# ARPA-SIMC/CRITERIA3D

Hardware: AMD Instinct MI355X
Metric: simulated-hours/sec on 512x512x20 grid (higher is better)
Workload: dtype f64

## Files before the change

### criteria3d_amd/csrc/sf3d_device.h

```cpp
#ifndef SF3D_DEVICE_H
#define SF3D_DEVICE_H

#include <stdint.h>

#define SF3D_SLOTS 10
#ifndef SF3D_LINKS_RING
#define SF3D_LINKS_RING 8
#endif
static_assert(SF3D_LINKS_RING >= 2 && SF3D_LINKS_RING <= 16, "the ring holds the matrix of the step in progress and at least one accepted step's");
#define SF3D_POOL 5
#define SF3D_BLOCK 256
#define SF3D_CHUNK 64
#define SF3D_MAX_BLOCKS 2048
#define CK_NONE 0
#define CK_MIXED 255

enum : uint8_t { LK_NONE = 0, LK_SOIL_VERT = 1, LK_SOIL_LAT = 2, LK_RUNOFF = 3, LK_INFILTRATION = 4 };

enum : uint32_t {
    ST_IDLE = 0,
    ST_ATTEMPT = 1,
    ST_APPROX = 2,
    ST_SWEEP = 3,
    ST_POST = 4,
// ... 100 lines not shown
    uint32_t probePad;
    uint64_t earlyCourant;
    uint64_t counters[8];
    uint64_t heatCounters[4];
};

#define SF3D_MAX_RANKS 16
struct DistMail { unsigned long long w[8]; };
struct DistWindow {
    DistMail mail[2][SF3D_MAX_RANKS];
    unsigned long long ping[SF3D_MAX_RANKS];
    unsigned long long rrec[2][SF3D_MAX_RANKS][4];
};
struct RecGet { uint32_t off0, cnt; };
struct RecPut { uint32_t off0, cnt, peer, nDest; };
struct DistView {
    int32_t world, rank;
    DistWindow* win[SF3D_MAX_RANKS];
    double* payload[SF3D_MAX_RANKS];
    const uint32_t* sendIdx[SF3D_MAX_RANKS]; uint32_t sendCount[SF3D_MAX_RANKS]; uint64_t sendOff[SF3D_MAX_RANKS];
    const uint32_t* recvIdx[SF3D_MAX_RANKS]; uint32_t recvCount[SF3D_MAX_RANKS]; uint64_t recvOff[SF3D_MAX_RANKS];
    const uint8_t* owner;
    const uint32_t* bndStart;
    const uint8_t* bndLane; const uint8_t* bndPeer; const uint32_t* bndSlot;
    const uint32_t* fsrc;
    const RecGet* recGet; const RecPut* recPut;
    int32_t rccl;
    double* mine;
    const double* gathered;
    double* sendBuf[SF3D_MAX_RANKS];
    const double* recvBuf[SF3D_MAX_RANKS];
    unsigned long long* stats;
    long long spinTicks;
};
#define SF3D_DIST_FIELDS 9
enum { DF_X = 0, DF_K = 1, DF_FLOW = 2, DF_RECLO = 3, DF_RECHI = 4, DF_KLO = 5, DF_KHI = 6, DF_FLO = 7, DF_FHI = 8 };
#define SF3D_FSRC_NONE 0xFFFFFFFFu

struct HeatDev {
    uint32_t on, water, vapor, advection, save;
    uint32_t gs;
    uint32_t redBlack;
    const uint8_t* lpar;
    const uint32_t* colourList[2]; uint32_t nColour[2];
    const uint32_t* gsOrder;
    double wf;
    double* TX[3];
    const double* heatSink;
    double *heatFlux, *invariant;
    double *hC, *hcapTerm, *hb, *hD;
    sf3d_d2* hA2;
    const double* hdist;
    const double* airP;
    double* thetaOld;
    double *thAvgC, *thNewC;
    double *kHeat, *kIsoVap, *hAvg;
    double *wThLiq, *wThVap, *wTm;
    const double *bHeightWind, *bHeightT, *bRoughH, *bT, *bRH, *bWind, *bNetIrr, *bFixT, *bFixDepth;
    double *bAero, *bSoilCond, *bSens, *bLat, *bRad, *bAdv;
    sf3d_f2* lwvFlux;
    double* lflux[SF3D_FLUX_TYPES];
};

#define SF3D_PAIR_NONE 15u
#define SF3D_PAIR_UP 9u
#define SF3D_PAIR_DOWN 10u
struct PairGrid {
    uint32_t NX, NY, NZ;
    uint32_t W;
    uint32_t patchCols, patchRows;
    uint32_t ownLo, ownHi;
    const uint32_t* nodeLat;
    const uint64_t* chunkCode;
    uint32_t masked;
    const int32_t* idxMap;
    const uint32_t* patchList;
    const uint8_t* patchDepth;
    uint32_t records;
    uint32_t recFast;
    int32_t sidePeer[2];
    uint32_t putBase[2], getBase[2];
    uint32_t recStride;
    const uint8_t* role;
};

struct ResGrid {
    uint32_t on;
    uint32_t NX, NY, NZ;
    uint32_t PR;
    uint32_t patchCols, rowGroups;
    uint32_t ownLo, ownHi;
    uint32_t K, NW;
    const uint32_t* nodeLat;
    const uint64_t* chunkCode;
    unsigned int* bar;
    unsigned long long* rec;
    unsigned long long* prec;
    unsigned long long* gpub;
    unsigned long long* prec2;
    uint32_t fusedPost;
    double* pub;
    const uint32_t* haloSrc;
    uint32_t forceTimeout;
    int32_t sidePeer[2];
    uint32_t recFast, putBase[2];
};

struct LinksBatch { uint32_t n, slot[SF3D_LINKS_RING]; double dt[SF3D_LINKS_RING]; };

struct DevView {
    uint32_t N, ns, nb;
    uint32_t Nnorm;
    uint32_t nChunks;
    uint32_t qSplit;
    uint32_t nbSurf, nbSoil;
    double probeMin;
    const uint32_t* chunkList; uint32_t nList, nListSurf;
    const uint32_t* asmList;
    uint32_t pLo, pHi;
    uint32_t aLo, aHi;
    const uint32_t* bndList; uint32_t nBnd;
    const uint16_t* lmask;
    uint32_t haloDirect;
    uint32_t ntStream;
    const DistView* dist;
    int32_t world, rank;
    const uint8_t* owner;
    const ChunkDesc* cdesc;
    const double *z, *size, *pond, *sink;
    const uint16_t* cls;
    const uint8_t* btype;
    const double *bslope, *bsize, *prescribed;
    const uint32_t* lto;
    const uint8_t* lkind;
    const uint8_t* probeMask;
    const double *larea, *ldist;
    double* lflowSum;
    sf3d_d2* A2x[SF3D_LINKS_RING];
    double* Hring[SF3D_LINKS_RING];
    double *b, *C;
    double* X[SF3D_POOL];
    double *Se, *SeHold, *K, *flow, *bflowRate, *bflowSum;
    double* compatCv; uint8_t* compatCn; double* compatDiag;
    double *cgDiag, *cgR, *cgP, *cgQ;
    double *part0, *part1;
    double *part2, *part3;
    unsigned int* arrive;
    unsigned int* gridBar;
    const SoilDev* soils;
    const double* roughness;
    PairGrid pair;
    ResGrid res;
    Ctrl* ctrl;
    HeatDev heat;
};

struct MapGeo {
    double cohesion;
    double tanFriction;
    double bulkDensity;
    double present;
};
struct MapView {
    const int32_t* col;
    const double* thick;
    const double* slope;
// ... 346 lines not shown
    const double* db[RAD_DOUBLE_MAPS];
    const int32_t* ok;
    double xll, yll, cellSize;
    float flag, demMax;
};

#define TR_MAX_WIDTH 63
#define TR_WINDOW_SLOTS 24
#define TR_MAX_POINTS 65536
#define TR_WAVE 64
enum { TR_MODE_POINTS = 0, TR_MODE_WINDOW = 1 };
struct TrPointDev {
    double x, y, z;
    RadCellDev cell;
    int32_t inGrid;
    int32_t pad;
};
struct TrView {
    RadGridDev grid;
    const RadHourDev* hours;
    const uint8_t* hourOk;
    const TrPointDev* points;
    const float* measured;
    uint8_t* written;
    float* elevationRefr;
    double* global;
    float* transmissivity;
    int32_t* windowSteps;
    uint32_t nPoints;
    int32_t nSlots, mode;
    float clearSky;
};
struct TrCall {
    const RadHourDev* hours;
    const uint8_t* hourOk;
    const TrPointDev* points;
    const float* measured;
    uint32_t nPoints;
    int32_t nSlots, mode;
    float clearSky;
};

struct HourRelhumView {
    const float* airT;
    const float* dewT;
    float* out;
    const uint8_t* mine;
    uint32_t nCells;
    float flag;
};
#define HOUR_TOTALS 3
struct HourTotalsView {
    const int32_t* col;
    const float* liquid;
    const double* actual;
    const float* dem;
    const uint8_t* mine;
    double* partials;
    double* totals;
    double area;
    uint32_t nCells, nBlocks, pass;
    float flag;
};
struct HourPondUnitDev { double maximumPond, laiMax; int32_t isCrop, pad; };
struct HourPondView {
    const int32_t* col;
    const double* tanSlope;
    const int32_t* unit;
    const float* lai;
    const HourPondUnitDev* units;
    float* out;
    const uint8_t* mine;
    uint32_t nCells;
    float laiFlag;
};
struct HourPondSetup {
    const double* tanSlope;
    const int32_t* unit;
    const HourPondUnitDev* units;
    uint32_t nCells, nUnits;
    uint64_t ver;
};

enum { KID_PROPS = 0, KID_ASSEMBLE, KID_SWEEP, KID_POST, KID_RESTORE, KID_ACCEPT, KID_SWEEP_PAIR, KID_SWEEP_RES, KID_MAPS, KID_COUNT };

#endif
```

### criteria3d_amd/csrc/sf3d_host_build.inc

```

namespace {

const char* kKernelNames[KID_COUNT] = {"k_props", "k_assemble", "k_sweep", "k_post", "k_restore", "k_accept", "k_sweep_pair", "k_sweep_resident", "k_output_map"};

}

struct ResShape { int K, NW; };
#define SF3D_RES_FOR_SHAPES(X) X(2, 5) X(2, 10) X(5, 8)
#define SF3D_RES_SHAPE(k, w) {k, w},
static const ResShape kResShapes[] = {SF3D_RES_FOR_SHAPES(SF3D_RES_SHAPE)};
#undef SF3D_RES_SHAPE

typedef void (*ViewKernel)(DevView);
static inline void launch_view(ViewKernel fn, dim3 grid, dim3 block, uint32_t lds, hipStream_t st, const DevView& v) { hipLaunchKernelGGL(fn, grid, block, lds, st, v); }
static ViewKernel res_kernel(int K, int NW, bool dist)
{
#define SF3D_RES_PTR(k, w) if (K == k && NW == w) return dist ? k_sweep_resident<k, w, true> : k_sweep_resident<k, w, false>;
    SF3D_RES_FOR_SHAPES(SF3D_RES_PTR)
#undef SF3D_RES_PTR
    return nullptr;
}
#define SF3D_PAIR_FOR_HEIGHTS(X) X(6) X(8) X(10) X(14)
static ViewKernel pair_kernel(uint32_t W, bool nt, bool dist, bool records, bool masked)
{
#define SF3D_PAIR_PTR(w)                                                                                                                      \
    if (W == w) {                                                                                                                             \
        if (masked) return dist ? (nt ? k_sweep_pair_masked<w, true, true> : k_sweep_pair_masked<w, false, true>)                             \
                                : (nt ? k_sweep_pair_masked<w, true, false> : k_sweep_pair_masked<w, false, false>);                          \
        if (dist && records) return nt ? k_sweep_pair<w, true, true, true> : k_sweep_pair<w, false, true, true>;                              \
        return dist ? (nt ? k_sweep_pair<w, true, true> : k_sweep_pair<w, false, true>) : (nt ? k_sweep_pair<w, true, false> : k_sweep_pair<w, false, false>); \
    }
    SF3D_PAIR_FOR_HEIGHTS(SF3D_PAIR_PTR)
#undef SF3D_PAIR_PTR
    return nullptr;
}
static ViewKernel sweep_kernel(int mode, bool nt)
{
#define SF3D_SWEEP_PTR(m) if (mode == m) return nt ? k_sweep<m, true> : k_sweep<m, false>;
    SF3D_SWEEP_PTR(0) SF3D_SWEEP_PTR(1) SF3D_SWEEP_PTR(2)
#undef SF3D_SWEEP_PTR
    return nullptr;
}

__global__ void k_dist_ping(DistView d, unsigned long long token, long long timeoutTicks, int* out);

struct MapsCache {
    int32_t* col = nullptr; double* thick = nullptr; double* slope = nullptr; MapGeo* geo = nullptr; float* out = nullptr; int* missing = nullptr;
    uint8_t* mine = nullptr;
    size_t colCap = 0, thickCap = 0, slopeCap = 0, geoCap = 0, outCap = 0, mineCap = 0;
    uint64_t colVer = 0, slopeVer = 0;
    std::vector<MapGeo> geoHost;
    void free_all()
    {
        for (void* q : {(void*)col, (void*)thick, (void*)slope, (void*)geo, (void*)out, (void*)missing, (void*)mine}) if (q) (void)hipFree(q);
        *this = MapsCache();
    }
};

struct SnowCache {
    float* base = nullptr; uint32_t nCells = 0; double lastMs = 0.; bool hourDone = false;
    const float* in[8] = {nullptr, nullptr, nullptr, nullptr, nullptr, nullptr, nullptr, nullptr};
    int feeds = 0;
    bool inputsHeld = false;
};
enum { FEED_METEO = 1, FEED_RAD = 2, FEED_SNOW = 4 };
struct CropCache { float* base = nullptr; CropUnitDev* units = nullptr; uint32_t nCells = 0, nUnits = 0; double lastMs[2] = {0., 0.}; };

struct RootCache {
    char* cells = nullptr;
    char* tables = nullptr;
    double* out = nullptr;
    size_t off[16] = {0};
    uint32_t nCells = 0, nUnits = 0, nSoils = 0, nRows = 0, nrLayers = 0, lunetteMax = 0;
    bool computed = false;
    double lastMs[3] = {0., 0., 0.};
};

struct MeteoCache {
    float* base = nullptr;
    char* stations = nullptr;
    bool hasMap[METEO_MAX_PROXIES] = {false};
    uint32_t nCells = 0, nRows = 0, nCols = 0, nProxies = 0;
    double xll = 0., yll = 0., cellSize = 0.;
    float flag = -9999.f;
    bool produced[METEO_VARIABLES] = {false};
    double lastMs = 0.;
    float* topoMaps = nullptr;
    char* topoTables = nullptr;
    float* topoMatrix = nullptr;
    uint32_t topoPoints = 0, topoMatrixCap = 0;
    double topoMs[3] = {0., 0., 0.};
    char* localFit = nullptr;
    char* localTables = nullptr;
    bool localDone = false;
    double localMs = 0.;
    char* proxiesFit = nullptr;
    char* proxiesTables = nullptr;
    bool proxiesDone = false;
    double proxiesMs = 0.;
};

struct RadCache {
    char* base = nullptr;
    uint32_t nCells = 0, nRows = 0, nCols = 0;
    double xll = 0., yll = 0., cellSize = 0.;
    float flag = -9999.f, demMax = -9999.f;
    double lastMs = 0.;
    bool hourDone = false;
    const float* trRead = nullptr;
    bool trFromMeteo = false;
    char* tr = nullptr;
    size_t trCap = 0, trOff[3] = {0, 0, 0};
    uint32_t trPoints = 0, trSlots = 0;
    double trMs = 0.;
};

struct SinkCache {
    char* cells = nullptr;
    char* tables = nullptr;
    double* nodes = nullptr;
    size_t off[8] = {0};
    uint32_t nCells = 0, nrLayers = 0, nUnits = 0, nSoils = 0, nodesN = 0;
    uint64_t nodesColVer = 0;
    int32_t lastEvapLayer = 0;
    double area = 0.;
    float flag = -9999.f;
    bool computed = false;
    double lastMs = 0.;
    SinkCrackDev crackDev{};
    char* crack = nullptr;
    uint64_t crackVer = 0;
    bool crackComputed = false;
    std::vector<double> layerDepth;
    const float* liquidRead = nullptr;
    int liquidFrom = 0;
};

struct HourCache {
    double* sums = nullptr; size_t sumsCap = 0;
    char* pond = nullptr;
    uint32_t pondCells = 0;
    uint64_t pondVer = 0;
    double lastMs[3] = {0., 0., 0.};
};

struct StepSwitches {
    bool residentGrids = true;
    bool graphs = true;
    bool asmNtOff = false;
    bool pairOddSingle = true;
    long residentFailAt = -1;
    int heatDebug = 0;
    int slabs = 0;
    uint32_t slabPropsBlocks = 512, slabAsmBlocks = 512; double slabFirst = 0.;
};

struct DeviceSolver::Impl {
    int device = -1;
    hipStream_t stream = nullptr;
    int overlapAccept = -1;
    uint32_t ring = 0;
    LinksBatch pend{};
    DevView v{};
    Ctrl* hostCtrl = nullptr;
    std::vector<void*> allocs;
    uint32_t N = 0, ns = 0;
    uint32_t ownedNodes = 0;
    uint32_t lastSweeps = 8;
    uint32_t lastBatches = 1;
    uint32_t predCount = 0, pred[16] = {0};
    uint32_t lastHeatSweeps = 8;
    std::vector<uint32_t> gsLevelStart;
    uint32_t lastHeatSteps = 1;
    double* heatOut[6] = {nullptr};
    double* heatAirP = nullptr;
    std::vector<std::pair<GraphKey, hipGraphExec_t>> graphs;
    template <class F> hipError_t replay(const GraphKey& key, hipStream_t st, F enqueue);
    int useFused = -1;
    StepSwitches sw;
    Partition part;
    DistWindow* window = nullptr;
    size_t windowBytes = 0;
    std::vector<void*> peerMaps;
    DistView hostDist{};
    DistView* devDist = nullptr;
    unsigned long long* distStats = nullptr;
    bool heatJacobiOnly = false;
    double hopUs[SF3D_MAX_RANKS] = {0};
    void* shmOwn = nullptr; int shmFd = -1; char shmName[48] = {0};
    std::vector<std::pair<void*, size_t>> shmPeers;
    std::vector<DistBlob> blobs;
    bool hostMode = false;
    void drop_shm()
    {
        for (auto& pr : shmPeers) { (void)hipHostUnregister(pr.first); munmap(pr.first, pr.second); }
        shmPeers.clear();
        if (shmOwn) { if (hostMode) (void)hipHostUnregister(shmOwn); munmap(shmOwn, windowBytes); shmOwn = nullptr; }
        if (shmFd >= 0) { close(shmFd); shmFd = -1; }
        if (shmName[0]) { shm_unlink(shmName); shmName[0] = 0; }
        hostMode = false;
    }
    uint32_t pushBlocks = 0;
    void* rcclLib = nullptr; ncclComm_t comm = nullptr; bool rcclMode = false;
    ncclResult_t (*pGetUniqueId)(ncclUniqueId*) = nullptr;
    ncclResult_t (*pCommInitRank)(ncclComm_t*, int, ncclUniqueId, int) = nullptr;
    ncclResult_t (*pCommDestroy)(ncclComm_t) = nullptr;
    ncclResult_t (*pSend)(const void*, size_t, ncclDataType_t, int, ncclComm_t, hipStream_t) = nullptr;
    ncclResult_t (*pRecv)(void*, size_t, ncclDataType_t, int, ncclComm_t, hipStream_t) = nullptr;
    ncclResult_t (*pAllGather)(const void*, void*, size_t, ncclDataType_t, ncclComm_t, hipStream_t) = nullptr;
    ncclResult_t (*pAllReduce)(const void*, void*, size_t, ncclDataType_t, ncclRedOp_t, ncclComm_t, hipStream_t) = nullptr;
    ncclResult_t (*pGroupStart)() = nullptr; ncclResult_t (*pGroupEnd)() = nullptr;
    double *rcclMine = nullptr, *rcclGathered = nullptr;
    bool rcclDistinct = false; unsigned char rcclId[128] = {0};
    bool load_rccl()
    {
        if (pAllGather) return true;
        if (const char* le = getenv("SF3D_RCCL_LIB")) if (!rcclLib && le[0]) rcclLib = dlopen(le, RTLD_NOW | RTLD_LOCAL);
        if (!rcclLib) rcclLib = dlopen("librccl.so.1", RTLD_NOW | RTLD_LOCAL);
        if (!rcclLib) rcclLib = dlopen("librccl.so", RTLD_NOW | RTLD_LOCAL);
        if (!rcclLib) return false;
        #define SF3D_SYM(ptr, name) ptr = reinterpret_cast<decltype(ptr)>(dlsym(rcclLib, name)); if (!ptr) return false
        SF3D_SYM(pGetUniqueId, "ncclGetUniqueId"); SF3D_SYM(pCommInitRank, "ncclCommInitRank"); SF3D_SYM(pCommDestroy, "ncclCommDestroy");
        SF3D_SYM(pSend, "ncclSend"); SF3D_SYM(pRecv, "ncclRecv"); SF3D_SYM(pAllReduce, "ncclAllReduce");
        SF3D_SYM(pGroupStart, "ncclGroupStart"); SF3D_SYM(pGroupEnd, "ncclGroupEnd"); SF3D_SYM(pAllGather, "ncclAllGather");
        #undef SF3D_SYM
        return true;
    }
    void rccl_halo(hipStream_t st, int fields)
    {
        pGroupStart();
        for (int p = 0; p < hostDist.world; ++p) {
            if (p == hostDist.rank) continue;
            if (hostDist.sendCount[p]) pSend(hostDist.sendBuf[p], (size_t)hostDist.sendCount[p] * fields, ncclDouble, p, comm, st);
            if (hostDist.recvCount[p]) pRecv(const_cast<double*>(hostDist.recvBuf[p]), (size_t)hostDist.recvCount[p] * fields, ncclDouble, p, comm, st);
        }
        pGroupEnd();
    }
    void rccl_gather(hipStream_t st) { pAllGather(rcclMine, rcclGathered, 4, ncclDouble, comm, st); }
    uint32_t resident_blocks(const void* fn)
    {
        for (auto& r : residentBlocks) if (r.first == fn) return r.second;
        int perCu = 0, dev = 0; hipDeviceProp_t prop;
        uint32_t nbk = SF3D_MAX_BLOCKS;
        if (hipOccupancyMaxActiveBlocksPerMultiprocessor(&perCu, fn, SF3D_BLOCK, 0) == hipSuccess && perCu > 0
            && hipGetDevice(&dev) == hipSuccess && hipGetDeviceProperties(&prop, dev) == hipSuccess && prop.multiProcessorCount > 0)
            nbk = (uint32_t)perCu * (uint32_t)prop.multiProcessorCount;
        if (!sw.residentGrids) nbk = SF3D_MAX_BLOCKS;
        residentBlocks.push_back({fn, nbk});
        return nbk;
    }
    hipError_t flush_links()
    {
        if (pend.n == 0) return hipSuccess;
        const void* fn = v.ntStream ? (const void*)k_links_flush<true> : (const void*)k_links_flush<false>;
        const uint32_t nbk = resident_blocks(fn);
        const dim3 fgrid(v.nb < nbk ? v.nb : nbk);
        if (v.ntStream) hipLaunchKernelGGL(k_links_flush<true>, fgrid, dim3(SF3D_BLOCK), 0, stream, v, pend);
        else hipLaunchKernelGGL(k_links_flush<false>, fgrid, dim3(SF3D_BLOCK), 0, stream, v, pend);
        pend.n = 0;
        return hipGetLastError();
    }
    bool links_pending(uint32_t slot) const { for (uint32_t k = 0; k < pend.n; ++k) if (pend.slot[k] == slot) return true; return false; }
    std::vector<uint8_t> dslot;
    std::vector<double> stage;
    uint32_t connectGen = 0;
    bool warnedShared = false;
    int timing = 0;
    std::vector<std::pair<const void*, uint32_t>> residentBlocks;
    std::vector<uint32_t> propsNeed;
    hipStream_t stream3 = nullptr;
    hipEvent_t evSlab[8] = {};
    uint32_t pairBlocks = 0;
    bool pairMasked = false;
    uint32_t resBlocks = 0, resLds = 0;
    uint32_t resCapacity = 0;
    uint32_t pairRecordsWish = 0;
    uint64_t stepSeq = 0;
    uint64_t stepSeqAll = 0;
    struct Pair { hipEvent_t a, b; int kid; };
    std::vector<Pair> pending;
    std::vector<hipEvent_t> freeEvents;
    uint64_t launches[KID_COUNT] = {0};
    double ms[KID_COUNT] = {0};
    MapsCache maps;
    SnowCache snow;
    CropCache crop;
    RootCache root;
    MeteoCache meteo;
    SinkCache sink;
    RadCache rad;
    HourCache hour;
};

#define HIP_TRY(expr)                                                                          \
    do { hipError_t e_ = (expr);                                                               \
         if (e_ != hipSuccess) {                                                               \
             snprintf(err_, sizeof(err_), "%s failed: %s (%s:%d)", #expr, hipGetErrorString(e_), __FILE__, __LINE__); \
             if (impl_ && impl_->stream) (void)hipStreamSynchronize(impl_->stream);           \
             fatal_ = true;                                                                    \
             return SF3D_SOLVER_ERROR; } } while (0)

#define RASTER_TRY(expr)                                                                       \
    do { hipError_t e_ = (expr);                                                               \
         if (e_ != hipSuccess) {                                                               \
             snprintf(err_, sizeof(err_), "%s failed: %s (%s:%d)", #expr, hipGetErrorString(e_), __FILE__, __LINE__); \
             if (impl_ && impl_->stream) (void)hipStreamSynchronize(impl_->stream);           \
             return SF3D_SOLVER_ERROR; } } while (0)

DeviceSolver& DeviceSolver::instance() { static DeviceSolver s; return s; }
const char* DeviceSolver::kernel_name(int kid) { return (kid >= 0 && kid < KID_COUNT) ? kKernelNames[kid] : nullptr; }

sf3d_error_t DeviceSolver::set_device(int dev)
{
    if (!impl_) impl_ = new Impl();
    int count = 0;
    HIP_TRY(hipGetDeviceCount(&count));
    if (dev < 0 || dev >= count) { snprintf(err_, sizeof(err_), "device %d out of range (%d visible)", dev, count); return SF3D_SOLVER_ERROR; }
    impl_->device = dev;
    HIP_TRY(hipSetDevice(dev));
    return SF3D_OK;
}

static uint64_t g_deviceBytes = 0;
sf3d_error_t DeviceSolver::release()
{
    if (!impl_) return SF3D_OK;
    Impl& I = *impl_;
    if (I.stream) hipStreamSynchronize(I.stream);
    if (I.stream3) hipStreamSynchronize(I.stream3);
#if SF3D_RES_PROFILE
    if (built_ && I.v.res.on && I.v.res.pub) {
        double pr[32];
        if (hipMemcpy(pr, I.v.res.pub, sizeof(pr), hipMemcpyDeviceToHost) == hipSuccess && pr[16] > 0.) {
            const char* names[7] = {"compute + record stores issued", "wave sum + block partial", "halo records", "partial records of all blocks", "barrier B", "norm + decision", "(prologue: per launch, not per iteration)"};
            fprintf(stderr, "[sf3d] resident sweep loop, block 0: %.0f launches, %.2f iterations per launch, %.2f us per launch\n", pr[16], pr[15] / pr[16], pr[17] / pr[16] / 100.);
            for (int p = 0; p < 7; ++p) fprintf(stderr, "[sf3d]   %-40s %7.2f us per iteration\n", names[p], pr[8 + p] / pr[15] / 100.);
        }
    }
#endif
    I.pend.n = 0; I.ring = 0;
    if (I.stream3) {
        (void)hipStreamDestroy(I.stream3); I.stream3 = nullptr;
        for (auto& ev : I.evSlab) if (ev) { (void)hipEventDestroy(ev); ev = nullptr; }
    }
    for (auto& p : I.pending) { I.freeEvents.push_back(p.a); I.freeEvents.push_back(p.b); }
    I.pending.clear();
    for (auto& g : I.graphs) hipGraphExecDestroy(g.second);
    I.graphs.clear();
    for (void* p : I.allocs) hipFree(p);
    I.allocs.clear();
    g_deviceBytes = 0;
    I.maps.free_all();
    if (I.sink.nodes) { (void)hipFree(I.sink.nodes); I.sink.nodes = nullptr; I.sink.nodesN = 0; I.sink.computed = false; }
    if (I.comm && I.pCommDestroy) { I.pCommDestroy(I.comm); I.comm = nullptr; }
    I.rcclMode = false; I.rcclMine = I.rcclGathered = nullptr;
    for (void* p : I.peerMaps) hipIpcCloseMemHandle(p);
    I.peerMaps.clear();
    I.drop_shm();
    if (I.window) { hipFree(I.window); I.window = nullptr; }
    I.devDist = nullptr; I.distStats = nullptr;
// ... 46 lines not shown
            for (const char* q = de; *q;) { char* end = nullptr; const long v = strtol(q, &end, 10); if (end == q) break; list.push_back((int)v); q = (*end == ',') ? end + 1 : end; }
            if (!list.empty()) {
                const int pick = list[(size_t)(dev < 0 ? 0 : dev) % list.size()];
                if (pick < 0 || pick >= count) { snprintf(err_, sizeof(err_), "SF3D_DEVICES names device %d, %d visible", pick, count); return SF3D_SOLVER_ERROR; }
                dev = pick;
            }
        }
        I.device = dev % count;
    }
    HIP_TRY(hipSetDevice(I.device));
    if (!I.stream) HIP_TRY(hipStreamCreateWithFlags(&I.stream, hipStreamNonBlocking));
    return SF3D_OK;
}

struct BuildSwitches {
    bool slotAlign;
    int pairSweep;
    bool residentSweep;
    bool forceMasked;
    uint32_t asmSoilBlocks;
    int overlapAccept;
    int ntStream;
    double probeMin;
    double autoCost;
    bool pairWSet; uint32_t pairW;
    double distTimeoutS;
    int fusedDecide;
    int haloDirect;
    uint32_t pairRecordsWish;
    uint32_t residentPR;
    uint32_t residentPost;
    uint32_t heatRedBlack;
    bool heatDebug, heatGS;
};
static BuildSwitches read_build_switches()
{
    BuildSwitches s;
    const char* re = getenv("SF3D_SLOT_ALIGN");
    s.slotAlign = !(re && re[0] == '0');
    const char* pe = getenv("SF3D_PAIR_SWEEP");
    s.pairSweep = pe ? (pe[0] == '0' ? 0 : 1) : -1;
    const char* rse = getenv("SF3D_RESIDENT_SWEEP");
    s.residentSweep = rse ? rse[0] != '0' : s.pairSweep != 1;
    s.forceMasked = false;
    if (const char* fm = getenv("SF3D_PAIR_FORCE_MASKED")) if (fm[0] == '1') s.forceMasked = true;
    s.asmSoilBlocks = 0;
    if (const char* be = getenv("SF3D_ASM_SOIL_BLOCKS")) s.asmSoilBlocks = (uint32_t)atoi(be);
    const char* oe = getenv("SF3D_OVERLAP_ACCEPT");
    s.overlapAccept = (oe && oe[0] == '0') ? 0 : 1;
    const char* e = getenv("SF3D_NT_STREAM");
    s.ntStream = e ? (e[0] != '0') : -1;
    s.probeMin = 0.8;
    if (const char* ce = getenv("SF3D_COURANT_PROBE")) { s.probeMin = atof(ce); if (ce[0] == '0' && ce[1] == 0) s.probeMin = -1.; if (ce[0] == 'a') s.probeMin = 0.; }
    s.autoCost = 1.9;
    if (const char* ae = getenv("SF3D_PAIR_AUTO_COST")) s.autoCost = atof(ae);
    const char* we = getenv("SF3D_PAIR_W");
    s.pairWSet = we != nullptr; s.pairW = we ? (uint32_t)atoi(we) : 0u;
    {   double ts = 10.; if (const char* te = getenv("SF3D_DIST_TIMEOUT_S")) { ts = atof(te); if (!(ts >= 0.5)) ts = 0.5; if (ts > 600.) ts = 600.; }
        s.distTimeoutS = ts; }
    { const char* fe = getenv("SF3D_FUSED_DECIDE"); s.fusedDecide = (fe && fe[0] == '0') ? 0 : 1; }
    s.haloDirect = -1;
    if (const char* hd = getenv("SF3D_HALO_DIRECT")) s.haloDirect = hd[0] == '1' ? 1 : 0;
    const char* pre = getenv("SF3D_PAIR_RECORDS");
    s.pairRecordsWish = (pre && pre[0] == '0') ? 0u : ((pre && pre[0] == '1') ? 2u : 1u);
    s.residentPR = 0; if (const char* pe = getenv("SF3D_RESIDENT_PR")) s.residentPR = (uint32_t)atoi(pe);
    {   const char* pe2 = getenv("SF3D_RESIDENT_POST"); s.residentPost = (pe2 && pe2[0] == '0') ? 0u : 1u; }
    const char* se = getenv("SF3D_HEAT_SWEEP");
    s.heatRedBlack = (se && se[0] == 'j') ? 0u : 1u;
    s.heatDebug = getenv("SF3D_HEAT_DEBUG") != nullptr;
    s.heatGS = false;
    if (const char* ge = getenv("SF3D_HEAT_GS")) if (ge[0] == '1') s.heatGS = true;
    return s;
}

static StepSwitches read_step_switches()
{
    StepSwitches s;
    auto off = [](const char* name) { const char* e = getenv(name); return e && e[0] == '0'; };
    s.residentGrids = !off("SF3D_RESIDENT_GRIDS");
    s.graphs = !off("SF3D_GRAPHS");
    s.asmNtOff = off("SF3D_ASM_NT");
    s.pairOddSingle = !off("SF3D_PAIR_ODD_SINGLE");
    if (const char* fe = getenv("SF3D_RESIDENT_FAIL_TEST")) s.residentFailAt = strtol(fe, nullptr, 10);
    if (const char* he = getenv("SF3D_HEAT_DEBUG")) s.heatDebug = he[0] == '2' ? 2 : 1;
    { const char* e = getenv("SF3D_SLAB_OVERLAP"); s.slabs = e ? atoi(e) : 0; if (s.slabs > 8) s.slabs = 8; if (s.slabs < 2) s.slabs = 0; }
    auto blocks_of = [](const char* e) -> uint32_t { const long n = e ? strtol(e, nullptr, 10) : 512L; return (uint32_t)(n < 1 ? 1 : (n > SF3D_MAX_BLOCKS ? SF3D_MAX_BLOCKS : n)); };
    s.slabPropsBlocks = blocks_of(getenv("SF3D_SLAB_PROPS_BLOCKS"));
    s.slabAsmBlocks = blocks_of(getenv("SF3D_SLAB_ASM_BLOCKS"));
    if (const char* fe = getenv("SF3D_SLAB_FIRST")) s.slabFirst = atof(fe);
    return s;
}

struct DeviceSolver::BuildState {
    BuildSwitches sw;
    LinkTables links;
    std::vector<ChunkDesc> cdesc;
    GridPlan grid;
    ChunkLists lists;
    EdgeRows edge;
};


sf3d_error_t DeviceSolver::build_dist_window(BuildState& st)
{
    Impl& I = *impl_; DevView& v = I.v; const BuildSwitches& sw = st.sw;
    const uint32_t N = I.N, ns = I.ns, nChunks = v.nChunks; const size_t NS = (size_t)N * SF3D_SLOTS;
    const std::vector<uint8_t>& kind = st.links.kind; const std::vector<uint32_t>& to = st.links.to;
    std::vector<ChunkDesc>& cdesc = st.cdesc; const std::vector<uint32_t>& listSurf = st.lists.listSurf;
    const uint32_t pairNX = st.grid.NX, pairNY = st.grid.NY, pairNZ = st.grid.NZ, pairOwnLo = st.grid.ownLo, pairOwnHi = st.grid.ownHi;
    const int32_t(&edgePeer)[2] = st.edge.edgePeer; const uint32_t(&edgePut)[2] = st.edge.edgePut, (&edgeGet)[2] = st.edge.edgeGet;
    auto edge_rows_direct = [&]() -> bool { return plan_edge_rows_direct(I.part, st.grid, ns, world_, rank_, st.edge); };
    uint8_t* downer; HIP_TRY(dev_alloc(I.allocs, downer, N));
    HIP_TRY(hipMemcpy(downer, I.part.owner.data(), N, hipMemcpyHostToDevice));
    v.owner = downer;
    DistView& d = I.hostDist;
    std::memset(&d, 0, sizeof(d));
    d.world = world_; d.rank = rank_; d.owner = downer;
    d.spinTicks = (long long)(sw.distTimeoutS * 1e8);
    uint64_t off = 0;
    uint32_t maxSend = 0;
    for (int pr = 0; pr < world_; ++pr) {
        d.recvCount[pr] = (uint32_t)I.part.recv[pr].size();
        d.recvOff[pr] = off;
        off += (uint64_t)d.recvCount[pr] * 2 * SF3D_DIST_FIELDS;
        d.sendCount[pr] = (uint32_t)I.part.send[pr].size();
        if (d.sendCount[pr] > maxSend) maxSend = d.sendCount[pr];
        uint32_t *si, *ri;
        HIP_TRY(dev_alloc(I.allocs, si, I.part.send[pr].size())); HIP_TRY(dev_alloc(I.allocs, ri, I.part.recv[pr].size()));
        if (d.sendCount[pr]) HIP_TRY(hipMemcpy(si, I.part.send[pr].data(), (size_t)d.sendCount[pr] * 4, hipMemcpyHostToDevice));
        if (d.recvCount[pr]) HIP_TRY(hipMemcpy(ri, I.part.recv[pr].data(), (size_t)d.recvCount[pr] * 4, hipMemcpyHostToDevice));
        d.sendIdx[pr] = si; d.recvIdx[pr] = ri;
    }
    {
        struct Ent { uint32_t node; uint8_t peer; uint32_t slot; };
        std::vector<Ent> ents;
        for (int pr = 0; pr < world_; ++pr)
            for (uint32_t k = 0; k < I.part.send[pr].size(); ++k) ents.push_back({I.part.send[pr][k], (uint8_t)pr, k});
        std::sort(ents.begin(), ents.end(), [](const Ent& a, const Ent& b) { return a.node != b.node ? a.node < b.node : a.peer < b.peer; });
        std::vector<uint32_t> bstart(nChunks + 1, 0), bslot(ents.size());
        std::vector<uint8_t> blane(ents.size()), bpeer(ents.size());
        for (size_t k = 0; k < ents.size(); ++k) {
            bstart[ents[k].node / SF3D_CHUNK + 1]++;
            blane[k] = (uint8_t)(ents[k].node % SF3D_CHUNK); bpeer[k] = ents[k].peer; bslot[k] = ents[k].slot;
        }
        for (uint32_t q = 0; q < nChunks; ++q) bstart[q + 1] += bstart[q];
        uint32_t *dbs, *dsl; uint8_t *dla, *dpe;
        HIP_TRY(dev_alloc(I.allocs, dbs, bstart.size())); HIP_TRY(dev_alloc(I.allocs, dsl, bslot.size()));
        HIP_TRY(dev_alloc(I.allocs, dla, blane.size())); HIP_TRY(dev_alloc(I.allocs, dpe, bpeer.size()));
        HIP_TRY(hipMemcpy(dbs, bstart.data(), bstart.size() * 4, hipMemcpyHostToDevice));
        if (!ents.empty()) {
            HIP_TRY(hipMemcpy(dsl, bslot.data(), bslot.size() * 4, hipMemcpyHostToDevice));
            HIP_TRY(hipMemcpy(dla, blane.data(), blane.size(), hipMemcpyHostToDevice));
            HIP_TRY(hipMemcpy(dpe, bpeer.data(), bpeer.size(), hipMemcpyHostToDevice));
        }
        d.bndStart = dbs; d.bndSlot = dsl; d.bndLane = dla; d.bndPeer = dpe;
    }
    v.haloDirect = I.useFused != 0 ? 1u : 0u;
    if (sw.haloDirect >= 0) v.haloDirect = (sw.haloDirect == 1 && I.useFused != 0) ? 1u : 0u;
    if (v.haloDirect) {
        std::vector<uint32_t> fsrc(NS, SF3D_FSRC_NONE);
        for (uint32_t i = 0; i < N; ++i) {
            if (I.part.owner[i] != rank_) continue;
            for (int sl = 0; sl < SF3D_SLOTS; ++sl) {
                const size_t e = (size_t)sl * N + i;
                if (kind[e] == LK_NONE) continue;
                const uint32_t j = to[e];
// ... 33 lines not shown
        if (ok && !bnd.empty()) {
            uint32_t* db; HIP_TRY(dev_alloc(I.allocs, db, bnd.size()));
            HIP_TRY(hipMemcpy(db, bnd.data(), bnd.size() * 4, hipMemcpyHostToDevice));
            v.bndList = db; v.nBnd = (uint32_t)bnd.size();
        } else if (!ok || I.pairMasked || (pairOwnLo > 0 || pairOwnHi < pairNY)) { I.pairBlocks = 0; v.pair.NX = v.pair.NY = v.pair.NZ = 0; }
    }
    v.pair.records = 0u; d.recGet = nullptr; d.recPut = nullptr; I.pairRecordsWish = 0u;
    if (I.pairBlocks != 0) {
        if (I.pairMasked) {
            std::vector<RecGet> rg(N, RecGet{SF3D_FSRC_NONE, 0u});
            std::vector<RecPut> rp(N, RecPut{0u, 0u, 0u, 0u});
            bool fits = true;
            for (int pr = 0; pr < world_; ++pr) {
                const uint64_t rc = d.recvCount[pr], sc = d.sendCount[pr];
                for (uint32_t k = 0; k < rc; ++k) {
                    const uint64_t o = d.recvOff[pr] + (uint64_t)DF_RECLO * rc + k;
                    if (o + (uint64_t)2 * SF3D_DIST_FIELDS * rc >= 0xFFFFFFFFull) fits = false;
                    rg[I.part.recv[pr][k]] = RecGet{(uint32_t)o, (uint32_t)rc};
                }
                for (uint32_t k = 0; k < sc; ++k) {
                    RecPut& e = rp[I.part.send[pr][k]];
                    if (e.nDest == 0u) {
                        e.off0 = (uint32_t)((uint64_t)DF_RECLO * sc + k); e.cnt = (uint32_t)sc; e.peer = (uint32_t)pr;
                    }
                    e.nDest++;
                }
            }
            if (fits) {
                RecGet* dg; RecPut* dp;
                HIP_TRY(dev_alloc(I.allocs, dg, N)); HIP_TRY(dev_alloc(I.allocs, dp, N));
                HIP_TRY(hipMemcpy(dg, rg.data(), (size_t)N * sizeof(RecGet), hipMemcpyHostToDevice));
                HIP_TRY(hipMemcpy(dp, rp.data(), (size_t)N * sizeof(RecPut), hipMemcpyHostToDevice));
                d.recGet = dg; d.recPut = dp;
            }
        }
        I.pairRecordsWish = sw.pairRecordsWish;
        if (I.pairRecordsWish != 0u) {
            bool all = true;
            for (uint32_t i = 0; i < N && all; ++i) {
                const int pr = I.part.owner[i];
                if (pr == rank_ || pr == SF3D_OWNER_NONE) continue;
                const auto& lst = I.part.recv[pr];
                const auto it = std::lower_bound(lst.begin(), lst.end(), i);
                if (it == lst.end() || *it != i) all = false;
            }
            v.pair.recFast = 0u; v.pair.sidePeer[0] = v.pair.sidePeer[1] = -1; v.pair.recStride = pairNX;
            if (all && !I.pairMasked && edge_rows_direct()) {
                v.pair.recFast = 1u;
                for (int side = 0; side < 2; ++side) { v.pair.sidePeer[side] = edgePeer[side]; v.pair.putBase[side] = edgePut[side]; v.pair.getBase[side] = edgeGet[side]; }
            }
            v.pair.records = (all && (I.pairMasked ? (d.recPut != nullptr && d.recGet != nullptr && pairNZ < 128u ) : v.pair.recFast != 0u)) ? 1u : 0u;
        }
    }
    I.windowBytes = sizeof(DistWindow) + off * sizeof(double);
    void* w = nullptr;
    HIP_TRY(hipExtMallocWithFlags(&w, I.windowBytes, hipDeviceMallocFinegrained));
    HIP_TRY(hipMemset(w, 0, I.windowBytes));
    I.window = static_cast<DistWindow*>(w);
    d.win[rank_] = I.window;
    d.payload[rank_] = reinterpret_cast<double*>(reinterpret_cast<char*>(w) + sizeof(DistWindow));
    HIP_TRY(dev_alloc(I.allocs, I.devDist, 1));
    HIP_TRY(dev_alloc(I.allocs, I.distStats, 1 + 2 * SF3D_MAX_RANKS));
    HIP_TRY(hipMemset(I.distStats, 0, sizeof(unsigned long long) * (1 + 2 * SF3D_MAX_RANKS)));
    d.stats = I.distStats;
    for (double& h : I.hopUs) h = 0.;
    I.pushBlocks = (maxSend + SF3D_BLOCK - 1) / SF3D_BLOCK;
    if (I.pushBlocks == 0) I.pushBlocks = 1;
    if (I.pushBlocks > 256) I.pushBlocks = 256;
    return SF3D_OK;
}

sf3d_error_t DeviceSolver::build_resident_plan(const HostModel& m, BuildState& st)
{
    Impl& I = *impl_; DevView& v = I.v; const BuildSwitches& sw = st.sw;
    const uint32_t N = I.N, ns = I.ns;
    const std::vector<uint64_t>&pairNode = st.grid.node, &pairChunk = st.grid.chunk; const std::vector<int32_t>& pairIdxMap = st.grid.idxMap;
    const uint32_t pairNX = st.grid.NX, pairNY = st.grid.NY, pairNZ = st.grid.NZ, pairOwnLo = st.grid.ownLo, pairOwnHi = st.grid.ownHi;
    const int32_t(&edgePeer)[2] = st.edge.edgePeer; const uint32_t(&edgePut)[2] = st.edge.edgePut;
    auto edge_rows_direct = [&]() -> bool { return plan_edge_rows_direct(I.part, st.grid, ns, world_, rank_, st.edge); };
    {
        v.res = ResGrid{};
        I.resBlocks = 0; I.resLds = 0;
        const bool asked = sw.residentSweep;
        const bool want = asked && I.useFused != 0 && !pairNode.empty() && pairIdxMap.empty() && (world_ == 1 || v.haloDirect);
        if (want) {
            const uint32_t ownRows = pairOwnHi - pairOwnLo, patchCols = pairNX / 64;
            int cus = 256; { hipDeviceProp_t prop; if (hipGetDeviceProperties(&prop, I.device) == hipSuccess && prop.multiProcessorCount > 0) cus = prop.multiProcessorCount; }
            const uint32_t onlyPR = sw.residentPR;
            for (uint32_t PR = 1; PR <= 8 && !v.res.on; ++PR) {
                if (ownRows % PR != 0 || (onlyPR != 0 && PR != onlyPR)) continue;
                const uint32_t blocks = patchCols * (ownRows / PR), T = PR * pairNZ;
                const uint32_t lds = 2u * pairNZ * (PR + 2) * SF3D_RES_RS * 8u;
                for (const ResShape& sh : kResShapes) {
                    if ((uint32_t)(sh.K * sh.NW) < T || (uint32_t)sh.NW % PR != 0) continue;
                    if (pairNZ * (2u * SF3D_RES_RS + 2u * PR) > (uint32_t)SF3D_RES_HM * sh.NW * 64u) continue;
                    const void* fn = (const void*)res_kernel(sh.K, sh.NW, world_ > 1);
                    if (!fn) continue;
                    if (lds > 48u * 1024u && hipFuncSetAttribute(fn, hipFuncAttributeMaxDynamicSharedMemorySize, (int)lds) != hipSuccess) { (void)hipGetLastError(); continue; }
                    int perCu = 0;
                    if (hipOccupancyMaxActiveBlocksPerMultiprocessor(&perCu, fn, sh.NW * 64, lds) != hipSuccess || perCu < 1) { (void)hipGetLastError(); continue; }
                    if (blocks > (uint32_t)perCu * (uint32_t)cus) continue;
                    v.res.on = 1; v.res.NX = pairNX; v.res.NY = pairNY; v.res.NZ = pairNZ; v.res.PR = PR;
                    v.res.patchCols = patchCols; v.res.rowGroups = ownRows / PR; v.res.ownLo = pairOwnLo; v.res.ownHi = pairOwnHi;
                    v.res.K = (uint32_t)sh.K; v.res.NW = (uint32_t)sh.NW;
                    I.resBlocks = blocks; I.resLds = lds; I.resCapacity = (uint32_t)perCu * (uint32_t)cus;
                    break;
                }
            }
        }
        if (v.res.on) {
            if (v.pair.nodeLat && v.pair.chunkCode && !v.pair.masked && v.pair.NX == pairNX) { v.res.nodeLat = v.pair.nodeLat; v.res.chunkCode = v.pair.chunkCode; }
            else {
                uint32_t* dn; uint64_t* dq;
                std::vector<uint32_t> lat(pairNode.size());
                for (size_t k = 0; k < pairNode.size(); ++k) lat[k] = (uint32_t)(pairNode[k] >> 8);
                HIP_TRY(dev_alloc(I.allocs, dn, lat.size()));
                HIP_TRY(hipMemcpy(dn, lat.data(), lat.size() * 4, hipMemcpyHostToDevice));
                HIP_TRY(dev_alloc(I.allocs, dq, pairChunk.size()));
                HIP_TRY(hipMemcpy(dq, pairChunk.data(), pairChunk.size() * 8, hipMemcpyHostToDevice));
                v.res.nodeLat = dn; v.res.chunkCode = dq;
            }
            HIP_TRY(dev_alloc(I.allocs, v.res.bar, (size_t)SF3D_RES_LINE * 18)); HIP_TRY(hipMemset(v.res.bar, 0, (size_t)SF3D_RES_LINE * 18 * sizeof(unsigned int)));
            HIP_TRY(dev_alloc(I.allocs, v.res.rec, (size_t)4 * N)); HIP_TRY(hipMemset(v.res.rec, 0, (size_t)4 * N * sizeof(unsigned long long)));
            HIP_TRY(dev_alloc(I.allocs, v.res.prec, (size_t)8 * I.resBlocks)); HIP_TRY(hipMemset(v.res.prec, 0, (size_t)8 * I.resBlocks * sizeof(unsigned long long)));
            HIP_TRY(dev_alloc(I.allocs, v.res.gpub, 8)); HIP_TRY(hipMemset(v.res.gpub, 0, 8 * sizeof(unsigned long long)));
            HIP_TRY(dev_alloc(I.allocs, v.res.prec2, (size_t)8 * I.resBlocks)); HIP_TRY(hipMemset(v.res.prec2, 0, (size_t)8 * I.resBlocks * sizeof(unsigned long long)));
            {   v.res.fusedPost = sw.residentPost;
                if (m.heat) v.res.fusedPost = 0u; }
            HIP_TRY(dev_alloc(I.allocs, v.res.pub, 32)); HIP_TRY(hipMemset(v.res.pub, 0, 32 * sizeof(double)));
            if (world_ > 1) {
                std::vector<uint32_t> hs((size_t)2 * pairNZ * pairNX, SF3D_FSRC_NONE);
                v.res.sidePeer[0] = v.res.sidePeer[1] = -1;
                bool oneRank = true;
                for (uint32_t side = 0; side < 2; ++side) {
                    if ((side == 0 && pairOwnLo == 0) || (side == 1 && pairOwnHi >= pairNY)) continue;
                    const uint32_t r = side == 0 ? pairOwnLo - 1 : pairOwnHi;
                    for (uint32_t l = 0; l < pairNZ; ++l)
                        for (uint32_t cc = 0; cc < pairNX; ++cc) {
                            const uint32_t j = l * ns + r * pairNX + cc;
                            const int pr = I.part.owner[j];
                            if (pr == rank_ || pr == SF3D_OWNER_NONE) continue;
                            const auto& lst = I.part.recv[pr];
                            const auto itp = std::lower_bound(lst.begin(), lst.end(), j);
                            if (itp != lst.end() && *itp == j) {
                                hs[((size_t)side * pairNZ + l) * pairNX + cc] = ((uint32_t)pr << 27) | (uint32_t)(itp - lst.begin());
                                if (v.res.sidePeer[side] < 0) v.res.sidePeer[side] = pr; else if (v.res.sidePeer[side] != pr) oneRank = false;
                            }
                        }
                }
                uint32_t* dh; HIP_TRY(dev_alloc(I.allocs, dh, hs.size()));
                HIP_TRY(hipMemcpy(dh, hs.data(), hs.size() * 4, hipMemcpyHostToDevice));
                v.res.haloSrc = dh;
                v.res.recFast = 0u; v.res.putBase[0] = v.res.putBase[1] = 0u;
                if (oneRank && edge_rows_direct() && edgePeer[0] == v.res.sidePeer[0] && edgePeer[1] == v.res.sidePeer[1]) {
                    v.res.recFast = 1u; v.res.putBase[0] = edgePut[0]; v.res.putBase[1] = edgePut[1];
                }
                if (!oneRank) { v.res.on = 0; I.resBlocks = 0; }
            }
        }
    }
    return SF3D_OK;
}

sf3d_error_t DeviceSolver::build_heat(HostModel& m, const ParamsHost& p, BuildState& st)
{
    Impl& I = *impl_; DevView& v = I.v; const BuildSwitches& sw = st.sw;
    const uint32_t N = I.N, ns = I.ns, nChunks = v.nChunks; const size_t NS = (size_t)N * SF3D_SLOTS;
// ... 174 lines not shown
        }
        v.pLo = 0; v.pHi = v.nList; v.aLo = v.nListSurf; v.aHi = v.nList;
        double *z, *size, *pond, *sink, *bslope, *bsize, *prescribed, *roughness, *larea, *ldist;
        uint16_t* cls; uint8_t *btype, *lkind; uint32_t* lto; SoilDev* soils; ChunkDesc* dcdesc;
        HIP_TRY(dev_alloc(I.allocs, z, N)); HIP_TRY(dev_alloc(I.allocs, size, N));
        HIP_TRY(dev_alloc(I.allocs, pond, N)); HIP_TRY(dev_alloc(I.allocs, sink, N));
        HIP_TRY(dev_alloc(I.allocs, cls, N)); HIP_TRY(dev_alloc(I.allocs, btype, N));
        HIP_TRY(dev_alloc(I.allocs, bslope, N)); HIP_TRY(dev_alloc(I.allocs, bsize, N));
        HIP_TRY(dev_alloc(I.allocs, prescribed, N));
        HIP_TRY(dev_alloc(I.allocs, lto, NS)); HIP_TRY(dev_alloc(I.allocs, lkind, NS));
        HIP_TRY(dev_alloc(I.allocs, larea, NS)); HIP_TRY(dev_alloc(I.allocs, ldist, NS));
        HIP_TRY(dev_alloc(I.allocs, v.lflowSum, NS)); HIP_TRY(dev_alloc(I.allocs, v.A2x[0], NS / 2)); HIP_TRY(dev_alloc(I.allocs, v.A2x[1], NS / 2));
        {
            I.overlapAccept = sw.overlapAccept;
            I.ring = 0; I.pend.n = 0;
            if (I.overlapAccept && world_ == 1 && !m.compat) {
                const size_t keep = I.allocs.size(); const uint64_t bytesBefore = g_deviceBytes;
                bool ok = true;
                for (int k = 2; k < SF3D_LINKS_RING && ok; ++k) ok = dev_alloc(I.allocs, v.A2x[k], NS / 2) == hipSuccess;
                for (int k = 0; k < SF3D_LINKS_RING && ok; ++k) ok = dev_alloc(I.allocs, v.Hring[k], N) == hipSuccess;
                if (ok) I.ring = SF3D_LINKS_RING;
                else {
                    (void)hipGetLastError();
                    while (I.allocs.size() > keep) { (void)hipFree(I.allocs.back()); I.allocs.pop_back(); }
                    g_deviceBytes = bytesBefore;
                    for (int k = 2; k < SF3D_LINKS_RING; ++k) v.A2x[k] = nullptr;
                    for (int k = 0; k < SF3D_LINKS_RING; ++k) v.Hring[k] = nullptr;
                }
            }
        }
        HIP_TRY(dev_alloc(I.allocs, v.b, N)); HIP_TRY(dev_alloc(I.allocs, v.C, N));
        for (int k = 0; k < SF3D_POOL; ++k) HIP_TRY(dev_alloc(I.allocs, v.X[k], N));
        HIP_TRY(dev_alloc(I.allocs, v.Se, N)); HIP_TRY(dev_alloc(I.allocs, v.K, N)); HIP_TRY(dev_alloc(I.allocs, v.SeHold, N));
        HIP_TRY(dev_alloc(I.allocs, dcdesc, (size_t)nChunks));
        uint32_t* dlist; HIP_TRY(dev_alloc(I.allocs, dlist, listSurf.size()));
        if (!listSurf.empty()) HIP_TRY(hipMemcpy(dlist, listSurf.data(), listSurf.size() * 4, hipMemcpyHostToDevice));
        v.chunkList = dlist;
        v.asmList = dlist;
        v.owner = nullptr; v.dist = nullptr;
        {
            const double sweepBytes = 152.0 * (double)v.nList * SF3D_CHUNK;
            v.ntStream = sw.ntStream >= 0 ? sw.ntStream : (sweepBytes > 256.0 * 1024 * 1024);
        }
        {
            v.probeMin = sw.probeMin;
        }
        I.pairBlocks = 0; I.pairMasked = false; v.pair.masked = 0;
        plan_strip_rows(I.part, N, ns, world_, rank_, st.grid);
        if (!pairNode.empty()) {
            bool on = sw.pairSweep >= 0 ? (sw.pairSweep != 0) : (v.ntStream != 0);
            const double autoCost = sw.autoCost;
            const bool tryAuto = sw.pairSweep < 0 && !on && autoCost > 0.;
            if (on || tryAuto) {
                int cus = 256; { hipDeviceProp_t prop; if (hipGetDeviceProperties(&prop, I.device) == hipSuccess && prop.multiProcessorCount > 0) cus = prop.multiProcessorCount; }
                const PairPlan pp = plan_pair_patches(st.grid, I.part, world_, rank_, cus, SF3D_PAIR_WAVES, tryAuto, autoCost, sw.pairWSet, sw.pairW);
                const uint32_t bestW = pp.bestW, ownRows = pairOwnHi - pairOwnLo;
                const std::vector<uint32_t>(&plist)[4] = pp.plist; const std::vector<uint8_t>(&pdepth)[4] = pp.pdepth;
                if (bestW) {
                    uint32_t* dn; uint64_t* dq;
                    {
                        std::vector<uint32_t> lat(pairNode.size());
                        for (size_t k = 0; k < pairNode.size(); ++k) lat[k] = (uint32_t)(pairNode[k] >> 8);
                        HIP_TRY(dev_alloc(I.allocs, dn, lat.size()));
                        HIP_TRY(hipMemcpy(dn, lat.data(), lat.size() * 4, hipMemcpyHostToDevice));
                    }
                    HIP_TRY(dev_alloc(I.allocs, dq, pairChunk.size()));
                    HIP_TRY(hipMemcpy(dq, pairChunk.data(), pairChunk.size() * 8, hipMemcpyHostToDevice));
                    v.pair.NX = pairNX; v.pair.NY = pairNY; v.pair.NZ = pairNZ; v.pair.W = bestW;
                    v.pair.ownLo = pairOwnLo; v.pair.ownHi = pairOwnHi;
                    v.pair.patchCols = pairNX / 64; v.pair.patchRows = (ownRows + bestW - 3) / (bestW - 2);
                    v.pair.nodeLat = dn; v.pair.chunkCode = dq;
                    I.pairBlocks = v.pair.patchCols * v.pair.patchRows;
                    v.pair.masked = 0; I.pairMasked = false;
                    if (!pairIdxMap.empty()) {
                        const int wi = pair_widx(bestW);
                        int32_t* dm; uint32_t* dl; uint8_t* dd;
                        HIP_TRY(dev_alloc(I.allocs, dm, pairIdxMap.size())); HIP_TRY(dev_alloc(I.allocs, dl, plist[wi].size())); HIP_TRY(dev_alloc(I.allocs, dd, pdepth[wi].size()));
                        HIP_TRY(hipMemcpy(dm, pairIdxMap.data(), pairIdxMap.size() * 4, hipMemcpyHostToDevice));
                        HIP_TRY(hipMemcpy(dl, plist[wi].data(), plist[wi].size() * 4, hipMemcpyHostToDevice));
                        HIP_TRY(hipMemcpy(dd, pdepth[wi].data(), pdepth[wi].size(), hipMemcpyHostToDevice));
                        v.pair.masked = 1; v.pair.idxMap = dm; v.pair.patchList = dl; v.pair.patchDepth = dd;
                        I.pairBlocks = (uint32_t)plist[wi].size(); I.pairMasked = true;
                    }
                }
            }
        }
        if (world_ > 1) { const sf3d_error_t e = build_dist_window(st); if (e != SF3D_OK) return e; }
        { const sf3d_error_t e = build_resident_plan(m, st); if (e != SF3D_OK) return e; }
        if (m.compat) {
            HIP_TRY(dev_alloc(I.allocs, v.compatCv, (size_t)N * (SF3D_SLOTS + 2))); HIP_TRY(hipMemset(v.compatCv, 0, (size_t)N * (SF3D_SLOTS + 2) * 8));
            HIP_TRY(dev_alloc(I.allocs, v.compatCn, N)); HIP_TRY(hipMemset(v.compatCn, 0, N));
            HIP_TRY(dev_alloc(I.allocs, v.compatDiag, N)); HIP_TRY(hipMemset(v.compatDiag, 0, (size_t)N * 8));
        }
        if (m.cgArrays && world_ == 1) {
            HIP_TRY(dev_alloc(I.allocs, v.cgDiag, N)); HIP_TRY(dev_alloc(I.allocs, v.cgR, N)); HIP_TRY(dev_alloc(I.allocs, v.cgP, N)); HIP_TRY(dev_alloc(I.allocs, v.cgQ, N));
            HIP_TRY(hipMemset(v.cgDiag, 0, (size_t)N * 8)); HIP_TRY(hipMemset(v.cgR, 0, (size_t)N * 8)); HIP_TRY(hipMemset(v.cgP, 0, (size_t)N * 8)); HIP_TRY(hipMemset(v.cgQ, 0, (size_t)N * 8));
        }
        HIP_TRY(dev_alloc(I.allocs, v.flow, N)); HIP_TRY(dev_alloc(I.allocs, v.bflowRate, N));
        HIP_TRY(dev_alloc(I.allocs, v.bflowSum, N));
        {   const size_t np = std::max<size_t>(v.nb + v.nbSurf, I.pairBlocks) + 8;
            HIP_TRY(dev_alloc(I.allocs, v.part0, np)); HIP_TRY(dev_alloc(I.allocs, v.part1, np));
            HIP_TRY(dev_alloc(I.allocs, v.part2, np)); HIP_TRY(dev_alloc(I.allocs, v.part3, np)); }
        HIP_TRY(dev_alloc(I.allocs, v.arrive, 16 * 17)); HIP_TRY(hipMemset(v.arrive, 0, 16 * 17 * sizeof(unsigned int)));
        HIP_TRY(dev_alloc(I.allocs, v.gridBar, 16)); HIP_TRY(hipMemset(v.gridBar, 0, 16 * sizeof(unsigned int)));
        HIP_TRY(dev_alloc(I.allocs, soils, m.soils.size())); HIP_TRY(dev_alloc(I.allocs, roughness, m.roughness.size()));
        HIP_TRY(dev_alloc(I.allocs, v.ctrl, 1));
        v.z = z; v.size = size; v.pond = pond; v.sink = sink; v.cls = cls; v.btype = btype;
        v.bslope = bslope; v.bsize = bsize; v.prescribed = prescribed;
        v.lto = lto; v.lkind = lkind; v.larea = larea; v.ldist = ldist; v.soils = soils; v.roughness = roughness;
        v.cdesc = dcdesc;

        I.heatAirP = nullptr;
        if (m.heat) { const sf3d_error_t e = build_heat(m, p, st); if (e != SF3D_OK) return e; }

        std::vector<SoilDev> sd(m.soils.size());
        for (size_t k = 0; k < sd.size(); ++k) {
            const SoilHost& s = m.soils[k];
            sd[k] = SoilDev{s.alpha, s.n, s.m, s.he, s.Sc, 1.0 / s.Sc, s.thetaS, s.thetaR, s.Ksat, s.L, 1.0 / s.m, s.mualemDen, s.clay, s.organicMatter};
        }
        HIP_TRY(hipMemcpy(z, m.z.data(), N * 8, hipMemcpyHostToDevice));
        HIP_TRY(hipMemcpy(size, m.size.data(), N * 8, hipMemcpyHostToDevice));
        HIP_TRY(hipMemcpy(cls, m.cls.data(), N * 2, hipMemcpyHostToDevice));
        HIP_TRY(hipMemcpy(lto, to.data(), NS * 4, hipMemcpyHostToDevice));
        HIP_TRY(hipMemcpy(lkind, kind.data(), NS, hipMemcpyHostToDevice));
        {
            const std::vector<uint8_t> pm = plan_probe_mask(st.links, N, ns);
            for (int sl = 0; sl < 2 && v.probeMin >= 0.; ++sl)
                for (uint32_t i = 0; i < ns; ++i) if (kind[(size_t)sl * N + i] == LK_RUNOFF) { v.probeMin = -1.; break; }
            uint8_t* dpm; HIP_TRY(dev_alloc(I.allocs, dpm, (size_t)(ns ? ns : 1)));
            if (ns) HIP_TRY(hipMemcpy(dpm, pm.data(), ns, hipMemcpyHostToDevice));
            v.probeMask = dpm;
        }
        {   std::vector<uint16_t> mask(N, 0);
            for (int sl = 0; sl < SF3D_SLOTS; ++sl) { const uint8_t* kk = kind.data() + (size_t)sl * N; for (uint32_t i = 0; i < N; ++i) if (kk[i] != LK_NONE) mask[i] |= (uint16_t)(1u << sl); }
            uint16_t* dm; HIP_TRY(dev_alloc(I.allocs, dm, N));
            HIP_TRY(hipMemcpy(dm, mask.data(), (size_t)N * 2, hipMemcpyHostToDevice));
            v.lmask = dm; }
        HIP_TRY(hipMemcpy(larea, area.data(), NS * 8, hipMemcpyHostToDevice));
        HIP_TRY(hipMemcpy(ldist, dist.data(), NS * 8, hipMemcpyHostToDevice));
        HIP_TRY(hipMemcpy(dcdesc, cdesc.data(), cdesc.size() * sizeof(ChunkDesc), hipMemcpyHostToDevice));
        if (!sd.empty()) HIP_TRY(hipMemcpy(soils, sd.data(), sd.size() * sizeof(SoilDev), hipMemcpyHostToDevice));
        if (!m.roughness.empty()) HIP_TRY(hipMemcpy(roughness, m.roughness.data(), m.roughness.size() * 8, hipMemcpyHostToDevice));
        for (uint32_t k = 0; k < (I.ring ? I.ring : 2u); ++k) HIP_TRY(hipMemset(v.A2x[k], 0, NS * 8));
        for (uint32_t k = 0; k < I.ring; ++k) HIP_TRY(hipMemset(v.Hring[k], 0, N * 8));
        HIP_TRY(hipMemset(v.b, 0, N * 8)); HIP_TRY(hipMemset(v.C, 0, N * 8));
        HIP_TRY(hipMemset(v.flow, 0, N * 8)); HIP_TRY(hipMemset(v.bflowRate, 0, N * 8)); HIP_TRY(hipMemset(v.SeHold, 0, N * 8));
        for (int k = 0; k < SF3D_POOL; ++k) HIP_TRY(hipMemset(v.X[k], 0, N * 8));
        if (m.heat && I.heatAirP) hipLaunchKernelGGL(k_heat_static, dim3(v.nb), dim3(SF3D_BLOCK), 0, 0, v, I.heatAirP);
        HIP_TRY(hipDeviceSynchronize());

        std::memset(&mirror_, 0, sizeof(mirror_));
        mirror_.cur = 0; mirror_.hold = 0; mirror_.best = -1; mirror_.stage = ST_IDLE;
        mirror_.bestMBR = NODATA_D;
        mirror_.tCur = 0; mirror_.tOld = 0; mirror_.hStage = HS_IDLE;
        mirror_.aRing = I.ring ? I.ring : 2u;
        built_ = true;
        m.graphDirty = false;
        m.stateDirty = m.sinkDirty = m.pondDirty = m.boundaryDirty = m.flowSumsDirty = m.ctrlDirty = true;
        m.sinkLo = 0; m.sinkHi = UINT32_MAX;
        m.hostStaleState = m.hostStaleFlows = false;
    }

    DevView& v = I.v;
    if (m.stateDirty) {
        HIP_TRY(hipMemcpyAsync(v.X[mirror_.cur], m.H.data(), N * 8, hipMemcpyHostToDevice, I.stream));
        HIP_TRY(hipMemcpyAsync(v.Se, m.Se.data(), N * 8, hipMemcpyHostToDevice, I.stream));
// ... 59 lines not shown
```

### criteria3d_amd/csrc/sf3d_host_plan.inc

```
#include <algorithm>
#include <atomic>
#include <cmath>
#include <cstdio>
#include <cstdlib>
#include <cstring>
#include <thread>
#include <vector>

namespace {

template <class F> void parallel_for(uint32_t n, F f)
{
    unsigned nt = std::thread::hardware_concurrency();
    if (nt == 0) nt = 1;
    if (nt > 16) nt = 16;
    if (n < 65536 || nt == 1) { f(0u, n); return; }
    std::vector<std::thread> th;
    const uint32_t chunk = (n + nt - 1) / nt;
    for (unsigned t = 0; t < nt; ++t) {
        const uint32_t a = t * chunk, b = (a + chunk < n) ? a + chunk : n;
        if (a >= b) break;
        th.emplace_back([=] { f(a, b); });
    }
    for (auto& t : th) t.join();
// ... 184 lines not shown
                    kind[e] = LK_INFILTRATION;
                    const uint32_t su = sj ? i : j, so = sj ? j : i;
                    dist[e] = m.z[su] - m.z[so];
                }
            }
            if (m.btype[i] == SF3D_BND_FREE_DRAINAGE && m.ltype[0][i] == SF3D_LINK_NONE
                && (m.presetPartition == nullptr || m.presetPartition->owner[i] == rank)) bad = true;
        }
    });
    if (bad) { snprintf(err, errLen, "FreeDrainage node without an Up link"); return SF3D_BOUNDARY_ERROR; }
    t.kind.swap(kind); t.dist.swap(dist); t.area.swap(area); t.to.swap(to);
    return SF3D_OK;
}

inline std::vector<ChunkDesc> plan_chunk_descriptors(const LinkTables& t, uint32_t N, uint32_t ns)
{
    const std::vector<uint8_t>& kind = t.kind; const std::vector<double>&dist = t.dist, &area = t.area; const std::vector<uint32_t>& to = t.to;
    const uint32_t nChunks = (N + SF3D_CHUNK - 1) / SF3D_CHUNK;
    std::vector<ChunkDesc> cdesc(nChunks);
    parallel_for(nChunks, [&](uint32_t qa, uint32_t qb) {
        for (uint32_t q = qa; q < qb; ++q) {
            const uint32_t i0 = q * SF3D_CHUNK, i1 = (i0 + SF3D_CHUNK < N) ? i0 + SF3D_CHUNK : N;
            ChunkDesc d;
            std::memset(&d, 0, sizeof(d));
            d.rowType = (i1 <= ns) ? 0 : (i0 >= ns ? 1 : 2);
            for (int s = 0; s < SF3D_SLOTS; ++s) {
                bool any = false, all = true, same = true, sameDelta = true;
                uint8_t k0 = LK_NONE; int64_t d0 = 0;
                for (uint32_t i = i0; i < i1; ++i) {
                    const size_t e = (size_t)s * N + i;
                    if (kind[e] == LK_NONE) { all = false; continue; }
                    const int64_t dd = (int64_t)to[e] - (int64_t)i;
                    if (!any) { any = true; k0 = kind[e]; d0 = dd; }
                    else { if (kind[e] != k0 || dd != d0) same = false; if (dd != d0) sameDelta = false; }
                }
                const bool fits = d0 >= INT32_MIN && d0 <= INT32_MAX;
                uint8_t ck = CK_NONE;
                if (any) ck = (all && same && fits) ? k0 : (uint8_t)CK_MIXED;
                d.kind[s] = ck;
                d.ukind[s] = any ? ((same && fits) ? k0 : (uint8_t)CK_MIXED) : (uint8_t)CK_NONE;
                d.delta[s] = (ck != CK_NONE && ck != CK_MIXED) ? (int32_t)d0 : 0;
                if (ck == CK_MIXED && sameDelta && fits) { d.delta[s] = (int32_t)d0; d.sweepUniform |= (uint16_t)(1u << s); }
                if (any) {
                    bool first = true, uni = true; double a0 = 0.;
                    for (uint32_t i = i0; i < i1 && uni; ++i) {
                        const size_t e = (size_t)s * N + i;
                        if (kind[e] == LK_NONE) continue;
                        if (first) { a0 = area[e]; first = false; }
                        else if (area[e] != a0) uni = false;
                    }
                    if (uni) { d.areaUniform |= (uint16_t)(1u << s); d.area[s] = a0; }
                    first = true; uni = true; double d0v = 0.;
                    for (uint32_t i = i0; i < i1 && uni; ++i) {
                        const size_t e = (size_t)s * N + i;
                        if (kind[e] == LK_NONE) continue;
                        if (first) { d0v = dist[e]; first = false; }
                        else if (dist[e] != d0v) uni = false;
                    }
                    if (uni) { d.distUniform |= (uint16_t)(1u << s); d.dist[s] = d0v; }
                }
            }
            {
                bool su = d.rowType == 1 && i1 - i0 == SF3D_CHUNK, partial = false;
                for (int s = 0; s < SF3D_SLOTS && su; ++s) {
                    if (d.kind[s] == CK_NONE) continue;
                    if (d.kind[s] == CK_MIXED) partial = true;
                    su = (d.ukind[s] == LK_SOIL_VERT || d.ukind[s] == LK_SOIL_LAT) && (d.kind[s] != CK_MIXED || ((d.sweepUniform >> s) & 1u))
                         && ((d.areaUniform >> s) & 1u) && ((d.distUniform >> s) & 1u);
                }
                d.soilUniform = su ? (partial ? 2 : 1) : 0;
            }
            cdesc[q] = d;
        }
    });
    return cdesc;
}

inline bool plan_regular_box(const LinkTables& t, const HostModel& m, GridPlan& g)
{
    const std::vector<uint8_t>& kind = t.kind; const std::vector<uint32_t>& to = t.to;
    std::vector<uint64_t>&pairNode = g.node, &pairChunk = g.chunk;
    uint32_t &pairNX = g.NX, &pairNY = g.NY, &pairNZ = g.NZ;
    const uint32_t N = m.N, ns = m.ns, nChunks = (N + SF3D_CHUNK - 1) / SF3D_CHUNK;
    bool regular = ns >= 64 && N % ns == 0 && N / ns >= 2 && N < (1u << 28);
    int64_t maxOff = 0;
    if (regular) {
        for (int sl = 2; sl < SF3D_SLOTS && regular; ++sl)
            for (uint32_t i = 0; i < N; ++i) {
                const size_t e = (size_t)sl * N + i;
                if (kind[e] == LK_NONE) continue;
                const int64_t o = std::llabs((int64_t)to[e] - (int64_t)i);
                if (o > maxOff) maxOff = o;
            }
        const int64_t NX = maxOff - 1;
        regular = NX >= 64 && NX % 64 == 0 && ns % (uint64_t)NX == 0 && ns / (uint64_t)NX >= 6;
        if (regular) { pairNX = (uint32_t)NX; pairNY = (uint32_t)(ns / (uint64_t)NX); pairNZ = N / ns; }
    }
    if (regular) {
        pairNode.assign(N, 0);
        std::atomic<bool> irregular{false};
        const int64_t NX = pairNX, NY = pairNY;
        parallel_for(N, [&](uint32_t a, uint32_t b) {
            for (uint32_t i = a; i < b && !irregular.load(std::memory_order_relaxed); ++i) {
                const int64_t l = i / ns, r = (i % ns) / NX, cidx = i % NX;
                uint64_t code = 0; unsigned seen = 0;
                for (int sl = 0; sl < SF3D_SLOTS; ++sl) {
                    const size_t e = (size_t)sl * N + i;
                    uint64_t nib = SF3D_PAIR_NONE;
                    if (kind[e] != LK_NONE) {
                        const int64_t off = (int64_t)to[e] - (int64_t)i;
                        if (sl == 0) { if (off != -(int64_t)ns) irregular = true; nib = SF3D_PAIR_UP; }
                        else if (sl == 1) { if (off != (int64_t)ns) irregular = true; nib = SF3D_PAIR_DOWN; }
                        else {
                            const int64_t rr = (off >= 0) ? (off + NX / 2) / NX : -((-off + NX / 2) / NX), cc = off - rr * NX;
                            if (rr < -1 || rr > 1 || cc < -1 || cc > 1 || (rr == 0 && cc == 0) || r + rr < 0 || r + rr >= NY || cidx + cc < 0 || cidx + cc >= NX
                                || (int64_t)(to[e] / ns) != l) { irregular = true; break; }
                            nib = (uint64_t)((rr + 1) * 3 + (cc + 1));
                            if (seen & (1u << nib)) irregular = true;
                            seen |= 1u << nib;
                        }
                    }
                    code |= nib << (4 * sl);
                }
                pairNode[i] = code;
            }
        });
        regular = !irregular;
    }
    if (regular) {
        pairChunk.assign(nChunks, 0);
        for (uint32_t q = 0; q < nChunks; ++q) {
            bool same = (size_t)(q + 1) * SF3D_CHUNK <= N;
            for (uint32_t k = 1; k < SF3D_CHUNK && same; ++k) same = pairNode[(size_t)q * SF3D_CHUNK + k] == pairNode[(size_t)q * SF3D_CHUNK];
            if (same) pairChunk[q] = pairNode[(size_t)q * SF3D_CHUNK] | (1ull << 63);
        }
    } else { pairNode.clear(); pairNX = pairNY = pairNZ = 0; }
    return regular;
}

inline bool plan_masked_grid(const LinkTables& t, const HostModel& m, int world, int rank, GridPlan& g)
{
    const std::vector<uint8_t>& kind = t.kind; const std::vector<uint32_t>& to = t.to;
    std::vector<uint64_t>&pairNode = g.node, &pairChunk = g.chunk; std::vector<int32_t>& pairIdxMap = g.idxMap;
    uint32_t &pairNX = g.NX, &pairNY = g.NY, &pairNZ = g.NZ;
    const uint32_t N = m.N, ns = m.ns, nChunks = (N + SF3D_CHUNK - 1) / SF3D_CHUNK;
    if (ns >= 64 && N < (1u << 28) && m.x.size() == N && m.y.size() == N) {
        bool ok = true;
        std::vector<int32_t> lay(N, -1), row(N, -1), colv(N, -1);
        double cell = 0.;
        for (int sl = 2; sl < SF3D_SLOTS; ++sl)
            for (uint32_t i = 0; i < ns; ++i) {
                const size_t e = (size_t)sl * N + i;
                if (kind[e] == LK_NONE) continue;
                const double dx = std::fabs(m.x[to[e]] - m.x[i]), dy = std::fabs(m.y[to[e]] - m.y[i]);
                const double d = dx > 0 ? (dy > 0 ? std::min(dx, dy) : dx) : dy;
                if (d > 0 && (cell == 0. || d < cell)) cell = d;
            }
        ok = cell > 0.;
        double xmin = 0, ymin = 0, ymax = 0;
        bool northFirst = false;
        auto place_rc = [&](uint32_t i) -> bool {
            const double fc = (m.x[i] - xmin) / cell, fr = (northFirst ? (ymax - m.y[i]) : (m.y[i] - ymin)) / cell;
            const long long c = std::llround(fc), r = std::llround(fr);
            if (std::fabs(fc - (double)c) > 1e-6 || std::fabs(fr - (double)r) > 1e-6 || c < 0 || r < 0 || c > 60000 || r > 60000) return false;
            row[i] = (int32_t)r; colv[i] = (int32_t)c;
            return true;
        };
// ... 140 lines not shown
        if (ok && pairIdxMap.empty()) {
            while (lo < pairNY && rowMine[lo] != 1) ++lo;
            hi = lo;
            while (hi < pairNY && rowMine[hi] == 1) ++hi;
            for (uint32_t r = hi; r < pairNY && ok; ++r) if (rowMine[r] == 1) ok = false;
            if (hi <= lo) ok = false;
        }
        if (ok) { pairOwnLo = lo; pairOwnHi = hi; }
        else { pairNode.clear(); pairChunk.clear(); pairNX = pairNY = pairNZ = 0; }
    }
    return !pairNode.empty();
}

inline PairPlan plan_pair_patches(const GridPlan& g, const Partition& part, int world, int rank, int cus, int pairWaves, bool tryAuto, double autoCost,
                                  bool wSet, uint32_t onlyW)
{
    const std::vector<int32_t>& pairIdxMap = g.idxMap;
    const uint32_t pairNX = g.NX, pairNY = g.NY, pairNZ = g.NZ, pairOwnLo = g.ownLo, pairOwnHi = g.ownHi;
    PairPlan pp;
    uint32_t& bestW = pp.bestW; double bestCost = 1e30;
    std::vector<uint32_t>(&plist)[4] = pp.plist; std::vector<uint8_t>(&pdepth)[4] = pp.pdepth;
    if (!pairIdxMap.empty()) {
        std::vector<uint8_t> colDepth((size_t)pairNX * pairNY, 0);
        for (uint32_t l = 0; l < pairNZ; ++l)
            for (size_t k = 0; k < colDepth.size(); ++k)
                if (pairIdxMap[(size_t)l * colDepth.size() + k] >= 0) colDepth[k] = (uint8_t)(l + 1);
        std::vector<uint8_t> colMine(colDepth.size(), 1);
        if (world > 1) for (size_t k = 0; k < colMine.size(); ++k) colMine[k] = pairIdxMap[k] >= 0 && part.owner[(uint32_t)pairIdxMap[k]] == rank;
        int wi = 0;
        for (uint32_t W : {6u, 8u, 10u, 14u}) {
            const uint32_t prs = (pairNY + W - 3) / (W - 2);
            std::vector<uint8_t> band(pairNX);
            for (uint32_t pr = 0; pr < prs; ++pr) {
                const int64_t r0 = (int64_t)pr * (W - 2) - 1;
                std::fill(band.begin(), band.end(), 0);
                for (int64_t r = r0 + 1; r < r0 + (int64_t)W - 1 && r < (int64_t)pairNY; ++r)
                    for (uint32_t cc = 0; cc < pairNX; ++cc) if (colDepth[(size_t)r * pairNX + cc] && colMine[(size_t)r * pairNX + cc]) band[cc] = 1;
                uint32_t cc = 0;
                while (cc < pairNX) {
                    if (!band[cc]) { ++cc; continue; }
                    const uint32_t c0 = pairNX <= 4096 ? cc : cc / 64 * 64;
                    uint8_t depth = 0;
                    for (int64_t r = r0; r < r0 + (int64_t)W; ++r) {
                        if (r < 0 || r >= (int64_t)pairNY) continue;
                        for (int64_t x = (int64_t)c0 - 1; x < (int64_t)c0 + 65; ++x) {
                            if (x < 0 || x >= (int64_t)pairNX) continue;
                            const uint8_t d = colDepth[(size_t)r * pairNX + (size_t)x];
                            if (d > depth) depth = d;
                        }
                    }
                    if (world > 1 && pairNZ < 128u)
                        for (int64_t r = r0 - 1; r < r0 + (int64_t)W + 1 && !(depth & 0x80u); ++r) {
                            if (r < 0 || r >= (int64_t)pairNY) continue;
                            for (int64_t x = (int64_t)c0 - 2; x < (int64_t)c0 + 66; ++x) {
                                if (x < 0 || x >= (int64_t)pairNX) continue;
                                const size_t k = (size_t)r * pairNX + (size_t)x;
                                if (colDepth[k] && !colMine[k]) { depth |= 0x80u; break; }
                            }
                        }
                    plist[wi].push_back(pairNX <= 4096 ? ((pr << 12) | c0) : ((pr << 12) | (c0 / 64)));
                    pdepth[wi].push_back(depth);
                    cc = c0 + 64;
                }
            }
            {
                const uint32_t nbk = (uint32_t)plist[wi].size(), per = nbk >> 3, rem = nbk & 7u;
                uint32_t at = 0;
                for (uint32_t x = 0; x < 8 && nbk >= 8; ++x) {
                    const uint32_t len = per + (x < rem ? 1u : 0u);
                    std::vector<uint32_t> ord(len);
                    for (uint32_t k = 0; k < len; ++k) ord[k] = at + k;
                    std::stable_sort(ord.begin(), ord.end(), [&](uint32_t a, uint32_t b) { return pdepth[wi][a] > pdepth[wi][b]; });
                    std::vector<uint32_t> pl(len); std::vector<uint8_t> pd(len);
                    for (uint32_t k = 0; k < len; ++k) { pl[k] = plist[wi][ord[k]]; pd[k] = pdepth[wi][ord[k]]; }
                    std::copy(pl.begin(), pl.end(), plist[wi].begin() + at); std::copy(pd.begin(), pd.end(), pdepth[wi].begin() + at);
                    at += len;
                }
            }
            ++wi;
        }
    }
    const uint32_t ownRows = pairOwnHi - pairOwnLo;
    for (uint32_t W : {6u, 8u, 10u, 14u}) {
        if (pairNY < W || (wSet && onlyW != W)) continue;
        if (W == 8 && !wSet) continue;
        const uint64_t blocks = pairIdxMap.empty() ? (uint64_t)((ownRows + W - 3) / (W - 2)) * (pairNX / 64) : (uint64_t)plist[pair_widx(W)].size();
        if (blocks == 0) continue;
        const uint64_t perCU = (uint64_t)(4 * pairWaves / (W + 1)), resident = perCU * cus;
        double quant = 1., busyShare = 1., wavesPerCU = (double)(perCU * (W + 1));
        if (blocks >= resident) { const uint64_t rounds = (blocks + resident - 1) / resident; quant = (double)(rounds * resident) / (double)blocks; }
        else { const uint64_t busy = std::min<uint64_t>(blocks, (uint64_t)cus); busyShare = (double)busy / cus; wavesPerCU = (double)blocks / (double)busy * (W + 1); }
        const double cost = (1. + 0.6 / (double)(W - 2)) * quant * (1. + 3.26 / (busyShare * wavesPerCU)) / std::sqrt(busyShare);
        if (cost < bestCost) { bestCost = cost; bestW = W; }
    }
    if (tryAuto && !(bestCost < autoCost)) bestW = 0;
    return pp;
}

inline bool plan_edge_rows_direct(const Partition& part, const GridPlan& g, uint32_t ns, int world, int rank, EdgeRows& er)
{
    const uint32_t pairNX = g.NX, pairNY = g.NY, pairNZ = g.NZ, pairOwnLo = g.ownLo, pairOwnHi = g.ownHi;
    int32_t(&edgePeer)[2] = er.edgePeer; uint32_t(&edgePut)[2] = er.edgePut, (&edgeGet)[2] = er.edgeGet;
    if (pairNX == 0 || pairOwnHi - pairOwnLo < 2) return false;
    for (uint32_t side = 0; side < 2; ++side) {
        if ((side == 0 && pairOwnLo == 0) || (side == 1 && pairOwnHi >= pairNY)) continue;
        const uint32_t rEdge = side == 0 ? pairOwnLo : pairOwnHi - 1, rHalo = side == 0 ? pairOwnLo - 1 : pairOwnHi;
        const int pr = part.owner[rHalo * pairNX];
        if (pr == rank || pr == SF3D_OWNER_NONE || pr >= world) return false;
        const auto& sl = part.send[pr]; const auto& rl = part.recv[pr];
        const auto si = std::lower_bound(sl.begin(), sl.end(), rEdge * pairNX), ri = std::lower_bound(rl.begin(), rl.end(), rHalo * pairNX);
        if (si == sl.end() || ri == rl.end()) return false;
        const size_t sb = (size_t)(si - sl.begin()), rb = (size_t)(ri - rl.begin());
        for (uint32_t l = 0; l < pairNZ; ++l)
            for (uint32_t cc = 0; cc < pairNX; ++cc) {
                const size_t ks = sb + (size_t)l * pairNX + cc, kr = rb + (size_t)l * pairNX + cc;
                if (ks >= sl.size() || kr >= rl.size() || sl[ks] != l * ns + rEdge * pairNX + cc || rl[kr] != l * ns + rHalo * pairNX + cc
                    || part.owner[l * ns + rHalo * pairNX + cc] != pr) return false;
            }
        edgePeer[side] = pr; edgePut[side] = (uint32_t)sb; edgeGet[side] = (uint32_t)rb;
    }
    return true;
}

inline std::vector<uint8_t> plan_probe_mask(const LinkTables& t, uint32_t N, uint32_t ns)
{
    const std::vector<uint8_t>& kind = t.kind; const std::vector<uint32_t>& to = t.to;
    std::vector<uint8_t> pm(ns, 0);
    parallel_for(ns, [&](uint32_t a, uint32_t b) {
        for (uint32_t i = a; i < b; ++i)
            for (int sl = 2; sl < SF3D_SLOTS; ++sl) {
                const size_t e = (size_t)sl * N + i;
                if (kind[e] != LK_RUNOFF) continue;
                const uint32_t j = to[e];
                bool mineToDo = j > i;
                if (!mineToDo) {
                    bool back = false;
                    for (int s2 = 2; s2 < SF3D_SLOTS && !back; ++s2) back = kind[(size_t)s2 * N + j] == LK_RUNOFF && to[(size_t)s2 * N + j] == i;
                    mineToDo = !back || j == i;
                }
                if (mineToDo) pm[i] |= (uint8_t)(1u << (sl - 2));
            }
    });
    return pm;
}

struct StepFacts {
    bool multi = false;
    bool heatOn = false;
    bool useFused = true;
    bool lineal = false, haveCg = false;
    bool resAvail = false, resFusedPost = false;
    bool haloDirect = false, rccl = false;
    uint32_t nBnd = 0;
    bool pairAvail = false;
    int timing = 0; bool sampled = false;
    bool overlapAccept = false, ring = false;
    bool compat = false;
    bool ntStream = false, asmNtOff = false;
    double probeMin = -1., courant = 0.; uint32_t probeBudget = 0;
    int slabs = 0; bool havePropsNeed = false; uint32_t nList = 0, nListSurf = 0;
    bool useGraphs = true, heatGs = false;
    long residentFailAt = -1; uint64_t residentSteps = 0;
};
struct StepPlan {
    bool useFused;
    bool fused, fusedMulti;
    bool linealOn;
    bool resOn;
    bool resFusedPost;
    bool countsResidentStep, forceTimeout;
    bool pairOn;
    bool timedStep;
    bool overlap;
    bool compat, asmNT;
    bool probeNow;
    bool slabOn;
    bool replayWater, replayHeat;
};
inline StepPlan plan_step(const StepFacts& f)
{
    StepPlan P;
    P.useFused = f.useFused || (f.heatOn && f.multi);
    P.fused = !f.multi && P.useFused;
    P.fusedMulti = f.multi && P.useFused;
    P.linealOn = f.lineal && f.haveCg && !f.multi && P.useFused;
    P.resOn = f.resAvail && (P.fused || (P.fusedMulti && f.haloDirect && !f.rccl)) && !P.linealOn;
    P.resFusedPost = P.resOn && f.resFusedPost;
    P.countsResidentStep = P.resOn && !f.multi;
    P.forceTimeout = P.countsResidentStep && f.residentFailAt >= 0 && (long)f.residentSteps == f.residentFailAt;
    P.pairOn = !P.resOn && (P.fused || (P.fusedMulti && f.haloDirect && f.nBnd != 0)) && f.pairAvail && !P.linealOn;
    P.timedStep = f.timing == 1 || (f.timing == 2 && f.sampled);
    P.overlap = f.overlapAccept && !f.multi && f.ring && !P.timedStep && f.timing != 1 && !f.compat;
    P.compat = f.compat;
    P.asmNT = f.ntStream && !f.asmNtOff;
    P.probeNow = f.probeMin >= 0. && !f.heatOn && !f.multi && !f.compat && f.courant >= 0.75 * f.probeMin && (f.probeBudget > 0 || f.probeMin == 0.);
    P.slabOn = f.slabs >= 2 && !f.multi && !f.heatOn && P.useFused && !f.compat && !P.timedStep && f.timing != 1 && f.havePropsNeed
               && f.nList > f.nListSurf + 64u * (uint32_t)f.slabs;
    P.replayWater = f.useGraphs && !P.timedStep && !f.rccl;
    P.replayHeat = f.useGraphs && !f.heatGs;
    return P;
}

inline uint32_t predicted_sweeps(uint32_t index, bool withHead, uint32_t predCount, const uint32_t* pred, uint32_t lastSweeps)
{
    uint32_t chunk;
    if (withHead && index < predCount && index < 16u) { chunk = pred[index] + 1; if (chunk < 2) chunk = 2; }
    else { chunk = lastSweeps + 2; if (chunk < 4) chunk = 4; }
    if (chunk > 40) chunk = 40;
    return chunk;
}
struct PairSchedule { uint32_t nPairs, singleAfter; };
inline PairSchedule pair_schedule(uint32_t chunk, bool oddSingle)
{
    const uint32_t expected = chunk > 1 ? chunk - 1 : 1;
    return {oddSingle ? expected / 2 + 1 : (chunk + 1) / 2, (oddSingle && (expected & 1u)) ? expected / 2 : UINT32_MAX};
}
inline uint32_t heat_chunk(uint32_t lastHeatSweeps)
{
    const uint32_t chunk = ((lastHeatSweeps + 1 + 1) / 2) * 2;
    return chunk < 4 ? 4 : (chunk > 64 ? 64 : chunk);
}
inline uint32_t water_look_ahead(uint32_t lastBatches) { return lastBatches < 1 ? 1 : (lastBatches > 6 ? 6 : lastBatches); }
inline uint32_t heat_look_ahead(uint32_t lastHeatSteps, bool gs) { return gs ? 1 : (lastHeatSteps < 1 ? 1 : (lastHeatSteps > 8 ? 8 : lastHeatSteps)); }

enum : uint32_t { GK_HEAT = 1u, GK_HEAD = 2u, GK_TAIL = 4u, GK_RES = 8u, GK_RES_POST = 16u, GK_RES_FAIL = 32u, GK_OVERLAP = 64u, GK_PAIR = 128u,
                  GK_LINEAL = 256u, GK_PROBE = 512u, GK_SLAB = 1024u, GK_SAVE = 2048u };
struct GraphKey {
    uint32_t flags, sweeps, steps;
    bool operator==(const GraphKey& o) const { return flags == o.flags && sweeps == o.sweeps && steps == o.steps; }
};
inline GraphKey water_graph_key(const StepPlan& P, bool withHead, bool withTail, uint32_t chunk)
{
    const uint32_t flags = (withHead ? GK_HEAD : 0u) | (withTail ? GK_TAIL : 0u) | (P.resOn ? GK_RES : 0u) | (P.resFusedPost ? GK_RES_POST : 0u) | (P.forceTimeout ? GK_RES_FAIL : 0u)
                           | (P.overlap ? GK_OVERLAP : 0u) | (P.pairOn ? GK_PAIR : 0u) | (P.linealOn ? GK_LINEAL : 0u) | (P.probeNow ? GK_PROBE : 0u) | (P.slabOn ? GK_SLAB : 0u);
    return {flags, P.resOn ? 0u : chunk, 0u};
}
inline GraphKey heat_graph_key(uint32_t steps, uint32_t chunk, bool save) { return {GK_HEAT | (save ? GK_SAVE : 0u), chunk, steps}; }
```

### criteria3d_amd/csrc/sf3d_host_step.inc

```
sf3d_error_t DeviceSolver::fetch_state(HostModel& m)
{
    Impl& I = *impl_;
    HIP_TRY(hipMemcpyAsync(m.H.data(), I.v.X[mirror_.cur], (size_t)m.N * 8, hipMemcpyDeviceToHost, I.stream));
    HIP_TRY(hipMemcpyAsync(m.Se.data(), I.v.Se, (size_t)m.N * 8, hipMemcpyDeviceToHost, I.stream));
    HIP_TRY(hipMemcpyAsync(m.K.data(), I.v.K, (size_t)m.N * 8, hipMemcpyDeviceToHost, I.stream));
    HIP_TRY(hipStreamSynchronize(I.stream));
    m.hostStaleState = false;
    return SF3D_OK;
}

sf3d_error_t DeviceSolver::fetch_flows(HostModel& m)
{
    Impl& I = *impl_;
    const size_t N = m.N;
    HIP_TRY(I.flush_links());
    HIP_TRY(hipMemcpyAsync(m.bflowSum.data(), I.v.bflowSum, N * 8, hipMemcpyDeviceToHost, I.stream));
    HIP_TRY(hipMemcpyAsync(m.bflowRate.data(), I.v.bflowRate, N * 8, hipMemcpyDeviceToHost, I.stream));
    if (I.dslot.empty()) {
        for (int s = 0; s < SF3D_SLOTS; ++s)
            HIP_TRY(hipMemcpyAsync(m.lflowSum[s].data(), I.v.lflowSum + (size_t)s * N, N * 8, hipMemcpyDeviceToHost, I.stream));
        HIP_TRY(hipStreamSynchronize(I.stream));
    } else {
        I.stage.resize(N * SF3D_SLOTS);
        HIP_TRY(hipMemcpyAsync(I.stage.data(), I.v.lflowSum, N * SF3D_SLOTS * 8, hipMemcpyDeviceToHost, I.stream));
// ... 621 lines not shown
                if (!h) h = dlopen("libroctx64.so", RTLD_NOW | RTLD_GLOBAL);
                if (h) { push() = reinterpret_cast<push_t>(dlsym(h, "roctxRangePushA")); pop() = reinterpret_cast<pop_t>(dlsym(h, "roctxRangePop")); }
                if (push() && pop()) state = 1;
                else fprintf(stderr, "sf3d: SF3D_ROCTX=1 but no roctx library could be loaded: no ranges\n");
            }
        }
        return state == 1;
    }
};
struct RoctxRange {
    bool active;
    explicit RoctxRange(const char* name) : active(Roctx::on()) { if (active) Roctx::push()(name); }
    ~RoctxRange() { if (active) Roctx::pop()(); }
    RoctxRange(const RoctxRange&) = delete; RoctxRange& operator=(const RoctxRange&) = delete;
};
}


template <class F> hipError_t DeviceSolver::Impl::replay(const GraphKey& key, hipStream_t st, F enqueue)
{
    for (auto& g : graphs) if (g.first == key) return hipGraphLaunch(g.second, st);
    hipGraph_t graph = nullptr; hipGraphExec_t exec = nullptr;
    hipError_t e = hipStreamBeginCapture(st, hipStreamCaptureModeThreadLocal);
    if (e != hipSuccess) return e;
    enqueue();
    e = hipStreamEndCapture(st, &graph);
    if (e != hipSuccess) return e;
    e = hipGraphInstantiate(&exec, graph, nullptr, nullptr, 0);
    (void)hipGraphDestroy(graph);
    if (e != hipSuccess) return e;
    graphs.push_back({key, exec});
    return hipGraphLaunch(exec, st);
}

static ViewKernel assemble_kernel(bool fused, bool nt, bool heat)
{
    if (heat) return fused ? (nt ? k_assemble<true, true, true> : k_assemble<true, false, true>) : k_assemble<false, false, true>;
    return fused ? (nt ? k_assemble<true, true, false> : k_assemble<true, false, false>) : (nt ? k_assemble<false, true, false> : k_assemble<false, false, false>);
}

struct StepCounts {
    uint64_t counters[8], pairLaunches, singleLaunches, earlyCourant, residentLaunches;
    explicit StepCounts(const Ctrl& c) : pairLaunches(c.pairLaunches), singleLaunches(c.singleLaunches), earlyCourant(c.earlyCourant), residentLaunches(c.residentLaunches)
    { std::memcpy(counters, c.counters, sizeof(counters)); }
};

struct DeviceSolver::StepCtx {
    Impl& I;
    const DevView& v;
    const StepPlan P;
    const hipStream_t st;
    const bool multi, heatOn;
    const dim3 grid, block, one, pgrid;
    dim3 propsGrid, propsHeatGrid, acceptGrid;
    ViewKernel sweepFn = nullptr;
    dim3 gSaveWater, gBoundary, gHProps, gHAsm, gHPost, gHSave;
    bool slabFailed = false;

    StepCtx(Impl& impl, const StepPlan& plan, bool multiRank)
        : I(impl), v(impl.v), P(plan), st(impl.stream), multi(multiRank), heatOn(impl.v.heat.on != 0), grid(impl.v.nb), block(SF3D_BLOCK), one(1), pgrid(impl.pushBlocks ? impl.pushBlocks : 1) {}

    dim3 resident(ViewKernel fn) const
    {
        const uint32_t nbk = I.resident_blocks((const void*)fn);
        return dim3(v.nb < nbk ? v.nb : nbk);
    }
    void launch(ViewKernel fn, dim3 g) const { launch_view(fn, g, block, 0, st, v); }
    template <class F> void timed(int kid, F queue)
    {
        if (!P.timedStep || (I.timing == 2 && kid != KID_SWEEP && kid != KID_SWEEP_PAIR && kid != KID_SWEEP_RES)) { queue(); return; }
        hipEvent_t a, b;
        if (I.freeEvents.size() >= 2) { a = I.freeEvents.back(); I.freeEvents.pop_back(); b = I.freeEvents.back(); I.freeEvents.pop_back(); }
        else { (void)hipEventCreate(&a); (void)hipEventCreate(&b); }
        (void)hipEventRecord(a, st); queue(); (void)hipEventRecord(b, st);
        I.pending.push_back({a, b, kid});
    }
    void timed_launch(int kid, ViewKernel fn, dim3 g) { timed(kid, [&] { launch(fn, g); }); }

    bool water_grids()
    {
        propsGrid = resident(k_props<0, false>); propsHeatGrid = resident(k_props<0, true>);
        acceptGrid = resident(v.ntStream ? k_accept<true> : k_accept<false>);
        if (P.resOn) sweepFn = res_kernel((int)v.res.K, (int)v.res.NW, multi);
        else if (P.pairOn) sweepFn = pair_kernel(v.pair.W, v.ntStream != 0, multi, v.pair.records != 0, I.pairMasked);
        return sweepFn != nullptr || !(P.resOn || P.pairOn);
    }
    void heat_grids()
    {
        gSaveWater = resident(v.ntStream ? k_heat_save_water<true> : k_heat_save_water<false>); gBoundary = resident(k_heat_boundary);
        gHProps = resident(k_heat_props); gHAsm = resident(v.ntStream ? k_heat_assemble<true> : k_heat_assemble<false>);
        gHPost = resident(k_heat_post); gHSave = resident(k_heat_save);
    }

    void enqueue_props()
    {
        if (heatOn && multi) {
            timed_launch(KID_PROPS, k_props<2, true>, grid);
            launch(k_halo_copy<0>, pgrid);
            launch(k_heat_halo_water, pgrid);
        }
        else if (heatOn) timed_launch(KID_PROPS, k_props<0, true>, propsHeatGrid);
        else if (multi && P.fusedMulti) { timed_launch(KID_PROPS, k_props<2, false>, grid); launch(k_halo_copy<0>, pgrid); }
        else timed_launch(KID_PROPS, k_props<0, false>, propsGrid);
        if (multi && !P.fusedMulti) {
            launch(k_push_kf, pgrid);
            if (I.rcclMode) I.rccl_halo(st, 2);
            launch(k_sync_kf, one);
        }
    }
    void enqueue_slabs()
    {
        auto chk = [&](hipError_t e) { if (e != hipSuccess) slabFailed = true; };
        const int S = I.sw.slabs;
        const uint32_t soil = v.nList - v.nListSurf;
        uint32_t aEnd[8], pEnd[8];
        for (int k = 0; k < S; ++k) {
            double share = (double)(k + 1) / S;
            if (I.sw.slabFirst > 0. && I.sw.slabFirst < 1.) share = (k + 1 == S) ? 1. : I.sw.slabFirst + (1. - I.sw.slabFirst) * (double)k / (double)(S - 1);
            aEnd[k] = (k + 1 == S) ? v.nList : v.nListSurf + (uint32_t)(share * soil);
            pEnd[k] = (k + 1 == S) ? v.nList : I.propsNeed[aEnd[k] - 1];
            if (k > 0 && pEnd[k] < pEnd[k - 1]) pEnd[k] = pEnd[k - 1];
        }
        DevView w = v;
        w.pLo = 0; w.pHi = pEnd[0];
        launch_view(k_props<0, false>, propsGrid, block, 0, st, w); chk(hipGetLastError());
        chk(hipEventRecord(I.evSlab[0], st));
        chk(hipStreamWaitEvent(I.stream3, I.evSlab[0], 0));
        for (int k = 1; k < S; ++k) {
            w.pLo = pEnd[k - 1]; w.pHi = pEnd[k];
            if (w.pHi > w.pLo) { launch_view(k_props<0, false>, dim3(I.sw.slabPropsBlocks), block, 0, I.stream3, w); chk(hipGetLastError()); }
            chk(hipEventRecord(I.evSlab[k], I.stream3));
        }
        w = v;
        for (int k = 0; k < S; ++k) {
            const bool last = k + 1 == S;
            if (k > 0) chk(hipStreamWaitEvent(st, I.evSlab[k], 0));
            w.aLo = k == 0 ? v.nListSurf : aEnd[k - 1]; w.aHi = aEnd[k];
            if (!last) { w.nbSurf = 0; w.nbSoil = I.sw.slabAsmBlocks; }
            else { w.nbSurf = v.nbSurf; w.nbSoil = v.nbSoil; }
            launch_view(assemble_kernel(last, P.asmNT, false), dim3(w.nbSurf + w.nbSoil), block, 0, st, w);
        }
    }
    void enqueue_batch(bool withHead, bool withTail, uint32_t chunk)
    {
        if (withHead) {
            if (P.probeNow) {
                launch(k_props_surface, dim3(v.nbSurf));
                launch(P.asmNT ? k_courant_probe<true> : k_courant_probe<false>, dim3(v.nbSurf));
            }
            if (P.slabOn) enqueue_slabs();
            else {
                enqueue_props();
                timed_launch(KID_ASSEMBLE, assemble_kernel(P.useFused, P.asmNT, heatOn), dim3(v.nbSurf + v.nbSoil));
                if (!P.useFused) {
                    if (!heatOn && I.rcclMode) { hipLaunchKernelGGL(k_local_reduce, one, block, 0, st, v, 1); I.rccl_gather(st); }
                    launch(k_decide_courant, one);
                }
            }
            if (P.compat) launch(k_compat_rows, grid);
        }
        if (P.linealOn) {
            launch(k_cg_init, grid);
            for (uint32_t k = 0; k < chunk; ++k) timed(KID_SWEEP, [&] { launch(k_cg_matvec, grid); launch(k_cg_update, grid); launch(k_cg_dir, grid); });
            launch(k_cg_finish, grid);
        }
        else if (P.resOn) timed(KID_SWEEP_RES, [&] { launch_view(sweepFn, dim3(I.resBlocks), dim3(v.res.NW * 64), I.resLds, st, v); });
        else if (P.pairOn) {
// ... 6 lines not shown
                    if (multi && !v.pair.records) launch(v.ntStream ? k_sweep_bnd<true> : k_sweep_bnd<false>, bgr);
                });
            }
        }
        else for (uint32_t k = 0; k < chunk; ++k) {
            timed_launch(KID_SWEEP, sweep_kernel(P.fused ? 1 : (P.fusedMulti ? 2 : 0), v.ntStream != 0), grid);
            if (P.useFused) continue;
            if (multi) launch(k_push_x, pgrid);
            if (I.rcclMode) { I.rccl_halo(st, 1); hipLaunchKernelGGL(k_local_reduce, one, block, 0, st, v, 3); I.rccl_gather(st); }
            launch(k_decide_sweep, one);
        }
        if (P.useFused) {
            if (!P.resFusedPost) timed_launch(KID_POST, k_post<true>, grid);
            if (multi && v.haloDirect && !P.resFusedPost) launch(k_halo_copy<1>, pgrid);
        }
        else {
            timed_launch(KID_POST, k_post<false>, grid);
            if (I.rcclMode) { hipLaunchKernelGGL(k_local_reduce, one, block, 0, st, v, 2); I.rccl_gather(st); }
            launch(k_decide_balance, one);
        }
        if (withTail) {
            timed_launch(KID_RESTORE, P.useFused ? (heatOn ? k_restore<true, true> : k_restore<true, false>) : (heatOn ? k_restore<false, true> : k_restore<false, false>), grid);
            if (!P.useFused) {
                if (I.rcclMode) { hipLaunchKernelGGL(k_local_reduce, one, block, 0, st, v, 2); I.rccl_gather(st); }
                launch(k_decide_restore, one);
            }
            if (P.overlap) launch(k_accept_boundary, grid);
            else timed_launch(KID_ACCEPT, v.ntStream ? k_accept<true> : k_accept<false>, acceptGrid);
        }
    }
    hipError_t launch_batch(bool withHead, bool withTail, uint32_t chunk)
    {
        if (!P.replayWater) { enqueue_batch(withHead, withTail, chunk); return hipSuccess; }
        return I.replay(water_graph_key(P, withHead, withTail, chunk), st, [&] { enqueue_batch(withHead, withTail, chunk); });
    }
    void enqueue_heat(uint32_t steps, uint32_t chunk)
    {
        for (uint32_t bq = 0; bq < steps; ++bq) {
            launch(k_heat_boundary, gBoundary);
            launch(k_heat_props, gHProps);
            launch(v.ntStream ? k_heat_assemble<true> : k_heat_assemble<false>, gHAsm);
            if (v.heat.gs) {
                for (uint32_t k = 0; k < chunk; ++k) {
                    launch(k_heat_gs_begin, grid);
                    for (size_t l = 0; l + 1 < I.gsLevelStart.size(); ++l) {
                        const uint32_t first = I.gsLevelStart[l], cnt = I.gsLevelStart[l + 1] - first;
                        if (cnt) hipLaunchKernelGGL(k_heat_gs_level, dim3((cnt + SF3D_BLOCK - 1) / SF3D_BLOCK), block, 0, st, v, first, cnt);
                    }
                    hipLaunchKernelGGL(k_heat_gs_decide, one, one, 0, st, v.ctrl);
                }
            } else
            for (uint32_t k = 0; k < chunk; ++k) {
                if (v.heat.redBlack) { launch(v.ntStream ? k_heat_sweep<0, true> : k_heat_sweep<0, false>, grid); launch(v.ntStream ? k_heat_sweep<1, true> : k_heat_sweep<1, false>, grid); }
                else launch(k_heat_sweep<-1, false>, grid);
            }
            launch(k_heat_post, gHPost);
            if (v.heat.save != 0) launch(k_heat_save, gHSave);
        }
    }
    hipError_t launch_heat(uint32_t steps, uint32_t chunk)
    {
        if (!P.replayHeat) { enqueue_heat(steps, chunk); return hipSuccess; }
        return I.replay(heat_graph_key(steps, chunk, v.heat.save != 0), st, [&] { enqueue_heat(steps, chunk); });
    }
    void attribute_events(const Ctrl& c, const StepCounts& before)
    {
        uint64_t ran[KID_COUNT];
        ran[KID_PROPS] = ran[KID_ASSEMBLE] = (c.counters[2] - before.counters[2]) - (c.earlyCourant - before.earlyCourant);
        ran[KID_SWEEP] = P.pairOn ? c.singleLaunches - before.singleLaunches : (P.resOn ? 0 : c.counters[3] - before.counters[3]);
        ran[KID_SWEEP_RES] = c.residentLaunches - before.residentLaunches;
        ran[KID_SWEEP_PAIR] = c.pairLaunches - before.pairLaunches;
        ran[KID_POST] = c.counters[7] - before.counters[7];
        ran[KID_RESTORE] = c.counters[6] - before.counters[6];
        ran[KID_ACCEPT] = c.counters[1] - before.counters[1];
        std::vector<float> el[KID_COUNT];
        for (auto& pr : I.pending) {
            float t = 0.f;
            if (hipEventElapsedTime(&t, pr.a, pr.b) == hipSuccess) el[pr.kid].push_back(t);
            I.freeEvents.push_back(pr.a); I.freeEvents.push_back(pr.b);
        }
        I.pending.clear();
        for (int k = 0; k < KID_COUNT; ++k) {
            std::sort(el[k].begin(), el[k].end(), [](float x, float y) { return x > y; });
            for (size_t q = 0; q < el[k].size() && q < ran[k]; ++q) { I.ms[k] += el[k][q]; I.launches[k]++; }
        }
    }
};

sf3d_error_t DeviceSolver::step_water(StepCtx& c, double maxTimeStep, uint32_t& stage)
{
    Impl& I = c.I; const DevView& v = c.v; const StepPlan& P = c.P; hipStream_t st = c.st;
    if (!c.water_grids()) { snprintf(err_, sizeof(err_), "no kernel was compiled for the sweep form of this model (%s)", P.resOn ? "resident loop" : "paired pass"); fatal_ = true; return SF3D_SOLVER_ERROR; }
    {
        const uint32_t ringSlots = mirror_.aRing < 2u ? 2u : mirror_.aRing;
        if (I.pend.n && (!P.overlap || I.links_pending((mirror_.aBuf + 1u) % ringSlots))) HIP_TRY(I.flush_links());
    }
    hipLaunchKernelGGL(k_step_begin, c.one, c.one, 0, st, v.ctrl, maxTimeStep);
    stage = ST_APPROX;
    StepCounts before(mirror_);
    const uint64_t approxAtStart = mirror_.counters[2];
    int guard = 0;
    if (P.slabOn && !I.stream3) {
        HIP_TRY(hipStreamCreateWithFlags(&I.stream3, hipStreamNonBlocking));
        for (auto& ev : I.evSlab) HIP_TRY(hipEventCreateWithFlags(&ev, hipEventDisableTiming));
    }
    uint32_t look = water_look_ahead(I.lastBatches);
    uint32_t batchIndex = 0;
    while (true) {
        RoctxRange pollRange(look > 1 ? "sf3d water: look-ahead batches of approximations + poll" : "sf3d water: one approximation batch + poll");
        for (uint32_t bq = 0; bq < look; ++bq) {
            const bool head = bq > 0 || stage == ST_APPROX;
            HIP_TRY(c.launch_batch(head, bq + 1 == look, predicted_sweeps(batchIndex, head, I.predCount, I.pred, I.lastSweeps)));
            if (head) ++batchIndex;
        }
        look = 1;
        HIP_TRY(hipGetLastError());
        if (c.slabFailed) { I.sw.slabs = 0; snprintf(err_, sizeof(err_), "SF3D_SLAB_OVERLAP: a launch or an event call of the slab experiment failed - its rows may have read stale node properties"); (void)hipStreamSynchronize(st); fatal_ = true; return SF3D_SOLVER_ERROR; }
        HIP_TRY(hipMemcpyAsync(I.hostCtrl, v.ctrl, sizeof(Ctrl), hipMemcpyDeviceToHost, st));
        HIP_TRY(hipStreamSynchronize(st));
        const Ctrl& hc = *I.hostCtrl;
        if (P.timedStep) c.attribute_events(hc, before);
        before = StepCounts(hc);

        stage = hc.stage;
        if (stage != ST_SWEEP && hc.iter > 0) I.lastSweeps = hc.iter;
        if (stage == ST_ACCEPT || stage == ST_FAIL) break;
        if (++guard > 1000000) { snprintf(err_, sizeof(err_), "step state machine did not terminate (stage %u)", stage); return SF3D_SOLVER_ERROR; }
    }
    {
        const uint64_t used = I.hostCtrl->counters[2] - approxAtStart;
        I.lastBatches = used < 1 ? 1u : (uint32_t)used;
        I.predCount = I.hostCtrl->seqCount < 16u ? I.hostCtrl->seqCount : 16u;
        for (uint32_t k = 0; k < I.predCount; ++k) I.pred[k] = I.hostCtrl->seqSweeps[k];
    }
    if (P.overlap && stage == ST_ACCEPT) {
        const Ctrl& hc = *I.hostCtrl;
        if (I.pend.n >= (uint32_t)SF3D_LINKS_RING) HIP_TRY(I.flush_links());
        I.pend.slot[I.pend.n] = hc.acceptABuf < (uint32_t)SF3D_LINKS_RING ? hc.acceptABuf : 0u; I.pend.dt[I.pend.n] = hc.acceptDt; ++I.pend.n;
    }
    return SF3D_OK;
}

sf3d_error_t DeviceSolver::step_heat(StepCtx& c, HostModel& m, double maxTimeStep, uint32_t& stage)
{
    Impl& I = c.I; const DevView& v = c.v; hipStream_t st = c.st;
    hipLaunchKernelGGL(k_heat_begin, c.one, c.one, 0, st, v.ctrl, maxTimeStep, m.water ? 1 : 0);
    c.heat_grids();
    c.launch(k_heat_save_water_props, c.resident(k_heat_save_water_props));
    c.launch(v.ntStream ? k_heat_save_water<true> : k_heat_save_water<false>, c.gSaveWater);
    int hguard = 0;
    const uint32_t lookH = heat_look_ahead(I.lastHeatSteps, v.heat.gs != 0);
    RoctxRange heatRange("sf3d heat part of computeStep");
    while (true) {
        RoctxRange heatPoll("sf3d heat: sub-steps + poll");
        HIP_TRY(c.launch_heat(lookH, heat_chunk(I.lastHeatSweeps)));
        HIP_TRY(hipGetLastError());
        HIP_TRY(hipMemcpyAsync(I.hostCtrl, v.ctrl, sizeof(Ctrl), hipMemcpyDeviceToHost, st));
        HIP_TRY(hipStreamSynchronize(st));
        const Ctrl& hc = *I.hostCtrl;
        if (hc.hSweepsLast > 0) I.lastHeatSweeps = hc.hSweepsLast;
        if (I.sw.heatDebug == 2) fprintf(stderr, "gpu heatLoop stage %u next dt %g outer %g/%g sweeps %u MBR %.6e storage %.12e sink %.6e courant %.6e\n", hc.hStage, hc.hDt, hc.hOuterDt, hc.hOuterSum, hc.hSweepsLast, hc.heatCur.MBR, hc.heatCur.storage, hc.heatCur.sinkSource, hc.hCourant);
        if (hc.hStage == HS_FINISHED) { I.lastHeatSteps = hc.hRows + hc.hPad; break; }
        if (hc.hStage == HS_IDLE) { snprintf(err_, sizeof(err_), "heat step did not start (water stage %u)", hc.stage); stage = ST_FAIL; fatal_ = true; break; }
        if (++hguard > 1000000) { snprintf(err_, sizeof(err_), "heat state machine did not terminate (stage %u)", hc.hStage); return SF3D_SOLVER_ERROR; }
    }
    if (I.sw.heatDebug) fprintf(stderr, "heat: water dt %g: %u heat steps accepted, %u halved, last dt %g, last sweeps %u, courant %g, MBR %g\n", I.hostCtrl->dtWater, I.hostCtrl->hRows, I.hostCtrl->hPad, I.hostCtrl->hDt, I.hostCtrl->hSweepsLast, I.hostCtrl->hCourant, I.hostCtrl->heatCur.MBR);
    m.hostStaleHeat = true;
    return SF3D_OK;
}

sf3d_error_t DeviceSolver::step_finish(HostModel& m, ParamsHost& p, double maxTimeStep, double* dtOut, uint32_t stage)
{
    Impl& I = *impl_; const DevView& v = I.v; hipStream_t st = I.stream;
    if (world_ == 1 && stage == ST_FAIL && I.hostCtrl->barTimeout && !I.hostCtrl->distError && I.resBlocks != 0) {
        fprintf(stderr, "sf3d: warning: resident sweep loop: a wait for another block's records expired (%u blocks not on the device together: is the GPU shared?) - "
                        "the step is taken again with the sweeps as separate launches, and so are the following ones\n", I.resBlocks);
        I.resBlocks = 0; I.v.res.on = 0; I.v.res.forceTimeout = 0;
        Ctrl c0 = mirror_;
        c0.seSource = 0; c0.barTimeout = 0;
        mirror_ = c0;
        HIP_TRY(hipMemcpyAsync(v.ctrl, &mirror_, sizeof(Ctrl), hipMemcpyHostToDevice, st));
        HIP_TRY(hipStreamSynchronize(st));
        return step(m, p, maxTimeStep, dtOut);
    }
    mirror_ = *I.hostCtrl;
    if (mirror_.distError) {
        char who[96] = ""; size_t at = 0;
        for (int p = 0; p < world_ && at + 6 < sizeof(who); ++p) if ((mirror_.distSilent >> p) & 1u) at += (size_t)snprintf(who + at, sizeof(who) - at, "%s%d", at ? ", " : "", p);
        snprintf(err_, sizeof(err_), "rank %d: no mail from rank(s) %s within the bounded wait of an exchange epoch%s (multi-GPU exchange: the peer died, hangs or runs far behind)", rank_, who[0] ? who : "?", mirror_.pairRecTimeout ? " (the records of a paired pass: SF3D_PAIR_RECORDS=0 exchanges plain values between two launches)" : "");
        fatal_ = true;
    }
    else if (mirror_.barTimeout) { snprintf(err_, sizeof(err_), "resident sweep loop: a wait for another block's records expired (%u blocks not resident at once?%s); SF3D_RESIDENT_SWEEP=0 runs the sweeps as separate launches", I.resBlocks, world_ > 1 ? " or a neighbouring rank's records did not arrive within SF3D_DIST_TIMEOUT_S" : ""); fatal_ = true; }
    else if (stage != ST_ACCEPT && !fatal_) snprintf(err_, sizeof(err_), "the mass balance is not a number at the minimum time step (stepNan, cpusolver.cpp:176-180): state left as the reference leaves it");
    p.dtCurr = mirror_.dtCurr;
    *dtOut = mirror_.dt;
    m.hostStaleState = true;
    m.hostStaleFlows = true;
    return (stage == ST_ACCEPT) ? SF3D_OK : SF3D_SOLVER_ERROR;
}

sf3d_error_t DeviceSolver::step(HostModel& m, ParamsHost& p, double maxTimeStep, double* dtOut)
{
    RoctxRange stepRange("sf3d computeStep");
    sf3d_error_t e = sync_to_device(m, p);
    if (e != SF3D_OK) return e;
    if (world_ > 1 && !connected_) { snprintf(err_, sizeof(err_), "multi-GPU model used before sf3d_dist_connect / sf3d_dist_finalize%s%.150s", distWhy_[0] ? ": " : "", distWhy_); return SF3D_SOLVER_ERROR; }
    Impl& I = *impl_;
    StepFacts f;
    {
        const DevView& v = I.v; const StepSwitches& sw = I.sw;
        f.multi = world_ > 1; f.heatOn = v.heat.on != 0; f.useFused = I.useFused != 0;
        f.lineal = p.lineal; f.haveCg = v.cgDiag != nullptr;
        f.resAvail = v.res.on && I.resBlocks != 0; f.resFusedPost = v.res.fusedPost != 0;
        f.haloDirect = v.haloDirect != 0; f.rccl = I.rcclMode; f.nBnd = v.nBnd; f.pairAvail = I.pairBlocks != 0;
        f.timing = I.timing; f.sampled = I.timing == 2 && (I.stepSeq++ % 8 == 0);
        f.overlapAccept = I.overlapAccept != 0; f.ring = I.ring != 0; f.compat = v.compatCv != nullptr;
        f.ntStream = v.ntStream != 0; f.asmNtOff = sw.asmNtOff;
        f.probeMin = v.probeMin; f.courant = mirror_.courant; f.probeBudget = mirror_.probeBudget;
        f.slabs = sw.slabs; f.havePropsNeed = !I.propsNeed.empty(); f.nList = v.nList; f.nListSurf = v.nListSurf;
        f.useGraphs = sw.graphs; f.heatGs = v.heat.gs != 0;
        f.residentFailAt = sw.residentFailAt; f.residentSteps = I.stepSeqAll;
    }
    StepCtx c(I, plan_step(f), f.multi);
    I.useFused = c.P.useFused ? 1 : 0;
    if (c.P.countsResidentStep) { I.v.res.forceTimeout = c.P.forceTimeout ? 1u : 0u; ++I.stepSeqAll; }

    if (c.heatOn) {
        if (c.v.heat.save == 2) c.launch(k_heat_reset_water_fluxes, c.grid);
        c.launch(k_heat_conductance, c.grid);
        for (int t = 0; t < SF3D_FLUX_TYPES; ++t) m.lfluxValid[t] = false;
    }
    uint32_t stage = ST_ACCEPT;
    if (m.water) { e = step_water(c, maxTimeStep, stage); if (e != SF3D_OK) return e; }
    if (c.heatOn && stage == ST_ACCEPT) { e = step_heat(c, m, maxTimeStep, stage); if (e != SF3D_OK) return e; }
    else if (!m.water) {
        HIP_TRY(hipMemcpyAsync(I.hostCtrl, c.v.ctrl, sizeof(Ctrl), hipMemcpyDeviceToHost, c.st));
        HIP_TRY(hipStreamSynchronize(c.st));
    }
    return step_finish(m, p, maxTimeStep, dtOut, stage);
}
```

### criteria3d_amd/csrc/sf3d_pair.inc

```
template <class T> __device__ __forceinline__ const T* at32(const T* base, uint32_t idx)
{
    return reinterpret_cast<const T*>(reinterpret_cast<const char*>(base) + (idx * (uint32_t)sizeof(T)));
}
template <class T> __device__ __forceinline__ T* at32(T* base, uint32_t idx)
{
    return reinterpret_cast<T*>(reinterpret_cast<char*>(base) + (idx * (uint32_t)sizeof(T)));
}

#ifndef SF3D_PAIR_XCD_ROWS
#define SF3D_PAIR_XCD_ROWS 1
#endif
#ifndef SF3D_PAIR_WAVES
#define SF3D_PAIR_WAVES 6
#endif
#define SF3D_PAIR_WAVES_OF(W) ((W) == 14 ? 4 : ((W) == 8 ? 5 : SF3D_PAIR_WAVES))
__device__ __forceinline__ double pair_wait_record_at(const DevView& v, Ctrl* c, const double* lo, const double* hi, uint32_t tag, uint32_t peer)
{
    long long t0 = 0;
    unsigned long long a = (unsigned long long)__double_as_longlong(SYS_LOAD(lo)), b = (unsigned long long)__double_as_longlong(SYS_LOAD(hi));
    for (uint32_t polls = 0;; ++polls) {
        if (rec_ok(a, b, tag)) return rec_value(a, b);
        if (polls == 0) { t0 = wall_clock64(); if (__hip_atomic_load(&c->pairRecTimeout, __ATOMIC_RELAXED, __HIP_MEMORY_SCOPE_AGENT)) return 0.; }
        else __builtin_amdgcn_s_sleep(1);
        if ((polls & 63u) == 63u && (wall_clock64() - t0 > v.dist->spinTicks || __hip_atomic_load(&c->pairRecTimeout, __ATOMIC_RELAXED, __HIP_MEMORY_SCOPE_AGENT))) {
            atomicOr(&c->pairRecTimeout, 1u); if (peer < SF3D_MAX_RANKS) atomicOr(&c->distSilent, 1u << peer);
            return 0.;
        }
        a = (unsigned long long)__double_as_longlong(SYS_LOAD(lo));
        b = (unsigned long long)__double_as_longlong(SYS_LOAD(hi));
    }
}

__device__ __forceinline__ bool pair_records_failed(Ctrl* c, bool rec)
{
    if (!rec || !__hip_atomic_load(&c->pairRecTimeout, __ATOMIC_RELAXED, __HIP_MEMORY_SCOPE_AGENT)) return false;
    if (threadIdx.x == 0) { c->distError = 1; c->stage = ST_FAIL; }
    return true;
}

template <int W, bool NT, bool DIST, bool RECORDS = false>
__global__ void __launch_bounds__((W + 1) * 64, SF3D_PAIR_WAVES_OF(W)) k_sweep_pair(DevView v)
{
    Ctrl* c = v.ctrl;
    if (c->stage != ST_SWEEP) return;
    if (DIST && c->pairPending) return;
    __shared__ double ring[4][W][66];
    __shared__ double xs[2][W + 2][68];
    __shared__ sf3d_d2 parked[SF3D_SLOTS / 2][W - 2][64];
    __shared__ double parkedB[W - 2][64];
    __shared__ int32_t tabRing[16], tabXs[16];
    __shared__ double sm[4][W + 1];
    int nxt1, nxt2;
    free_buffers2(c, nxt1, nxt2);
    const double* __restrict__ xin = v.X[c->cur];
    const sf3d_d2* __restrict__ A2 = cur_A2(v);
    double* __restrict__ xo1 = v.X[nxt1];
    double* __restrict__ xo2 = v.X[nxt2];
    const int32_t NX = (int32_t)v.pair.NX, NY = (int32_t)v.pair.NY, NZ = (int32_t)v.pair.NZ;
    const int32_t layer = NX * NY;
    if (threadIdx.x < 16) {
        const int32_t n = (int32_t)threadIdx.x, tq = (int32_t)((threadIdx.x * 11u) >> 5);
        tabRing[n] = n < 9 ? (tq - 1) * 66 + (n - 3 * tq - 1) : 0;
        tabXs[n] = n < 9 ? (tq - 1) * 68 + (n - 3 * tq - 1) : 0;
    }
    const int wave = __builtin_amdgcn_readfirstlane(threadIdx.x >> 6), lane = threadIdx.x & 63;
#if SF3D_PAIR_XCD_ROWS
    uint32_t lb;
    {   const uint32_t nb = gridDim.x, x = blockIdx.x & 7u, k = blockIdx.x >> 3, per = nb >> 3, rem = nb & 7u;
        lb = (x < rem ? x * (per + 1u) : rem * (per + 1u) + (x - rem) * per) + k; }
#else
    const uint32_t lb = blockIdx.x;
#endif
    const int pr = (int)(lb / v.pair.patchCols), pc = (int)(lb % v.pair.patchCols);
    const int ownLo = DIST ? (int)v.pair.ownLo : 0, ownHi = DIST ? (int)v.pair.ownHi : NY;
    static_assert(DIST || !RECORDS, "record hand-over is a strip's");
    constexpr bool REC = RECORDS;
    if (DIST && ((v.pair.records != 0u) != REC || (REC && !v.pair.recFast))) return;
    const int bLo = (DIST && !REC && ownLo > 0) ? ownLo + 1 : ownLo, bHi = (DIST && !REC && ownHi < NY) ? ownHi - 1 : ownHi;
    const uint32_t par = DIST ? (c->epoch & 1u) : 0u;
    const uint32_t rtag = DIST ? c->epoch + 1u : 0u;
    const bool later = DIST && c->iter > 0;
    int r0 = ownLo + pr * (W - 2) - 1;
    if (r0 + W > NY + 1) r0 = NY + 1 - W;
    const int c0 = pc * 64;
    const bool halo = wave == W;
    const int prow = halo ? (lane >> 1) : wave;
    const int r = r0 + prow;
    const int col = halo ? ((lane & 1) ? c0 + 64 : c0 - 1) : c0 + lane;
    const int slot = halo ? ((lane & 1) ? 65 : 0) : lane + 1;
    const bool inGrid = prow < W && r >= 0 && r < NY && col >= 0 && col < NX;
    const bool ok = inGrid && (!DIST || (r >= ownLo && r < ownHi));
    const bool foreign = REC && inGrid && !ok;
    constexpr bool FAST = REC;
    const int rowS = __builtin_amdgcn_readfirstlane(r0 + (halo ? 0 : wave));
    const bool edgeRow = DIST && !halo && ((ownLo > 0 && rowS == ownLo) || (ownHi < NY && rowS == ownHi - 1));
    double* putBase = nullptr; uint32_t putLoOff = 0u, putCnt = 0u;
    __shared__ uint32_t getTab[6];
    const double* getBase = nullptr;
    if (DIST && FAST) {
        const DistView* d = v.dist;
        if (edgeRow) {
            const int side = (ownLo > 0 && rowS == ownLo) ? 0 : 1, p = v.pair.sidePeer[side];
            putCnt = d->sendCount[p];
            putBase = d->payload[p] + d->sendOff[p];
            const uint32_t o = par * SF3D_DIST_FIELDS * putCnt + v.pair.putBase[side] - (uint32_t)rowS * (uint32_t)NX;
            putLoOff = o + DF_RECLO * putCnt;
        }
        getBase = d->payload[v.rank];
        if (threadIdx.x < 2) {
            const int side = (int)threadIdx.x, p = v.pair.sidePeer[side];
            const uint32_t cnt = p >= 0 ? d->recvCount[p] : 0u;
            getTab[2 + side] = cnt;
            getTab[4 + side] = p >= 0 ? (uint32_t)d->recvOff[p] + ((par ^ 1u) * SF3D_DIST_FIELDS + DF_X) * cnt + v.pair.getBase[side] - (uint32_t)(side == 0 ? ownLo - 1 : ownHi) * (uint32_t)NX : 0u;
            getTab[side] = p >= 0 ? (uint32_t)d->recvOff[p] + (par * SF3D_DIST_FIELDS + DF_RECLO) * cnt + v.pair.getBase[side] - (uint32_t)(side == 0 ? ownLo - 1 : ownHi) * (uint32_t)NX : 0u;
        }
    }
    const uint32_t recStride = (uint32_t)NX;
    const bool rowsOwned = wave >= 1 && wave <= W - 2;
    const bool owned = rowsOwned && ok && r >= ownLo + pr * (W - 2) && r < ownLo + (pr + 1) * (W - 2) && r < ownHi;
    const bool second = owned && r >= bLo && r < bHi;
    const bool edge = DIST && ok && ((ownLo > 0 && r == ownLo) || (ownHi < NY && r == ownHi - 1));
    const uint32_t i0 = inGrid ? (uint32_t)(r * NX + col) : 0u;
    const bool rowWave = !halo && r >= 0 && r < NY;
    int er = 0, ec = 0;
    bool hasOuter = !rowsOwned;
    if (wave == 0) { er = 0; ec = lane + 2; }
    else if (wave == W - 1) { er = W + 1; ec = lane + 2; }
    else if (halo) {
        if (lane < 2 * W) { er = (lane >> 1) + 1; ec = (lane & 1) ? 67 : 0; }
        else if (lane < 2 * W + 8) { const int k = lane - 2 * W; er = (k & 4) ? W + 1 : 0; ec = (k & 2) ? 66 + (k & 1) : (k & 1); }
        else hasOuter = false;
    }
    const int xr = r0 - 1 + er, xc = c0 - 2 + ec;
    const bool outer = hasOuter && xr >= 0 && xr < NY && xc >= 0 && xc < NX;
    const uint32_t e0 = outer ? (uint32_t)(xr * NX + xc) : 0u;
    const int32_t ePos = er * 68 + ec;
    double n1 = 0., n1l = 0., n2 = 0., n2l = 0.;
    const int32_t ownPos = (prow < W ? prow : 0) * 66 + slot;
    const int32_t xsPos = ((prow < W ? prow : 0) + 1) * 68 + slot + 1;
    sf3d_d2* park = &parked[0][rowsOwned ? wave - 1 : 0][lane];
    double* parkB = &parkedB[rowsOwned ? wave - 1 : 0][lane];
    constexpr uint32_t order[SF3D_SLOTS] = {0, 2, 3, 4, 5, 6, 7, 8, 9, 1};
    constexpr size_t PSTRIDE = (size_t)(W - 2) * 64;
    auto fetch_lat = [&](int t) -> uint32_t {
        const uint32_t i = (uint32_t)t * (uint32_t)layer + i0;
        uint64_t code = 0;
        if (rowWave) code = v.pair.chunkCode[__builtin_amdgcn_readfirstlane(i >> 6)];
        return (code >> 63) ? (uint32_t)(code >> 8) : *at32(v.pair.nodeLat, i);
    };
    uint32_t latP = 0, latC = 0;
    const bool fromWindow = REC && foreign && later;
    if (REC) __syncthreads();
    const uint32_t oldAt = fromWindow ? getTab[4 + (i0 >= (uint32_t)ownHi * (uint32_t)NX ? 1 : 0)] + i0 : 0u;
    const bool outerWin = REC && later && outer && (xr < ownLo || xr >= ownHi);
    const uint32_t outerAt = outerWin ? getTab[4 + (xr >= ownHi ? 1 : 0)] + e0 : 0u;
    if (NZ > 0) {
        if (inGrid) xs[0][0][xsPos] = fromWindow ? SYS_LOAD(getBase + oldAt) : *at32(xin, i0);
        if (outer) xs[0][0][ePos] = outerWin ? SYS_LOAD(getBase + outerAt) : *at32(xin, e0);
    }
    double zP = 0., zc = 0., bc = 0., ac[SF3D_SLOTS];
    auto stage_a = [&](int t, auto haloWave) {
        constexpr bool HALO = decltype(haloWave)::value;
        #pragma unroll
        for (int s = 0; s < SF3D_SLOTS; ++s) ac[s] = 0.;
        bc = 0.;
        double xouter = 0.;
        if (HALO && outer && t + 1 < NZ) xouter = (REC && outerWin) ? SYS_LOAD(getBase + (outerAt + (uint32_t)(t + 1) * recStride)) : *at32(xin, (uint32_t)(t + 1) * (uint32_t)layer + e0);
        if (t < NZ && prow < W) {
            double x1 = 0., xnext = 0., xj[SF3D_SLOTS];
            const uint32_t i = (uint32_t)t * (uint32_t)layer + i0;
            const double* xo = &xs[t & 1][0][0] + xsPos;
            double* xw = &xs[(t + 1) & 1][0][0];
            if (inGrid && t + 1 < NZ) xnext = (REC && fromWindow) ? SYS_LOAD(getBase + (oldAt + (uint32_t)(t + 1) * recStride)) : *at32(xin, i + (uint32_t)layer);
            if (ok) {
                #pragma unroll
                for (int p = 0; p < SF3D_SLOTS / 2; ++p) { const sf3d_d2 w = load_coeff<NT>(at32(A2 + (size_t)p * v.N, i)); ac[2 * p] = w.x; ac[2 * p + 1] = w.y; }
                bc = *at32(v.b, i);
                if (owned || t == 0) zc = *at32(v.z, i);
                latC = fetch_lat(t);
                xj[0] = xw[xsPos];
                xj[1] = xnext;
                #pragma unroll
                for (int k = 0; k < SF3D_SLOTS - 2; ++k) xj[2 + k] = xo[tabXs[(latC >> (4 * k)) & 15u]];
                if (DIST && !REC && edge && later) {
                    const DistView* d = v.dist;
                    #pragma unroll
                    for (int s = 0; s < SF3D_SLOTS; ++s) {
                        const uint32_t f = d->fsrc[(size_t)s * v.N + i];
                        if (f != SF3D_FSRC_NONE) {
                            const uint32_t p = f >> 27, k = f & 0x07FFFFFFu;
                            xj[s] = SYS_LOAD(d->payload[v.rank] + d->recvOff[p] + (size_t)((par ^ 1u) * SF3D_DIST_FIELDS + DF_X) * d->recvCount[p] + k);
                        }
                    }
                }
                x1 = bc;
                #pragma unroll
                for (int o = 0; o < SF3D_SLOTS; ++o) { const uint32_t s = order[o]; if (ac[s] != 0.) x1 -= ac[s] * xj[s]; }
                if (t == 0) x1 = dmax(x1, zc);
            }
            xw[xsPos] = xnext;
            ring[t & 3][0][ownPos] = x1;
            if (!HALO && owned) {
                double d = fabs(x1 - xo[0]);
                const double psi = fabs(x1 - zc);
                if (psi > 1.) d *= (1. / psi);
                dd_add(n1, n1l, d);
                *at32(xo1, i) = x1;
            }
            if (DIST && !HALO && owned && edge) {
                if (REC) {
                    double* dst = putBase + (putLoOff + i0 + (uint32_t)t * recStride);
                    SYS_STORE(dst, __longlong_as_double((long long)rec_lo(x1, rtag)));
                    SYS_STORE(dst + putCnt, __longlong_as_double((long long)rec_hi(x1, rtag)));
                } else dist_put_chunk(v, __builtin_amdgcn_readfirstlane(((uint32_t)t * (uint32_t)layer + i0) >> 6), (uint32_t)lane, par, DF_X, x1);
            }
        }
        if (DIST && HALO && foreign && t >= 1) {
            const uint32_t i = (uint32_t)(t - 1) * (uint32_t)layer + i0;
            const int below = i0 >= (uint32_t)ownHi * (uint32_t)NX ? 1 : 0;
            uint32_t ii = i0;
            asm volatile("" : "+v"(ii));
            const double* q = getBase + (getTab[below] + ii + (uint32_t)(t - 1) * recStride);
            const uint32_t hiAt = getTab[2 + below];
            const double xv = pair_wait_record_at(v, c, q, q + hiAt, rtag, (uint32_t)v.pair.sidePeer[below]);
            ring[(t - 1) & 3][0][ownPos] = xv;
            *at32(xo1, i) = xv;
        }
        if (HALO && hasOuter) xs[(t + 1) & 1][0][ePos] = xouter;
    };
    __syncthreads();
    const bool foreignRow = REC && !halo && (rowS < ownLo || rowS >= ownHi);
    if (!rowsOwned || foreignRow) {
        for (int t = 0; t <= NZ; ++t) { stage_a(t, std::true_type{}); __syncthreads(); }
    } else for (int t = 0; t <= NZ; ++t) {
        latP = latC;
        zP = zc;
        stage_a(t, std::false_type{});
        __syncthreads();
        if (owned) {
            double ap[SF3D_SLOTS];
            #pragma unroll
            for (int p = 0; p < SF3D_SLOTS / 2; ++p) {
                const sf3d_d2 w = park[(size_t)p * PSTRIDE];
                sf3d_d2 n; n.x = ac[2 * p]; n.y = ac[2 * p + 1];
                park[(size_t)p * PSTRIDE] = n;
                ap[2 * p] = w.x; ap[2 * p + 1] = w.y;
            }
            const double bP = *parkB;
            *parkB = bc;
            if (t >= 1 && second) {
                const int l = t - 1;
                const uint32_t i = (uint32_t)l * (uint32_t)layer + i0;
                const double* own = &ring[l & 3][0][0] + ownPos;
                double xj[SF3D_SLOTS];
                #pragma unroll
                for (int k = 0; k < SF3D_SLOTS - 2; ++k) xj[2 + k] = own[tabRing[(latP >> (4 * k)) & 15u]];
                xj[0] = ring[(l + 3) & 3][0][ownPos];
                xj[1] = ring[(l + 1) & 3][0][ownPos];
                const double x1 = own[0];
                double x2 = bP;
                #pragma unroll
                for (int o = 0; o < SF3D_SLOTS; ++o) { const uint32_t s = order[o]; if (ap[s] != 0.) x2 -= ap[s] * xj[s]; }
                if (l == 0) x2 = dmax(x2, zP);
                double d = fabs(x2 - x1);
                const double psi = fabs(x2 - zP);
                if (psi > 1.) d *= (1. / psi);
                dd_add(n2, n2l, d);
                *at32(xo2, i) = x2;
                if (DIST && REC && edge) SYS_STORE(putBase + (putLoOff - DF_RECLO * putCnt + i0 + (uint32_t)l * recStride), x2);
            }
        }
    }
    if (DIST) asm volatile("s_waitcnt vmcnt(0)" ::: "memory");
    wave_sum_dd(n1, n1l); wave_sum_dd(n2, n2l);
    if (lane == 0) { sm[0][wave] = n1; sm[1][wave] = n1l; sm[2][wave] = n2; sm[3][wave] = n2l; }
    __syncthreads();
    double s1 = 0., s1l = 0., s2 = 0., s2l = 0.;
    if (threadIdx.x == 0) for (int w = 0; w <= W; ++w) { dd_merge(s1, s1l, sm[0][w], sm[1][w]); dd_merge(s2, s2l, sm[2][w], sm[3][w]); }
    if (!arrive_last4(v, s1, s1l, s2, s2l)) return;
    double t1, t1l, t2, t2l;
    sum_published_dd(v.part0, v.part1, gridDim.x, t1, t1l);
    sum_published_dd(v.part2, v.part3, gridDim.x, t2, t2l);
    wave_sum_dd(t1, t1l); wave_sum_dd(t2, t2l);
    __syncthreads();
    if (lane == 0) { sm[0][wave] = t1; sm[1][wave] = t1l; sm[2][wave] = t2; sm[3][wave] = t2l; }
    __syncthreads();
    double a = sm[0][0], al = sm[1][0], b = sm[2][0], bl = sm[3][0];
    for (int w = 1; w < SF3D_BLOCK / 64; ++w) { dd_merge(a, al, sm[0][w], sm[1][w]); dd_merge(b, bl, sm[2][w], sm[3][w]); }
    if (DIST) {
        double vals[4] = {a, al, b, bl};
        __syncthreads();
        if (pair_records_failed(c, REC)) return;
        if (!dist_allgather(v, c, vals, 3)) return;
        if (threadIdx.x == 0) {
            c->pairLaunches++;
            sweep_decision(c, nxt1, (vals[0] + vals[1]) / v.Nnorm);
            if (REC) {
                if (c->stage == ST_SWEEP) sweep_decision(c, nxt2, (vals[2] + vals[3]) / v.Nnorm);
                else c->haloLocalTag = c->epoch + 1u;
            } else if (c->stage == ST_SWEEP) { c->pairNorm2 = vals[2]; c->pairNorm2Lo = vals[3]; c->pairX2 = nxt2; c->pairPending = 1; }
        }
        return;
    }
    if (threadIdx.x == 0) {
        c->pairLaunches++;
        sweep_decision(c, nxt1, (a + al) / v.Nnorm);
        if (c->stage == ST_SWEEP) sweep_decision(c, nxt2, (b + bl) / v.Nnorm);
    }
}
```

Before: 46.68.

## Exchange pair-sweep halo rows between blocks via tagged records on a single GPU

Adds a local-records variant of the paired sweep kernel for single-device runs. Blocks publish their edge-row first-sweep values to a tagged record buffer and neighbouring blocks spin-wait on those records, instead of recomputing the halo rows redundantly. The aim is to cut the duplicated halo computation and let blocks carry fewer extra rows. It depends on all blocks being co-resident, so it adds an occupancy check and a timeout that falls back to the old path and retakes the step. It also relaxes grid planning to allow NZ=1 and to accept heights close to NY.

Measured after the change: 46.35. About the same (-0.7%).

```diff
diff --git a/criteria3d_amd/csrc/sf3d_device.h b/criteria3d_amd/csrc/sf3d_device.h
--- a/criteria3d_amd/csrc/sf3d_device.h
+++ b/criteria3d_amd/csrc/sf3d_device.h
@@ -206,6 +206,10 @@
     uint32_t putBase[2], getBase[2];
     uint32_t recStride;
     const uint8_t* role;
+    uint32_t local;
+    uint32_t lrFail;
+    double* lrec;
+    uint32_t* lrTag;
 };
 
 struct ResGrid {
@@ -718,6 +722,6 @@
     uint64_t ver;
 };
 
-enum { KID_PROPS = 0, KID_ASSEMBLE, KID_SWEEP, KID_POST, KID_RESTORE, KID_ACCEPT, KID_SWEEP_PAIR, KID_SWEEP_RES, KID_MAPS, KID_COUNT };
+enum { KID_PROPS = 0, KID_ASSEMBLE, KID_SWEEP, KID_POST, KID_RESTORE, KID_ACCEPT, KID_SWEEP_PAIR, KID_SWEEP_RES, KID_MAPS, KID_SWEEP_PAIR_LOCAL, KID_COUNT };
 
 #endif
diff --git a/criteria3d_amd/csrc/sf3d_host_build.inc b/criteria3d_amd/csrc/sf3d_host_build.inc
--- a/criteria3d_amd/csrc/sf3d_host_build.inc
+++ b/criteria3d_amd/csrc/sf3d_host_build.inc
@@ -1,7 +1,7 @@
 
 namespace {
 
-const char* kKernelNames[KID_COUNT] = {"k_props", "k_assemble", "k_sweep", "k_post", "k_restore", "k_accept", "k_sweep_pair", "k_sweep_resident", "k_output_map"};
+const char* kKernelNames[KID_COUNT] = {"k_props", "k_assemble", "k_sweep", "k_post", "k_restore", "k_accept", "k_sweep_pair", "k_sweep_resident", "k_output_map", "k_sweep_pair_local"};
 
 }
 
@@ -21,8 +21,13 @@
     return nullptr;
 }
 #define SF3D_PAIR_FOR_HEIGHTS(X) X(6) X(8) X(10) X(14)
-static ViewKernel pair_kernel(uint32_t W, bool nt, bool dist, bool records, bool masked)
-{
+static ViewKernel pair_kernel(uint32_t W, bool nt, bool dist, bool records, bool masked, bool local = false)
+{
+    if (local && !dist && !masked) {
+        if (W == 6) return nt ? k_sweep_pair_local<6, true> : k_sweep_pair_local<6, false>;
+        if (W == 10) return nt ? k_sweep_pair_local<10, true> : k_sweep_pair_local<10, false>;
+        return nullptr;
+    }
 #define SF3D_PAIR_PTR(w)                                                                                                                      \
     if (W == w) {                                                                                                                             \
         if (masked) return dist ? (nt ? k_sweep_pair_masked<w, true, true> : k_sweep_pair_masked<w, false, true>)                             \
@@ -150,6 +155,8 @@
     bool asmNtOff = false;
     bool pairOddSingle = true;
     long residentFailAt = -1;
+    bool pairLocal = true;
+    long pairLocalFailAt = -1;
     int heatDebug = 0;
     int slabs = 0;
     uint32_t slabPropsBlocks = 512, slabAsmBlocks = 512; double slabFirst = 0.;
@@ -276,6 +283,7 @@
     uint32_t resCapacity = 0;
     uint32_t pairRecordsWish = 0;
     uint64_t stepSeq = 0;
+    uint64_t stepSeqPairLocal = 0;
     uint64_t stepSeqAll = 0;
     struct Pair { hipEvent_t a, b; int kid; };
     std::vector<Pair> pending;
@@ -488,6 +496,8 @@
     s.asmNtOff = off("SF3D_ASM_NT");
     s.pairOddSingle = !off("SF3D_PAIR_ODD_SINGLE");
     if (const char* fe = getenv("SF3D_RESIDENT_FAIL_TEST")) s.residentFailAt = strtol(fe, nullptr, 10);
+    s.pairLocal = !off("SF3D_PAIR_LOCAL_RECORDS");
+    if (const char* fe = getenv("SF3D_PAIR_LOCAL_FAIL_TEST")) s.pairLocalFailAt = strtol(fe, nullptr, 10);
     if (const char* he = getenv("SF3D_HEAT_DEBUG")) s.heatDebug = he[0] == '2' ? 2 : 1;
     { const char* e = getenv("SF3D_SLAB_OVERLAP"); s.slabs = e ? atoi(e) : 0; if (s.slabs > 8) s.slabs = 8; if (s.slabs < 2) s.slabs = 0; }
     auto blocks_of = [](const char* e) -> uint32_t { const long n = e ? strtol(e, nullptr, 10) : 512L; return (uint32_t)(n < 1 ? 1 : (n > SF3D_MAX_BLOCKS ? SF3D_MAX_BLOCKS : n)); };
@@ -687,7 +697,7 @@
         v.res = ResGrid{};
         I.resBlocks = 0; I.resLds = 0;
         const bool asked = sw.residentSweep;
-        const bool want = asked && I.useFused != 0 && !pairNode.empty() && pairIdxMap.empty() && (world_ == 1 || v.haloDirect);
+        const bool want = asked && I.useFused != 0 && !pairNode.empty() && pairIdxMap.empty() && pairNZ >= 2 && (world_ == 1 || v.haloDirect);
         if (want) {
             const uint32_t ownRows = pairOwnHi - pairOwnLo, patchCols = pairNX / 64;
             int cus = 256; { hipDeviceProp_t prop; if (hipGetDeviceProperties(&prop, I.device) == hipSuccess && prop.multiProcessorCount > 0) cus = prop.multiProcessorCount; }
@@ -1028,6 +1038,21 @@
                         v.pair.masked = 1; v.pair.idxMap = dm; v.pair.patchList = dl; v.pair.patchDepth = dd;
                         I.pairBlocks = (uint32_t)plist[wi].size(); I.pairMasked = true;
                     }
+                    v.pair.local = 0u; v.pair.lrFail = 0u; v.pair.lrec = nullptr; v.pair.lrTag = nullptr;
+                    if (I.sw.pairLocal && world_ == 1 && !I.pairMasked) {
+                        PairLocalFacts lf;
+                        lf.world = world_; lf.masked = I.pairMasked; lf.NX = pairNX; lf.NY = pairNY; lf.W = bestW;
+                        lf.fused = I.useFused != 0; lf.sideLaunches = I.sw.slabs >= 2;
+                        const ViewKernel lfn = pair_kernel(bestW, v.ntStream != 0, false, false, false, true);
+                        int perCu = 0;
+                        if (lfn && hipOccupancyMaxActiveBlocksPerMultiprocessor(&perCu, lfn, (int)(bestW + 1) * 64, 0) == hipSuccess && perCu > 0) lf.slots = (uint64_t)perCu * (uint64_t)cus;
+                        else (void)hipGetLastError();
+                        if (plan_pair_local(lf)) {
+                            HIP_TRY(dev_alloc(I.allocs, v.pair.lrec, (size_t)2 * N)); HIP_TRY(hipMemset(v.pair.lrec, 0, (size_t)2 * N * 8));
+                            HIP_TRY(dev_alloc(I.allocs, v.pair.lrTag, 1)); HIP_TRY(hipMemset(v.pair.lrTag, 0, sizeof(uint32_t)));
+                            v.pair.local = 1u;
+                        }
+                    }
                 }
             }
         }
diff --git a/criteria3d_amd/csrc/sf3d_host_plan.inc b/criteria3d_amd/csrc/sf3d_host_plan.inc
--- a/criteria3d_amd/csrc/sf3d_host_plan.inc
+++ b/criteria3d_amd/csrc/sf3d_host_plan.inc
@@ -290,7 +290,7 @@
     std::vector<uint64_t>&pairNode = g.node, &pairChunk = g.chunk;
     uint32_t &pairNX = g.NX, &pairNY = g.NY, &pairNZ = g.NZ;
     const uint32_t N = m.N, ns = m.ns, nChunks = (N + SF3D_CHUNK - 1) / SF3D_CHUNK;
-    bool regular = ns >= 64 && N % ns == 0 && N / ns >= 2 && N < (1u << 28);
+    bool regular = ns >= 64 && N % ns == 0 && N / ns >= 1 && N < (1u << 28);
     int64_t maxOff = 0;
     if (regular) {
         for (int sl = 2; sl < SF3D_SLOTS && regular; ++sl)
@@ -597,7 +597,8 @@
     }
     const uint32_t ownRows = pairOwnHi - pairOwnLo;
     for (uint32_t W : {6u, 8u, 10u, 14u}) {
-        if (pairNY < W || (wSet && onlyW != W)) continue;
+        const bool askedFits = wSet && onlyW == W && world == 1 && pairIdxMap.empty() && pairNY + 2 >= W;
+        if ((pairNY < W && !askedFits) || (wSet && onlyW != W)) continue;
         if (W == 8 && !wSet) continue;
         const uint64_t blocks = pairIdxMap.empty() ? (uint64_t)((ownRows + W - 3) / (W - 2)) * (pairNX / 64) : (uint64_t)plist[pair_widx(W)].size();
         if (blocks == 0) continue;
@@ -610,6 +611,21 @@
     }
     if (tryAuto && !(bestCost < autoCost)) bestW = 0;
     return pp;
+}
+
+struct PairLocalFacts {
+    int world = 1; bool masked = false;
+    uint32_t NX = 0, NY = 0, W = 0;
+    uint64_t slots = 0;
+    bool fused = true, sideLaunches = false;
+};
+inline bool plan_pair_local(const PairLocalFacts& f)
+{
+    if (f.world != 1 || f.masked) return false;
+    if (f.W < 6 || f.NX == 0 || f.NX % 64 != 0 || f.NY < f.W - 2 || f.NY % (f.W - 2) != 0) return false;
+    const uint64_t blocks = (uint64_t)(f.NY / (f.W - 2)) * (f.NX / 64);
+    if (blocks == 0 || blocks > f.slots) return false;
+    return f.fused && !f.sideLaunches;
 }
 
 inline bool plan_edge_rows_direct(const Partition& part, const GridPlan& g, uint32_t ns, int world, int rank, EdgeRows& er)
@@ -676,6 +692,8 @@
     int slabs = 0; bool havePropsNeed = false; uint32_t nList = 0, nListSurf = 0;
     bool useGraphs = true, heatGs = false;
     long residentFailAt = -1; uint64_t residentSteps = 0;
+    bool pairLocalAvail = false;
+    long pairLocalFailAt = -1; uint64_t pairLocalSteps = 0;
 };
 struct StepPlan {
     bool useFused;
@@ -685,6 +703,8 @@
     bool resFusedPost;
     bool countsResidentStep, forceTimeout;
     bool pairOn;
+    bool pairLocal;
+    bool pairLocalFail;
     bool timedStep;
     bool overlap;
     bool compat, asmNT;
@@ -704,6 +724,8 @@
     P.countsResidentStep = P.resOn && !f.multi;
     P.forceTimeout = P.countsResidentStep && f.residentFailAt >= 0 && (long)f.residentSteps == f.residentFailAt;
     P.pairOn = !P.resOn && (P.fused || (P.fusedMulti && f.haloDirect && f.nBnd != 0)) && f.pairAvail && !P.linealOn;
+    P.pairLocal = P.pairOn && P.fused && f.pairLocalAvail;
+    P.pairLocalFail = P.pairLocal && f.pairLocalFailAt >= 0 && (long)f.pairLocalSteps == f.pairLocalFailAt;
     P.timedStep = f.timing == 1 || (f.timing == 2 && f.sampled);
     P.overlap = f.overlapAccept && !f.multi && f.ring && !P.timedStep && f.timing != 1 && !f.compat;
     P.compat = f.compat;
@@ -739,7 +761,7 @@
 inline uint32_t heat_look_ahead(uint32_t lastHeatSteps, bool gs) { return gs ? 1 : (lastHeatSteps < 1 ? 1 : (lastHeatSteps > 8 ? 8 : lastHeatSteps)); }
 
 enum : uint32_t { GK_HEAT = 1u, GK_HEAD = 2u, GK_TAIL = 4u, GK_RES = 8u, GK_RES_POST = 16u, GK_RES_FAIL = 32u, GK_OVERLAP = 64u, GK_PAIR = 128u,
-                  GK_LINEAL = 256u, GK_PROBE = 512u, GK_SLAB = 1024u, GK_SAVE = 2048u };
+                  GK_LINEAL = 256u, GK_PROBE = 512u, GK_SLAB = 1024u, GK_SAVE = 2048u, GK_PAIR_LOCAL = 4096u, GK_PAIR_LOCAL_FAIL = 8192u };
 struct GraphKey {
     uint32_t flags, sweeps, steps;
     bool operator==(const GraphKey& o) const { return flags == o.flags && sweeps == o.sweeps && steps == o.steps; }
@@ -747,7 +769,8 @@
 inline GraphKey water_graph_key(const StepPlan& P, bool withHead, bool withTail, uint32_t chunk)
 {
     const uint32_t flags = (withHead ? GK_HEAD : 0u) | (withTail ? GK_TAIL : 0u) | (P.resOn ? GK_RES : 0u) | (P.resFusedPost ? GK_RES_POST : 0u) | (P.forceTimeout ? GK_RES_FAIL : 0u)
-                           | (P.overlap ? GK_OVERLAP : 0u) | (P.pairOn ? GK_PAIR : 0u) | (P.linealOn ? GK_LINEAL : 0u) | (P.probeNow ? GK_PROBE : 0u) | (P.slabOn ? GK_SLAB : 0u);
+                           | (P.overlap ? GK_OVERLAP : 0u) | (P.pairOn ? GK_PAIR : 0u) | (P.linealOn ? GK_LINEAL : 0u) | (P.probeNow ? GK_PROBE : 0u) | (P.slabOn ? GK_SLAB : 0u)
+                           | (P.pairLocal ? GK_PAIR_LOCAL : 0u) | (P.pairLocalFail ? GK_PAIR_LOCAL_FAIL : 0u);
     return {flags, P.resOn ? 0u : chunk, 0u};
 }
 inline GraphKey heat_graph_key(uint32_t steps, uint32_t chunk, bool save) { return {GK_HEAT | (save ? GK_SAVE : 0u), chunk, steps}; }
diff --git a/criteria3d_amd/csrc/sf3d_host_step.inc b/criteria3d_amd/csrc/sf3d_host_step.inc
--- a/criteria3d_amd/csrc/sf3d_host_step.inc
+++ b/criteria3d_amd/csrc/sf3d_host_step.inc
@@ -727,7 +727,7 @@
         propsGrid = resident(k_props<0, false>); propsHeatGrid = resident(k_props<0, true>);
         acceptGrid = resident(v.ntStream ? k_accept<true> : k_accept<false>);
         if (P.resOn) sweepFn = res_kernel((int)v.res.K, (int)v.res.NW, multi);
-        else if (P.pairOn) sweepFn = pair_kernel(v.pair.W, v.ntStream != 0, multi, v.pair.records != 0, I.pairMasked);
+        else if (P.pairOn) sweepFn = pair_kernel(v.pair.W, v.ntStream != 0, multi, v.pair.records != 0, I.pairMasked, P.pairLocal);
         return sweepFn != nullptr || !(P.resOn || P.pairOn);
     }
     void heat_grids()
@@ -900,7 +900,10 @@
         I.pending.clear();
         for (int k = 0; k < KID_COUNT; ++k) {
             std::sort(el[k].begin(), el[k].end(), [](float x, float y) { return x > y; });
-            for (size_t q = 0; q < el[k].size() && q < ran[k]; ++q) { I.ms[k] += el[k][q]; I.launches[k]++; }
+            for (size_t q = 0; q < el[k].size() && q < ran[k]; ++q) {
+                I.ms[k] += el[k][q]; I.launches[k]++;
+                if (k == KID_SWEEP_PAIR && P.pairLocal) I.launches[KID_SWEEP_PAIR_LOCAL]++;
+            }
         }
     }
 };
@@ -990,6 +993,17 @@
 sf3d_error_t DeviceSolver::step_finish(HostModel& m, ParamsHost& p, double maxTimeStep, double* dtOut, uint32_t stage)
 {
     Impl& I = *impl_; const DevView& v = I.v; hipStream_t st = I.stream;
+    if (world_ == 1 && stage == ST_FAIL && I.hostCtrl->pairRecTimeout && !I.hostCtrl->distError && I.v.pair.local) {
+        fprintf(stderr, "sf3d: warning: paired pass: a wait for another block's records expired (%u blocks not on the device together: is the GPU shared?) - "
+                        "the step is taken again with the halo rows recomputed, and so are the following ones\n", I.pairBlocks);
+        I.v.pair.local = 0; I.v.pair.lrFail = 0;
+        Ctrl c0 = mirror_;
+        c0.seSource = 0; c0.pairRecTimeout = 0;
+        mirror_ = c0;
+        HIP_TRY(hipMemcpyAsync(v.ctrl, &mirror_, sizeof(Ctrl), hipMemcpyHostToDevice, st));
+        HIP_TRY(hipStreamSynchronize(st));
+        return step(m, p, maxTimeStep, dtOut);
+    }
     if (world_ == 1 && stage == ST_FAIL && I.hostCtrl->barTimeout && !I.hostCtrl->distError && I.resBlocks != 0) {
         fprintf(stderr, "sf3d: warning: resident sweep loop: a wait for another block's records expired (%u blocks not on the device together: is the GPU shared?) - "
                         "the step is taken again with the sweeps as separate launches, and so are the following ones\n", I.resBlocks);
@@ -1038,10 +1052,12 @@
         f.slabs = sw.slabs; f.havePropsNeed = !I.propsNeed.empty(); f.nList = v.nList; f.nListSurf = v.nListSurf;
         f.useGraphs = sw.graphs; f.heatGs = v.heat.gs != 0;
         f.residentFailAt = sw.residentFailAt; f.residentSteps = I.stepSeqAll;
+        f.pairLocalAvail = v.pair.local != 0; f.pairLocalFailAt = sw.pairLocalFailAt; f.pairLocalSteps = I.stepSeqPairLocal;
     }
     StepCtx c(I, plan_step(f), f.multi);
     I.useFused = c.P.useFused ? 1 : 0;
     if (c.P.countsResidentStep) { I.v.res.forceTimeout = c.P.forceTimeout ? 1u : 0u; ++I.stepSeqAll; }
+    if (c.P.pairLocal) { I.v.pair.lrFail = c.P.pairLocalFail ? 1u : 0u; ++I.stepSeqPairLocal; }
 
     if (c.heatOn) {
         if (c.v.heat.save == 2) c.launch(k_heat_reset_water_fluxes, c.grid);
diff --git a/criteria3d_amd/csrc/sf3d_pair.inc b/criteria3d_amd/csrc/sf3d_pair.inc
--- a/criteria3d_amd/csrc/sf3d_pair.inc
+++ b/criteria3d_amd/csrc/sf3d_pair.inc
@@ -1,3 +1,6 @@
+#ifndef SF3D_PAIR_LOCAL_SPIN_TICKS
+#define SF3D_PAIR_LOCAL_SPIN_TICKS 300000000LL
+#endif
 template <class T> __device__ __forceinline__ const T* at32(const T* base, uint32_t idx)
 {
     return reinterpret_cast<const T*>(reinterpret_cast<const char*>(base) + (idx * (uint32_t)sizeof(T)));
@@ -14,6 +17,7 @@
 #define SF3D_PAIR_WAVES 6
 #endif
 #define SF3D_PAIR_WAVES_OF(W) ((W) == 14 ? 4 : ((W) == 8 ? 5 : SF3D_PAIR_WAVES))
+template <bool LOCAL = false>
 __device__ __forceinline__ double pair_wait_record_at(const DevView& v, Ctrl* c, const double* lo, const double* hi, uint32_t tag, uint32_t peer)
 {
     long long t0 = 0;
@@ -22,7 +26,7 @@
         if (rec_ok(a, b, tag)) return rec_value(a, b);
         if (polls == 0) { t0 = wall_clock64(); if (__hip_atomic_load(&c->pairRecTimeout, __ATOMIC_RELAXED, __HIP_MEMORY_SCOPE_AGENT)) return 0.; }
         else __builtin_amdgcn_s_sleep(1);
-        if ((polls & 63u) == 63u && (wall_clock64() - t0 > v.dist->spinTicks || __hip_atomic_load(&c->pairRecTimeout, __ATOMIC_RELAXED, __HIP_MEMORY_SCOPE_AGENT))) {
+        if ((polls & 63u) == 63u && (wall_clock64() - t0 > (LOCAL ? SF3D_PAIR_LOCAL_SPIN_TICKS : v.dist->spinTicks)  || __hip_atomic_load(&c->pairRecTimeout, __ATOMIC_RELAXED, __HIP_MEMORY_SCOPE_AGENT))) {
             atomicOr(&c->pairRecTimeout, 1u); if (peer < SF3D_MAX_RANKS) atomicOr(&c->distSilent, 1u << peer);
             return 0.;
         }
@@ -41,270 +45,12 @@
 template <int W, bool NT, bool DIST, bool RECORDS = false>
 __global__ void __launch_bounds__((W + 1) * 64, SF3D_PAIR_WAVES_OF(W)) k_sweep_pair(DevView v)
 {
-    Ctrl* c = v.ctrl;
-    if (c->stage != ST_SWEEP) return;
-    if (DIST && c->pairPending) return;
-    __shared__ double ring[4][W][66];
-    __shared__ double xs[2][W + 2][68];
-    __shared__ sf3d_d2 parked[SF3D_SLOTS / 2][W - 2][64];
-    __shared__ double parkedB[W - 2][64];
-    __shared__ int32_t tabRing[16], tabXs[16];
-    __shared__ double sm[4][W + 1];
-    int nxt1, nxt2;
-    free_buffers2(c, nxt1, nxt2);
-    const double* __restrict__ xin = v.X[c->cur];
-    const sf3d_d2* __restrict__ A2 = cur_A2(v);
-    double* __restrict__ xo1 = v.X[nxt1];
-    double* __restrict__ xo2 = v.X[nxt2];
-    const int32_t NX = (int32_t)v.pair.NX, NY = (int32_t)v.pair.NY, NZ = (int32_t)v.pair.NZ;
-    const int32_t layer = NX * NY;
-    if (threadIdx.x < 16) {
-        const int32_t n = (int32_t)threadIdx.x, tq = (int32_t)((threadIdx.x * 11u) >> 5);
-        tabRing[n] = n < 9 ? (tq - 1) * 66 + (n - 3 * tq - 1) : 0;
-        tabXs[n] = n < 9 ? (tq - 1) * 68 + (n - 3 * tq - 1) : 0;
-    }
-    const int wave = __builtin_amdgcn_readfirstlane(threadIdx.x >> 6), lane = threadIdx.x & 63;
-#if SF3D_PAIR_XCD_ROWS
-    uint32_t lb;
-    {   const uint32_t nb = gridDim.x, x = blockIdx.x & 7u, k = blockIdx.x >> 3, per = nb >> 3, rem = nb & 7u;
-        lb = (x < rem ? x * (per + 1u) : rem * (per + 1u) + (x - rem) * per) + k; }
-#else
-    const uint32_t lb = blockIdx.x;
-#endif
-    const int pr = (int)(lb / v.pair.patchCols), pc = (int)(lb % v.pair.patchCols);
-    const int ownLo = DIST ? (int)v.pair.ownLo : 0, ownHi = DIST ? (int)v.pair.ownHi : NY;
-    static_assert(DIST || !RECORDS, "record hand-over is a strip's");
-    constexpr bool REC = RECORDS;
-    if (DIST && ((v.pair.records != 0u) != REC || (REC && !v.pair.recFast))) return;
-    const int bLo = (DIST && !REC && ownLo > 0) ? ownLo + 1 : ownLo, bHi = (DIST && !REC && ownHi < NY) ? ownHi - 1 : ownHi;
-    const uint32_t par = DIST ? (c->epoch & 1u) : 0u;
-    const uint32_t rtag = DIST ? c->epoch + 1u : 0u;
-    const bool later = DIST && c->iter > 0;
-    int r0 = ownLo + pr * (W - 2) - 1;
-    if (r0 + W > NY + 1) r0 = NY + 1 - W;
-    const int c0 = pc * 64;
-    const bool halo = wave == W;
-    const int prow = halo ? (lane >> 1) : wave;
-    const int r = r0 + prow;
-    const int col = halo ? ((lane & 1) ? c0 + 64 : c0 - 1) : c0 + lane;
-    const int slot = halo ? ((lane & 1) ? 65 : 0) : lane + 1;
-    const bool inGrid = prow < W && r >= 0 && r < NY && col >= 0 && col < NX;
-    const bool ok = inGrid && (!DIST || (r >= ownLo && r < ownHi));
-    const bool foreign = REC && inGrid && !ok;
-    constexpr bool FAST = REC;
-    const int rowS = __builtin_amdgcn_readfirstlane(r0 + (halo ? 0 : wave));
-    const bool edgeRow = DIST && !halo && ((ownLo > 0 && rowS == ownLo) || (ownHi < NY && rowS == ownHi - 1));
-    double* putBase = nullptr; uint32_t putLoOff = 0u, putCnt = 0u;
-    __shared__ uint32_t getTab[6];
-    const double* getBase = nullptr;
-    if (DIST && FAST) {
-        const DistView* d = v.dist;
-        if (edgeRow) {
-            const int side = (ownLo > 0 && rowS == ownLo) ? 0 : 1, p = v.pair.sidePeer[side];
-            putCnt = d->sendCount[p];
-            putBase = d->payload[p] + d->sendOff[p];
-            const uint32_t o = par * SF3D_DIST_FIELDS * putCnt + v.pair.putBase[side] - (uint32_t)rowS * (uint32_t)NX;
-            putLoOff = o + DF_RECLO * putCnt;
-        }
-        getBase = d->payload[v.rank];
-        if (threadIdx.x < 2) {
-            const int side = (int)threadIdx.x, p = v.pair.sidePeer[side];
-            const uint32_t cnt = p >= 0 ? d->recvCount[p] : 0u;
-            getTab[2 + side] = cnt;
-            getTab[4 + side] = p >= 0 ? (uint32_t)d->recvOff[p] + ((par ^ 1u) * SF3D_DIST_FIELDS + DF_X) * cnt + v.pair.getBase[side] - (uint32_t)(side == 0 ? ownLo - 1 : ownHi) * (uint32_t)NX : 0u;
-            getTab[side] = p >= 0 ? (uint32_t)d->recvOff[p] + (par * SF3D_DIST_FIELDS + DF_RECLO) * cnt + v.pair.getBase[side] - (uint32_t)(side == 0 ? ownLo - 1 : ownHi) * (uint32_t)NX : 0u;
-        }
-    }
-    const uint32_t recStride = (uint32_t)NX;
-    const bool rowsOwned = wave >= 1 && wave <= W - 2;
-    const bool owned = rowsOwned && ok && r >= ownLo + pr * (W - 2) && r < ownLo + (pr + 1) * (W - 2) && r < ownHi;
-    const bool second = owned && r >= bLo && r < bHi;
-    const bool edge = DIST && ok && ((ownLo > 0 && r == ownLo) || (ownHi < NY && r == ownHi - 1));
-    const uint32_t i0 = inGrid ? (uint32_t)(r * NX + col) : 0u;
-    const bool rowWave = !halo && r >= 0 && r < NY;
-    int er = 0, ec = 0;
-    bool hasOuter = !rowsOwned;
-    if (wave == 0) { er = 0; ec = lane + 2; }
-    else if (wave == W - 1) { er = W + 1; ec = lane + 2; }
-    else if (halo) {
-        if (lane < 2 * W) { er = (lane >> 1) + 1; ec = (lane & 1) ? 67 : 0; }
-        else if (lane < 2 * W + 8) { const int k = lane - 2 * W; er = (k & 4) ? W + 1 : 0; ec = (k & 2) ? 66 + (k & 1) : (k & 1); }
-        else hasOuter = false;
-    }
-    const int xr = r0 - 1 + er, xc = c0 - 2 + ec;
-    const bool outer = hasOuter && xr >= 0 && xr < NY && xc >= 0 && xc < NX;
-    const uint32_t e0 = outer ? (uint32_t)(xr * NX + xc) : 0u;
-    const int32_t ePos = er * 68 + ec;
-    double n1 = 0., n1l = 0., n2 = 0., n2l = 0.;
-    const int32_t ownPos = (prow < W ? prow : 0) * 66 + slot;
-    const int32_t xsPos = ((prow < W ? prow : 0) + 1) * 68 + slot + 1;
-    sf3d_d2* park = &parked[0][rowsOwned ? wave - 1 : 0][lane];
-    double* parkB = &parkedB[rowsOwned ? wave - 1 : 0][lane];
-    constexpr uint32_t order[SF3D_SLOTS] = {0, 2, 3, 4, 5, 6, 7, 8, 9, 1};
-    constexpr size_t PSTRIDE = (size_t)(W - 2) * 64;
-    auto fetch_lat = [&](int t) -> uint32_t {
-        const uint32_t i = (uint32_t)t * (uint32_t)layer + i0;
-        uint64_t code = 0;
-        if (rowWave) code = v.pair.chunkCode[__builtin_amdgcn_readfirstlane(i >> 6)];
-        return (code >> 63) ? (uint32_t)(code >> 8) : *at32(v.pair.nodeLat, i);
-    };
-    uint32_t latP = 0, latC = 0;
-    const bool fromWindow = REC && foreign && later;
-    if (REC) __syncthreads();
-    const uint32_t oldAt = fromWindow ? getTab[4 + (i0 >= (uint32_t)ownHi * (uint32_t)NX ? 1 : 0)] + i0 : 0u;
-    const bool outerWin = REC && later && outer && (xr < ownLo || xr >= ownHi);
-    const uint32_t outerAt = outerWin ? getTab[4 + (xr >= ownHi ? 1 : 0)] + e0 : 0u;
-    if (NZ > 0) {
-        if (inGrid) xs[0][0][xsPos] = fromWindow ? SYS_LOAD(getBase + oldAt) : *at32(xin, i0);
-        if (outer) xs[0][0][ePos] = outerWin ? SYS_LOAD(getBase + outerAt) : *at32(xin, e0);
-    }
-    double zP = 0., zc = 0., bc = 0., ac[SF3D_SLOTS];
-    auto stage_a = [&](int t, auto haloWave) {
-        constexpr bool HALO = decltype(haloWave)::value;
-        #pragma unroll
-        for (int s = 0; s < SF3D_SLOTS; ++s) ac[s] = 0.;
-        bc = 0.;
-        double xouter = 0.;
-        if (HALO && outer && t + 1 < NZ) xouter = (REC && outerWin) ? SYS_LOAD(getBase + (outerAt + (uint32_t)(t + 1) * recStride)) : *at32(xin, (uint32_t)(t + 1) * (uint32_t)layer + e0);
-        if (t < NZ && prow < W) {
-            double x1 = 0., xnext = 0., xj[SF3D_SLOTS];
-            const uint32_t i = (uint32_t)t * (uint32_t)layer + i0;
-            const double* xo = &xs[t & 1][0][0] + xsPos;
-            double* xw = &xs[(t + 1) & 1][0][0];
-            if (inGrid && t + 1 < NZ) xnext = (REC && fromWindow) ? SYS_LOAD(getBase + (oldAt + (uint32_t)(t + 1) * recStride)) : *at32(xin, i + (uint32_t)layer);
-            if (ok) {
-                #pragma unroll
-                for (int p = 0; p < SF3D_SLOTS / 2; ++p) { const sf3d_d2 w = load_coeff<NT>(at32(A2 + (size_t)p * v.N, i)); ac[2 * p] = w.x; ac[2 * p + 1] = w.y; }
-                bc = *at32(v.b, i);
-                if (owned || t == 0) zc = *at32(v.z, i);
-                latC = fetch_lat(t);
-                xj[0] = xw[xsPos];
-                xj[1] = xnext;
-                #pragma unroll
-                for (int k = 0; k < SF3D_SLOTS - 2; ++k) xj[2 + k] = xo[tabXs[(latC >> (4 * k)) & 15u]];
-                if (DIST && !REC && edge && later) {
-                    const DistView* d = v.dist;
-                    #pragma unroll
-                    for (int s = 0; s < SF3D_SLOTS; ++s) {
-                        const uint32_t f = d->fsrc[(size_t)s * v.N + i];
-                        if (f != SF3D_FSRC_NONE) {
-                            const uint32_t p = f >> 27, k = f & 0x07FFFFFFu;
-                            xj[s] = SYS_LOAD(d->payload[v.rank] + d->recvOff[p] + (size_t)((par ^ 1u) * SF3D_DIST_FIELDS + DF_X) * d->recvCount[p] + k);
-                        }
-                    }
-                }
-                x1 = bc;
-                #pragma unroll
-                for (int o = 0; o < SF3D_SLOTS; ++o) { const uint32_t s = order[o]; if (ac[s] != 0.) x1 -= ac[s] * xj[s]; }
-                if (t == 0) x1 = dmax(x1, zc);
-            }
-            xw[xsPos] = xnext;
-            ring[t & 3][0][ownPos] = x1;
-            if (!HALO && owned) {
-                double d = fabs(x1 - xo[0]);
-                const double psi = fabs(x1 - zc);
-                if (psi > 1.) d *= (1. / psi);
-                dd_add(n1, n1l, d);
-                *at32(xo1, i) = x1;
-            }
-            if (DIST && !HALO && owned && edge) {
-                if (REC) {
-                    double* dst = putBase + (putLoOff + i0 + (uint32_t)t * recStride);
-                    SYS_STORE(dst, __longlong_as_double((long long)rec_lo(x1, rtag)));
-                    SYS_STORE(dst + putCnt, __longlong_as_double((long long)rec_hi(x1, rtag)));
-                } else dist_put_chunk(v, __builtin_amdgcn_readfirstlane(((uint32_t)t * (uint32_t)layer + i0) >> 6), (uint32_t)lane, par, DF_X, x1);
-            }
-        }
-        if (DIST && HALO && foreign && t >= 1) {
-            const uint32_t i = (uint32_t)(t - 1) * (uint32_t)layer + i0;
-            const int below = i0 >= (uint32_t)ownHi * (uint32_t)NX ? 1 : 0;
-            uint32_t ii = i0;
-            asm volatile("" : "+v"(ii));
-            const double* q = getBase + (getTab[below] + ii + (uint32_t)(t - 1) * recStride);
-            const uint32_t hiAt = getTab[2 + below];
-            const double xv = pair_wait_record_at(v, c, q, q + hiAt, rtag, (uint32_t)v.pair.sidePeer[below]);
-            ring[(t - 1) & 3][0][ownPos] = xv;
-            *at32(xo1, i) = xv;
-        }
-        if (HALO && hasOuter) xs[(t + 1) & 1][0][ePos] = xouter;
-    };
-    __syncthreads();
-    const bool foreignRow = REC && !halo && (rowS < ownLo || rowS >= ownHi);
-    if (!rowsOwned || foreignRow) {
-        for (int t = 0; t <= NZ; ++t) { stage_a(t, std::true_type{}); __syncthreads(); }
-    } else for (int t = 0; t <= NZ; ++t) {
-        latP = latC;
-        zP = zc;
-        stage_a(t, std::false_type{});
-        __syncthreads();
-        if (owned) {
-            double ap[SF3D_SLOTS];
-            #pragma unroll
-            for (int p = 0; p < SF3D_SLOTS / 2; ++p) {
-                const sf3d_d2 w = park[(size_t)p * PSTRIDE];
-                sf3d_d2 n; n.x = ac[2 * p]; n.y = ac[2 * p + 1];
-                park[(size_t)p * PSTRIDE] = n;
-                ap[2 * p] = w.x; ap[2 * p + 1] = w.y;
-            }
-            const double bP = *parkB;
-            *parkB = bc;
-            if (t >= 1 && second) {
-                const int l = t - 1;
-                const uint32_t i = (uint32_t)l * (uint32_t)layer + i0;
-                const double* own = &ring[l & 3][0][0] + ownPos;
-                double xj[SF3D_SLOTS];
-                #pragma unroll
-                for (int k = 0; k < SF3D_SLOTS - 2; ++k) xj[2 + k] = own[tabRing[(latP >> (4 * k)) & 15u]];
-                xj[0] = ring[(l + 3) & 3][0][ownPos];
-                xj[1] = ring[(l + 1) & 3][0][ownPos];
-                const double x1 = own[0];
-                double x2 = bP;
-                #pragma unroll
-                for (int o = 0; o < SF3D_SLOTS; ++o) { const uint32_t s = order[o]; if (ap[s] != 0.) x2 -= ap[s] * xj[s]; }
-                if (l == 0) x2 = dmax(x2, zP);
-                double d = fabs(x2 - x1);
-                const double psi = fabs(x2 - zP);
-                if (psi > 1.) d *= (1. / psi);
-                dd_add(n2, n2l, d);
-                *at32(xo2, i) = x2;
-                if (DIST && REC && edge) SYS_STORE(putBase + (putLoOff - DF_RECLO * putCnt + i0 + (uint32_t)l * recStride), x2);
-            }
-        }
-    }
-    if (DIST) asm volatile("s_waitcnt vmcnt(0)" ::: "memory");
-    wave_sum_dd(n1, n1l); wave_sum_dd(n2, n2l);
-    if (lane == 0) { sm[0][wave] = n1; sm[1][wave] = n1l; sm[2][wave] = n2; sm[3][wave] = n2l; }
-    __syncthreads();
-    double s1 = 0., s1l = 0., s2 = 0., s2l = 0.;
-    if (threadIdx.x == 0) for (int w = 0; w <= W; ++w) { dd_merge(s1, s1l, sm[0][w], sm[1][w]); dd_merge(s2, s2l, sm[2][w], sm[3][w]); }
-    if (!arrive_last4(v, s1, s1l, s2, s2l)) return;
-    double t1, t1l, t2, t2l;
-    sum_published_dd(v.part0, v.part1, gridDim.x, t1, t1l);
-    sum_published_dd(v.part2, v.part3, gridDim.x, t2, t2l);
-    wave_sum_dd(t1, t1l); wave_sum_dd(t2, t2l);
-    __syncthreads();
-    if (lane == 0) { sm[0][wave] = t1; sm[1][wave] = t1l; sm[2][wave] = t2; sm[3][wave] = t2l; }
-    __syncthreads();
-    double a = sm[0][0], al = sm[1][0], b = sm[2][0], bl = sm[3][0];
-    for (int w = 1; w < SF3D_BLOCK / 64; ++w) { dd_merge(a, al, sm[0][w], sm[1][w]); dd_merge(b, bl, sm[2][w], sm[3][w]); }
-    if (DIST) {
-        double vals[4] = {a, al, b, bl};
-        __syncthreads();
-        if (pair_records_failed(c, REC)) return;
-        if (!dist_allgather(v, c, vals, 3)) return;
-        if (threadIdx.x == 0) {
-            c->pairLaunches++;
-            sweep_decision(c, nxt1, (vals[0] + vals[1]) / v.Nnorm);
-            if (REC) {
-                if (c->stage == ST_SWEEP) sweep_decision(c, nxt2, (vals[2] + vals[3]) / v.Nnorm);
-                else c->haloLocalTag = c->epoch + 1u;
-            } else if (c->stage == ST_SWEEP) { c->pairNorm2 = vals[2]; c->pairNorm2Lo = vals[3]; c->pairX2 = nxt2; c->pairPending = 1; }
-        }
-        return;
-    }
-    if (threadIdx.x == 0) {
-        c->pairLaunches++;
-        sweep_decision(c, nxt1, (a + al) / v.Nnorm);
-        if (c->stage == ST_SWEEP) sweep_decision(c, nxt2, (b + bl) / v.Nnorm);
-    }
+    constexpr bool LOCAL = false;
+#include "sf3d_pair_body.inc"
 }
+template <int W, bool NT>
+__global__ void __launch_bounds__((W + 1) * 64, SF3D_PAIR_WAVES_OF(W)) k_sweep_pair_local(DevView v)
+{
+    constexpr bool DIST = false, RECORDS = false, LOCAL = true;
+#include "sf3d_pair_body.inc"
+}
diff --git a/criteria3d_amd/csrc/sf3d_pair_body.inc b/criteria3d_amd/csrc/sf3d_pair_body.inc
--- /dev/null
+++ b/criteria3d_amd/csrc/sf3d_pair_body.inc
@@ -0,0 +1,284 @@
+    Ctrl* c = v.ctrl;
+    if (c->stage != ST_SWEEP) return;
+    if (DIST && c->pairPending) return;
+    __shared__ double ring[4][W][66];
+    __shared__ double xs[2][W + 2][68];
+    __shared__ sf3d_d2 parked[SF3D_SLOTS / 2][W - 2][64];
+    __shared__ double parkedB[W - 2][64];
+    __shared__ int32_t tabRing[16], tabXs[16];
+    __shared__ double sm[4][W + 1];
+    int nxt1, nxt2;
+    free_buffers2(c, nxt1, nxt2);
+    const double* __restrict__ xin = v.X[c->cur];
+    const sf3d_d2* __restrict__ A2 = cur_A2(v);
+    double* __restrict__ xo1 = v.X[nxt1];
+    double* __restrict__ xo2 = v.X[nxt2];
+    const int32_t NX = (int32_t)v.pair.NX, NY = (int32_t)v.pair.NY, NZ = (int32_t)v.pair.NZ;
+    const int32_t layer = NX * NY;
+    if (threadIdx.x < 16) {
+        const int32_t n = (int32_t)threadIdx.x, tq = (int32_t)((threadIdx.x * 11u) >> 5);
+        tabRing[n] = n < 9 ? (tq - 1) * 66 + (n - 3 * tq - 1) : 0;
+        tabXs[n] = n < 9 ? (tq - 1) * 68 + (n - 3 * tq - 1) : 0;
+    }
+    const int wave = __builtin_amdgcn_readfirstlane(threadIdx.x >> 6), lane = threadIdx.x & 63;
+#if SF3D_PAIR_XCD_ROWS
+    uint32_t lb;
+    {   const uint32_t nb = gridDim.x, x = blockIdx.x & 7u, k = blockIdx.x >> 3, per = nb >> 3, rem = nb & 7u;
+        lb = (x < rem ? x * (per + 1u) : rem * (per + 1u) + (x - rem) * per) + k; }
+#else
+    const uint32_t lb = blockIdx.x;
+#endif
+    const int pr = (int)(lb / v.pair.patchCols), pc = (int)(lb % v.pair.patchCols);
+    const int ownLo = DIST ? (int)v.pair.ownLo : 0, ownHi = DIST ? (int)v.pair.ownHi : NY;
+    static_assert(DIST || !RECORDS, "record hand-over is a strip's");
+    static_assert(!LOCAL || !DIST, "the hand-over between blocks is one GPU's");
+    if (LOCAL && (!v.pair.local || !v.pair.lrec || !v.pair.lrTag)) return;
+    uint32_t ltag = 0u;
+    if (LOCAL) { ltag = __builtin_amdgcn_readfirstlane(*v.pair.lrTag + 1u); if (ltag == 0u) ltag = 1u; }
+    if (LOCAL && v.pair.lrFail && threadIdx.x == 0) atomicOr(&c->pairRecTimeout, 1u);
+    constexpr bool REC = RECORDS;
+    if (DIST && ((v.pair.records != 0u) != REC || (REC && !v.pair.recFast))) return;
+    const int bLo = (DIST && !REC && ownLo > 0) ? ownLo + 1 : ownLo, bHi = (DIST && !REC && ownHi < NY) ? ownHi - 1 : ownHi;
+    const uint32_t par = DIST ? (c->epoch & 1u) : 0u;
+    const uint32_t rtag = DIST ? c->epoch + 1u : 0u;
+    const bool later = DIST && c->iter > 0;
+    int r0 = ownLo + pr * (W - 2) - 1;
+    if (r0 + W > NY + 1) r0 = NY + 1 - W;
+    const int c0 = pc * 64;
+    const bool halo = wave == W;
+    const int prow = halo ? (lane >> 1) : wave;
+    const int r = r0 + prow;
+    const int col = halo ? ((lane & 1) ? c0 + 64 : c0 - 1) : c0 + lane;
+    const int slot = halo ? ((lane & 1) ? 65 : 0) : lane + 1;
+    const bool inGrid = prow < W && r >= 0 && r < NY && col >= 0 && col < NX;
+    const bool recvCell = LOCAL && inGrid && (prow == 0 || prow == W - 1);
+    const bool ok = inGrid && (!DIST || (r >= ownLo && r < ownHi)) && !recvCell;
+    const bool foreign = REC && inGrid && !ok;
+    constexpr bool FAST = REC;
+    const int rowS = __builtin_amdgcn_readfirstlane(r0 + (halo ? 0 : wave));
+    const bool edgeRow = DIST && !halo && ((ownLo > 0 && rowS == ownLo) || (ownHi < NY && rowS == ownHi - 1));
+    double* putBase = nullptr; uint32_t putLoOff = 0u, putCnt = 0u;
+    __shared__ uint32_t getTab[6];
+    const double* getBase = nullptr;
+    if (DIST && FAST) {
+        const DistView* d = v.dist;
+        if (edgeRow) {
+            const int side = (ownLo > 0 && rowS == ownLo) ? 0 : 1, p = v.pair.sidePeer[side];
+            putCnt = d->sendCount[p];
+            putBase = d->payload[p] + d->sendOff[p];
+            const uint32_t o = par * SF3D_DIST_FIELDS * putCnt + v.pair.putBase[side] - (uint32_t)rowS * (uint32_t)NX;
+            putLoOff = o + DF_RECLO * putCnt;
+        }
+        getBase = d->payload[v.rank];
+        if (threadIdx.x < 2) {
+            const int side = (int)threadIdx.x, p = v.pair.sidePeer[side];
+            const uint32_t cnt = p >= 0 ? d->recvCount[p] : 0u;
+            getTab[2 + side] = cnt;
+            getTab[4 + side] = p >= 0 ? (uint32_t)d->recvOff[p] + ((par ^ 1u) * SF3D_DIST_FIELDS + DF_X) * cnt + v.pair.getBase[side] - (uint32_t)(side == 0 ? ownLo - 1 : ownHi) * (uint32_t)NX : 0u;
+            getTab[side] = p >= 0 ? (uint32_t)d->recvOff[p] + (par * SF3D_DIST_FIELDS + DF_RECLO) * cnt + v.pair.getBase[side] - (uint32_t)(side == 0 ? ownLo - 1 : ownHi) * (uint32_t)NX : 0u;
+        }
+    }
+    const uint32_t recStride = (uint32_t)NX;
+    const bool rowsOwned = wave >= 1 && wave <= W - 2;
+    const bool owned = rowsOwned && ok && r >= ownLo + pr * (W - 2) && r < ownLo + (pr + 1) * (W - 2) && r < ownHi;
+    const bool second = owned && r >= bLo && r < bHi;
+    const bool edge = DIST && ok && ((ownLo > 0 && r == ownLo) || (ownHi < NY && r == ownHi - 1));
+    const uint32_t i0 = inGrid ? (uint32_t)(r * NX + col) : 0u;
+    const bool rowWave = !halo && r >= 0 && r < NY;
+    int er = 0, ec = 0;
+    bool hasOuter = !rowsOwned;
+    if (wave == 0) { er = 0; ec = lane + 2; if (LOCAL) hasOuter = false; }
+    else if (wave == W - 1) { er = W + 1; ec = lane + 2; if (LOCAL) hasOuter = false; }
+    else if (halo) {
+        if (lane < 2 * W) { er = (lane >> 1) + 1; ec = (lane & 1) ? 67 : 0; }
+        else if (lane < 2 * W + 8 && !LOCAL) { const int k = lane - 2 * W; er = (k & 4) ? W + 1 : 0; ec = (k & 2) ? 66 + (k & 1) : (k & 1); }
+        else hasOuter = false;
+    }
+    const int xr = r0 - 1 + er, xc = c0 - 2 + ec;
+    const bool outer = hasOuter && xr >= 0 && xr < NY && xc >= 0 && xc < NX;
+    const uint32_t e0 = outer ? (uint32_t)(xr * NX + xc) : 0u;
+    const int32_t ePos = er * 68 + ec;
+    double n1 = 0., n1l = 0., n2 = 0., n2l = 0.;
+    const int32_t ownPos = (prow < W ? prow : 0) * 66 + slot;
+    const int32_t xsPos = ((prow < W ? prow : 0) + 1) * 68 + slot + 1;
+    sf3d_d2* park = &parked[0][rowsOwned ? wave - 1 : 0][lane];
+    double* parkB = &parkedB[rowsOwned ? wave - 1 : 0][lane];
+    constexpr uint32_t order[SF3D_SLOTS] = {0, 2, 3, 4, 5, 6, 7, 8, 9, 1};
+    constexpr size_t PSTRIDE = (size_t)(W - 2) * 64;
+    auto fetch_lat = [&](int t) -> uint32_t {
+        const uint32_t i = (uint32_t)t * (uint32_t)layer + i0;
+        uint64_t code = 0;
+        if (rowWave) code = v.pair.chunkCode[__builtin_amdgcn_readfirstlane(i >> 6)];
+        return (code >> 63) ? (uint32_t)(code >> 8) : *at32(v.pair.nodeLat, i);
+    };
+    uint32_t latP = 0, latC = 0;
+    const bool fromWindow = REC && foreign && later;
+    if (REC) __syncthreads();
+    const uint32_t oldAt = fromWindow ? getTab[4 + (i0 >= (uint32_t)ownHi * (uint32_t)NX ? 1 : 0)] + i0 : 0u;
+    const bool outerWin = REC && later && outer && (xr < ownLo || xr >= ownHi);
+    const uint32_t outerAt = outerWin ? getTab[4 + (xr >= ownHi ? 1 : 0)] + e0 : 0u;
+    if (NZ > 0) {
+        if (inGrid) xs[0][0][xsPos] = fromWindow ? SYS_LOAD(getBase + oldAt) : *at32(xin, i0);
+        if (outer) xs[0][0][ePos] = outerWin ? SYS_LOAD(getBase + outerAt) : *at32(xin, e0);
+    }
+    double zP = 0., zc = 0., bc = 0., ac[SF3D_SLOTS];
+    auto stage_a = [&](int t, auto haloWave) {
+        constexpr bool HALO = decltype(haloWave)::value;
+        #pragma unroll
+        for (int s = 0; s < SF3D_SLOTS; ++s) ac[s] = 0.;
+        bc = 0.;
+        double xouter = 0.;
+        if (HALO && outer && t + 1 < NZ) xouter = (REC && outerWin) ? SYS_LOAD(getBase + (outerAt + (uint32_t)(t + 1) * recStride)) : *at32(xin, (uint32_t)(t + 1) * (uint32_t)layer + e0);
+        if (t < NZ && prow < W) {
+            double x1 = 0., xnext = 0., xj[SF3D_SLOTS];
+            const uint32_t i = (uint32_t)t * (uint32_t)layer + i0;
+            const double* xo = &xs[t & 1][0][0] + xsPos;
+            double* xw = &xs[(t + 1) & 1][0][0];
+            if (inGrid && t + 1 < NZ) xnext = (REC && fromWindow) ? SYS_LOAD(getBase + (oldAt + (uint32_t)(t + 1) * recStride)) : *at32(xin, i + (uint32_t)layer);
+            if (ok) {
+                #pragma unroll
+                for (int p = 0; p < SF3D_SLOTS / 2; ++p) { const sf3d_d2 w = load_coeff<NT>(at32(A2 + (size_t)p * v.N, i)); ac[2 * p] = w.x; ac[2 * p + 1] = w.y; }
+                bc = *at32(v.b, i);
+                if (owned || t == 0) zc = *at32(v.z, i);
+                latC = fetch_lat(t);
+                xj[0] = xw[xsPos];
+                xj[1] = xnext;
+                #pragma unroll
+                for (int k = 0; k < SF3D_SLOTS - 2; ++k) xj[2 + k] = xo[tabXs[(latC >> (4 * k)) & 15u]];
+                if (DIST && !REC && edge && later) {
+                    const DistView* d = v.dist;
+                    #pragma unroll
+                    for (int s = 0; s < SF3D_SLOTS; ++s) {
+                        const uint32_t f = d->fsrc[(size_t)s * v.N + i];
+                        if (f != SF3D_FSRC_NONE) {
+                            const uint32_t p = f >> 27, k = f & 0x07FFFFFFu;
+                            xj[s] = SYS_LOAD(d->payload[v.rank] + d->recvOff[p] + (size_t)((par ^ 1u) * SF3D_DIST_FIELDS + DF_X) * d->recvCount[p] + k);
+                        }
+                    }
+                }
+                x1 = bc;
+                #pragma unroll
+                for (int o = 0; o < SF3D_SLOTS; ++o) { const uint32_t s = order[o]; if (ac[s] != 0.) x1 -= ac[s] * xj[s]; }
+                if (t == 0) x1 = dmax(x1, zc);
+            }
+            xw[xsPos] = xnext;
+            ring[t & 3][0][ownPos] = x1;
+            if (!HALO && owned) {
+                double d = fabs(x1 - xo[0]);
+                const double psi = fabs(x1 - zc);
+                if (psi > 1.) d *= (1. / psi);
+                dd_add(n1, n1l, d);
+                *at32(xo1, i) = x1;
+            }
+            if (LOCAL && !HALO && owned && ((wave == 1 && r > 0) || (wave == W - 2 && r + 1 < NY))) {
+                SYS_STORE(at32(v.pair.lrec, i), __longlong_as_double((long long)rec_lo(x1, ltag)));
+                SYS_STORE(at32(v.pair.lrec, i + v.N), __longlong_as_double((long long)rec_hi(x1, ltag)));
+            }
+            if (DIST && !HALO && owned && edge) {
+                if (REC) {
+                    double* dst = putBase + (putLoOff + i0 + (uint32_t)t * recStride);
+                    SYS_STORE(dst, __longlong_as_double((long long)rec_lo(x1, rtag)));
+                    SYS_STORE(dst + putCnt, __longlong_as_double((long long)rec_hi(x1, rtag)));
+                } else dist_put_chunk(v, __builtin_amdgcn_readfirstlane(((uint32_t)t * (uint32_t)layer + i0) >> 6), (uint32_t)lane, par, DF_X, x1);
+            }
+        }
+        if (DIST && HALO && foreign && t >= 1) {
+            const uint32_t i = (uint32_t)(t - 1) * (uint32_t)layer + i0;
+            const int below = i0 >= (uint32_t)ownHi * (uint32_t)NX ? 1 : 0;
+            uint32_t ii = i0;
+            asm volatile("" : "+v"(ii));
+            const double* q = getBase + (getTab[below] + ii + (uint32_t)(t - 1) * recStride);
+            const uint32_t hiAt = getTab[2 + below];
+            const double xv = pair_wait_record_at(v, c, q, q + hiAt, rtag, (uint32_t)v.pair.sidePeer[below]);
+            ring[(t - 1) & 3][0][ownPos] = xv;
+            *at32(xo1, i) = xv;
+        }
+        if (LOCAL && HALO && recvCell && t >= 1) {
+            const uint32_t i = (uint32_t)(t - 1) * (uint32_t)layer + i0;
+            ring[(t - 1) & 3][0][ownPos] = pair_wait_record_at<true>(v, c, at32(v.pair.lrec, i), at32(v.pair.lrec, i + v.N), ltag, SF3D_MAX_RANKS);
+        }
+        if (HALO && hasOuter) xs[(t + 1) & 1][0][ePos] = xouter;
+    };
+    __syncthreads();
+    const bool foreignRow = REC && !halo && (rowS < ownLo || rowS >= ownHi);
+    if (!rowsOwned || foreignRow) {
+        for (int t = 0; t <= NZ; ++t) { stage_a(t, std::true_type{}); __syncthreads(); }
+    } else for (int t = 0; t <= NZ; ++t) {
+        latP = latC;
+        zP = zc;
+        stage_a(t, std::false_type{});
+        __syncthreads();
+        if (owned) {
+            double ap[SF3D_SLOTS];
+            #pragma unroll
+            for (int p = 0; p < SF3D_SLOTS / 2; ++p) {
+                const sf3d_d2 w = park[(size_t)p * PSTRIDE];
+                sf3d_d2 n; n.x = ac[2 * p]; n.y = ac[2 * p + 1];
+                park[(size_t)p * PSTRIDE] = n;
+                ap[2 * p] = w.x; ap[2 * p + 1] = w.y;
+            }
+            const double bP = *parkB;
+            *parkB = bc;
+            if (t >= 1 && second) {
+                const int l = t - 1;
+                const uint32_t i = (uint32_t)l * (uint32_t)layer + i0;
+                const double* own = &ring[l & 3][0][0] + ownPos;
+                double xj[SF3D_SLOTS];
+                #pragma unroll
+                for (int k = 0; k < SF3D_SLOTS - 2; ++k) xj[2 + k] = own[tabRing[(latP >> (4 * k)) & 15u]];
+                xj[0] = ring[(l + 3) & 3][0][ownPos];
+                xj[1] = ring[(l + 1) & 3][0][ownPos];
+                const double x1 = own[0];
+                double x2 = bP;
+                #pragma unroll
+                for (int o = 0; o < SF3D_SLOTS; ++o) { const uint32_t s = order[o]; if (ap[s] != 0.) x2 -= ap[s] * xj[s]; }
+                if (l == 0) x2 = dmax(x2, zP);
+                double d = fabs(x2 - x1);
+                const double psi = fabs(x2 - zP);
+                if (psi > 1.) d *= (1. / psi);
+                dd_add(n2, n2l, d);
+                *at32(xo2, i) = x2;
+                if (DIST && REC && edge) SYS_STORE(putBase + (putLoOff - DF_RECLO * putCnt + i0 + (uint32_t)l * recStride), x2);
+            }
+        }
+    }
+    if (DIST) asm volatile("s_waitcnt vmcnt(0)" ::: "memory");
+    wave_sum_dd(n1, n1l); wave_sum_dd(n2, n2l);
+    if (lane == 0) { sm[0][wave] = n1; sm[1][wave] = n1l; sm[2][wave] = n2; sm[3][wave] = n2l; }
+    __syncthreads();
+    double s1 = 0., s1l = 0., s2 = 0., s2l = 0.;
+    if (threadIdx.x == 0) for (int w = 0; w <= W; ++w) { dd_merge(s1, s1l, sm[0][w], sm[1][w]); dd_merge(s2, s2l, sm[2][w], sm[3][w]); }
+    if (!arrive_last4(v, s1, s1l, s2, s2l)) return;
+    double t1, t1l, t2, t2l;
+    sum_published_dd(v.part0, v.part1, gridDim.x, t1, t1l);
+    sum_published_dd(v.part2, v.part3, gridDim.x, t2, t2l);
+    wave_sum_dd(t1, t1l); wave_sum_dd(t2, t2l);
+    __syncthreads();
+    if (lane == 0) { sm[0][wave] = t1; sm[1][wave] = t1l; sm[2][wave] = t2; sm[3][wave] = t2l; }
+    __syncthreads();
+    double a = sm[0][0], al = sm[1][0], b = sm[2][0], bl = sm[3][0];
+    for (int w = 1; w < SF3D_BLOCK / 64; ++w) { dd_merge(a, al, sm[0][w], sm[1][w]); dd_merge(b, bl, sm[2][w], sm[3][w]); }
+    if (DIST) {
+        double vals[4] = {a, al, b, bl};
+        __syncthreads();
+        if (pair_records_failed(c, REC)) return;
+        if (!dist_allgather(v, c, vals, 3)) return;
+        if (threadIdx.x == 0) {
+            c->pairLaunches++;
+            sweep_decision(c, nxt1, (vals[0] + vals[1]) / v.Nnorm);
+            if (REC) {
+                if (c->stage == ST_SWEEP) sweep_decision(c, nxt2, (vals[2] + vals[3]) / v.Nnorm);
+                else c->haloLocalTag = c->epoch + 1u;
+            } else if (c->stage == ST_SWEEP) { c->pairNorm2 = vals[2]; c->pairNorm2Lo = vals[3]; c->pairX2 = nxt2; c->pairPending = 1; }
+        }
+        return;
+    }
+    if (LOCAL) {
+        if (threadIdx.x == 0) *v.pair.lrTag = ltag;
+        if (__hip_atomic_load(&c->pairRecTimeout, __ATOMIC_RELAXED, __HIP_MEMORY_SCOPE_AGENT)) { if (threadIdx.x == 0) c->stage = ST_FAIL; return; }
+    }
+    if (threadIdx.x == 0) {
+        c->pairLaunches++;
+        sweep_decision(c, nxt1, (a + al) / v.Nnorm);
+        if (c->stage == ST_SWEEP) sweep_decision(c, nxt2, (b + bl) / v.Nnorm);
+    }
```
